# zhengchen1999/DOVE

Hardware: AMD Instinct MI355X
Metric: SR frames/s (33x720x1280 4x one-step, whole job) (higher is better)
Workload: dtype bf16; 1 GPU; synthetic 33x720x1280 HR clip (LR 180x320, 4x), one-step t=399, CogVideoX1.5-5B VAE + 42-layer DiT random-init, 1 clip per GPU (BASELINE configs[1]); weight_sums=True, vae_streams=2, variant=headline (bf16)

## Files before the change

### dove_amd/csrc/graph.hip

```cpp
#include <dlfcn.h>
#include <math.h>
#include <stdio.h>
#include <stdlib.h>
#include <string.h>

#include <algorithm>
#include <map>
#include <string>
#include <unordered_map>
#include <vector>

#include "common.h"
#include "../../include/dove_hip.h"
#include "ctx_access.h"

namespace {

#define CHK(expr)            \
  do {                       \
    const int rc__ = (expr); \
    if (rc__ != 0) return rc__; \
  } while (0)
#define HIPCHK(expr)                                                              \
  do {                                                                            \
// ... 1821 lines not shown
  DOVE_CHECK_ARG(oall, "workspace exhausted (DiT head)");
  std::vector<size_t> g_off(R), g_cnt(R);
  for (int j = 0; j < R; ++j) {
    const long long a0 = std::max<long long>(bounds[j], L) - L, a1 = std::max<long long>(bounds[j + 1], L) - L;
    g_off[j] = (size_t)a0 * width * 2; g_cnt[j] = (size_t)(a1 - a0) * width * 2;
  }
  bf16_t* po = nullptr;
  if (v1 > v0) {
    bf16_t* xv = hs + (size_t)lt_loc * D;
    bf16_t* a1 = A((size_t)(v1 - v0) * D * 2);
    DOVE_CHECK_ARG(a1, "workspace exhausted (DiT head)");
    CHK(dove_layernorm_modulate_bf16(xv, a1, v1 - v0, D, cf.dit_norm_eps, c->nf_g, c->nf_b, nullptr, 0, stream));
    CHK(dove_layernorm_modulate_bf16(a1, n1, v1 - v0, D, cf.dit_norm_eps, c->no_g, c->no_b, c->final_mod, 0, stream));
    CHK(linear(c, n1, v1 - v0, c->proj_out, ConvOpt(), &po, stream));
    c->arena.release(a1);
  }
  CHK(all_gather_v(c, po, oall, g_off.data(), g_cnt.data(), stream));
  CHK(dove_unpatchify(oall, width, T, cf.dit_out_channels, h, w, pt, p, v_out, out_dtype, stream));
  c->arena.release(po); c->arena.release(oall); c->arena.release(n1); c->arena.release(hs);
  return DOVE_OK;
}

extern "C" int dove_dit_forward(dove_ctx* c, const void* hidden, int dtype, int T, int h, int w, const void* text, int L, int timestep,
                                const dove_dit_aux* aux, void* v_out, int out_dtype, void* stream) {
  DOVE_CHECK_ARG(hidden && text && v_out, "dove_dit_forward: null pointer");
  const auto& cf = c->cfg;
  const int p = cf.dit_patch, pt = cf.dit_patch_t, Cc = cf.dit_in_channels, D = cf.dit_heads * cf.dit_head_dim, Hh = cf.dit_heads;
  DOVE_CHECK_ARG(T % pt == 0 && h % p == 0 && w % p == 0 && L >= 1, "dove_dit_forward: T / h / w must be multiples of the patch sizes");
  StageGuard guard(c);
  CHK(ensure_ws(c, 1 + 4 * (T - 1), 8 * h, 8 * w));
  if (c->nranks > 1) return dit_forward_ulysses(c, hidden, dtype, T, h, w, text, L, timestep, aux, v_out, out_dtype, stream);
  const long long nv = (long long)(T / pt) * (h / p) * (w / p), N = L + nv, npad = ru(N, 128);
  const float *cosp, *sinp;
  if (aux && aux->rope_cos && aux->rope_sin) { cosp = aux->rope_cos; sinp = aux->rope_sin; }
  else CHK(rope_tables(c, T / pt, h / p, w / p, &cosp, &sinp, stream));
  CHK(modulation(c, timestep, aux ? aux->timestep_proj : nullptr, stream));
  if (c->attn_n != N) {
    if (c->Qh) { (void)hipFree(c->Qh); (void)hipFree(c->Kh); (void)hipFree(c->Vt); }
    const size_t b = (size_t)Hh * npad * 64 * 2;
    HIPCHK(hipMalloc((void**)&c->Qh, b)); HIPCHK(hipMalloc((void**)&c->Kh, b)); HIPCHK(hipMalloc((void**)&c->Vt, b));
    HIPCHK(hipMemsetAsync(c->Qh, 0, b, (hipStream_t)stream)); HIPCHK(hipMemsetAsync(c->Kh, 0, b, (hipStream_t)stream)); HIPCHK(hipMemsetAsync(c->Vt, 0, b, (hipStream_t)stream));
    c->attn_n = N;
  }
  auto A = [&](size_t bytes) -> bf16_t* { return (bf16_t*)c->arena.alloc(bytes); };
  bf16_t* hs = A((size_t)N * D * 2);
  bf16_t* n1 = A((size_t)N * D * 2);
  const int feat_pad = c->pe_proj.cin_pad;
  bf16_t* tok = A((size_t)nv * feat_pad * 2);
  DOVE_CHECK_ARG(hs && n1 && tok, "workspace exhausted (DiT token buffers)");
  if (feat_pad > Cc * pt * p * p) HIPCHK(hipMemsetAsync(tok, 0, (size_t)nv * feat_pad * 2, (hipStream_t)stream));
  CHK(dove_patchify(hidden, dtype, T, Cc, h, w, pt, p, tok, feat_pad, stream));
  ConvOpt o; bf16_t* dummy;
  o = ConvOpt(); o.out = hs; CHK(linear(c, (const bf16_t*)text, L, c->pe_text, o, &dummy, stream));
  o = ConvOpt(); o.out = hs + (size_t)L * D; CHK(linear(c, tok, nv, c->pe_proj, o, &dummy, stream));
  c->arena.release(tok);
  const float qscale = (1.0f / sqrtf((float)cf.dit_head_dim)) * 1.4426950408889634f;
  float* norm2 = (float*)c->arena.alloc((size_t)Hh * 2 * sizeof(float));
  DOVE_CHECK_ARG(norm2, "workspace exhausted (attention score bounds)");
  if (c->opt_attn_mx && c->attn8_n != N) {
    if (c->Q8) { (void)hipFree(c->Q8); (void)hipFree(c->K8); (void)hipFree(c->V8); (void)hipFree(c->Vs8); }
    const size_t b8 = (size_t)Hh * npad * 64;
    HIPCHK(hipMalloc((void**)&c->Q8, b8)); HIPCHK(hipMalloc((void**)&c->K8, b8)); HIPCHK(hipMalloc((void**)&c->V8, b8));
    HIPCHK(hipMalloc((void**)&c->Vs8, (size_t)Hh * (npad / 64) * 64 * 2));
    HIPCHK(hipMemsetAsync(c->Q8, 0, b8, (hipStream_t)stream)); HIPCHK(hipMemsetAsync(c->K8, 0, b8, (hipStream_t)stream));
    HIPCHK(hipMemsetAsync(c->V8, 0, b8, (hipStream_t)stream)); HIPCHK(hipMemsetAsync(c->Vs8, 0, (size_t)Hh * (npad / 64) * 64 * 2, (hipStream_t)stream));
    c->attn8_n = N;
  }
  auto big = [&](const bf16_t* x, const Packed& pc, const PackedMx& p8, ConvOpt oo, bf16_t** out) -> int {
    if (!c->opt_linear_mx) return linear(c, x, N, pc, oo, out, stream);
    const int K = p8.K, Nn = p8.rows;
    uint8_t* xq = (uint8_t*)c->arena.alloc((size_t)N * K);
    uint32_t* xs = (uint32_t*)c->arena.alloc((size_t)(K / 256) * N * 2 * 4);
    bf16_t* y = oo.out ? oo.out : (bf16_t*)c->arena.alloc((size_t)N * Nn * 2);
    if (!xq || !xs || !y) { dove_set_error("workspace exhausted (MXFP8 linear)"); return DOVE_EINVAL; }
    CHK(dove_mx_quant_bf16(x, N, K, xq, xs, stream));
    CHK(dove_linear_mxfp8(xq, xs, p8.q, p8.s, p8.bias, oo.resid, oo.gate, y, N, Nn, K, Nn, oo.ldr, oo.gate_split, oo.act, stream));
    c->arena.release(xq); c->arena.release(xs);
    *out = y;
    return 0;
  };
  for (auto& b : c->blocks) {
    CHK(dove_layernorm_modulate_bf16(hs, n1, N, D, cf.dit_norm_eps, b.ln1_g, b.ln1_b, b.m1, L, stream));
    bf16_t* qkv;
    CHK(big(n1, b.qkv, b.qkv8, ConvOpt(), &qkv));
    if (c->opt_attn_mx) {
      CHK(dove_qkv_post_mxfp8(qkv, N, npad, Hh, 64, L, b.nq_g, b.nq_b, b.nk_g, b.nk_b, cosp, sinp, qscale, 1e-6f, c->Q8, c->K8, c->V8, c->Vs8, stream));
      c->arena.release(qkv);
      CHK(dove_attention_fwd_mxfp8(c->Q8, c->K8, c->V8, c->Vs8, n1, N, npad, Hh, 64, D, stream));
    } else {
      CHK(dove_qkv_post_bf16(qkv, N, npad, Hh, 64, L, b.nq_g, b.nq_b, b.nk_g, b.nk_b, cosp, sinp, qscale, 1e-6f, c->Qh, c->Kh, c->Vt, 1, norm2, stream));
      c->arena.release(qkv);
      CHK(dove_attention_fwd_bf16(c->Qh, c->Kh, c->Vt, n1, N, npad, Hh, 64, D, norm2, stream));
    }
    o = ConvOpt(); o.resid = hs; o.ldr = D; o.gate = b.g1; o.gate_split = L; o.out = hs;
    CHK(big(n1, b.out, b.out8, o, &dummy));
    CHK(dove_layernorm_modulate_bf16(hs, n1, N, D, cf.dit_norm_eps, b.ln2_g, b.ln2_b, b.m2, L, stream));
    bf16_t* f1;
    o = ConvOpt(); o.act = 1;
    CHK(big(n1, b.ff1, b.ff18, o, &f1));
    o = ConvOpt(); o.resid = hs; o.ldr = D; o.gate = b.g2; o.gate_split = L; o.out = hs;
    CHK(big(f1, b.ff2, b.ff28, o, &dummy));
    c->arena.release(f1);
  }
  bf16_t* xv = hs + (size_t)L * D;
  bf16_t* a1 = A((size_t)nv * D * 2);
  DOVE_CHECK_ARG(a1, "workspace exhausted (DiT head)");
  CHK(dove_layernorm_modulate_bf16(xv, a1, nv, D, cf.dit_norm_eps, c->nf_g, c->nf_b, nullptr, 0, stream));
  CHK(dove_layernorm_modulate_bf16(a1, n1, nv, D, cf.dit_norm_eps, c->no_g, c->no_b, c->final_mod, 0, stream));
  bf16_t* po;
  CHK(linear(c, n1, nv, c->proj_out, ConvOpt(), &po, stream));
  CHK(dove_unpatchify(po, c->proj_out.cout_store(), T, cf.dit_out_channels, h, w, pt, p, v_out, out_dtype, stream));
  c->arena.release(po); c->arena.release(a1); c->arena.release(n1); c->arena.release(hs); c->arena.release(norm2);
  return DOVE_OK;
}

extern "C" int dove_sr_clip(dove_ctx* c, const void* video_in, int dtype, int F, int H, int W, const void* noise, int noise_dtype,
                            const void* text, int Ltxt, int timestep, float sqrt_alpha, float sqrt_one_minus_alpha, const dove_dit_aux* aux,
                            const dove_pre_noise* pre, void* video_out, int out_dtype, void* stream) {
  DOVE_CHECK_ARG(video_in && noise && text && video_out, "dove_sr_clip: null pointer");
  DOVE_CHECK_ARG(!pre || pre->eps, "dove_sr_clip: pre_noise without eps");
  StageGuard guard(c);
  DOVE_CHECK_ARG(F >= 1 && H % 16 == 0 && W % 16 == 0, "dove_sr_clip: H and W must be multiples of 16 (8x VAE, 2x patch)");
  CHK(ensure_ws(c, F, H, W));
  const auto& cf = c->cfg;
  const int Lc = cf.vae_latent_channels, h = H / 8, w = W / 8;
  hipStream_t s = (hipStream_t)stream;
  Tensor m;
  CHK(vae_encode_cl(c, video_in, dtype, F, H, W, &m, stream));
  const int T = m.T;
  const long long fsz = (long long)h * w;
  if (c->nranks > 1) {
    RankPlan rp;
    rank_plan(c, true, F, &rp);
    std::vector<size_t> off(c->nranks), cnt(c->nranks);
    for (int j = 0; j < c->nranks; ++j) { off[j] = (size_t)rp.rank_first[j] * fsz * m.C * 2; cnt[j] = (size_t)rp.rank_count[j] * fsz * m.C * 2; }
    CHK(all_gather_v(c, (char*)m.p + off[c->rank], m.p, off.data(), cnt.data(), stream));
  }
  bf16_t* samp = (bf16_t*)c->arena.alloc((size_t)Lc * T * fsz * 2);
  DOVE_CHECK_ARG(samp, "workspace exhausted");
  CHK(dove_posterior_sample(m.p, m.C, Lc, (long long)T * fsz, noise, noise_dtype, samp, DOVE_BF16, stream));
  free_t(c, m);
  const int ncopy = T % cf.dit_patch_t, Td = T + ncopy;
  bf16_t* lat = (bf16_t*)c->arena.alloc((size_t)Td * Lc * fsz * 2);
  bf16_t* scaled = (bf16_t*)c->arena.alloc((size_t)Lc * T * fsz * 2);
  DOVE_CHECK_ARG(lat && scaled, "workspace exhausted");
  CHK(dove_axpby(samp, samp, scaled, DOVE_BF16, (long long)Lc * T * fsz, cf.vae_scaling_factor, 0.0f, stream));
  for (int t = 0; t < Td; ++t) {
    const int ts = t < ncopy ? 0 : t - ncopy;
    CHK(copy2d(lat + (long long)t * Lc * fsz, (size_t)fsz * 2, scaled + (long long)ts * fsz, (size_t)T * fsz * 2, (size_t)fsz * 2, Lc, s));
  }
  c->arena.release(samp); c->arena.release(scaled);
  if (pre) {
    bf16_t* noisy = (bf16_t*)c->arena.alloc((size_t)Td * Lc * fsz * 2);
    DOVE_CHECK_ARG(noisy, "workspace exhausted");
    const void* eps = pre->eps;
    bf16_t* eps16 = nullptr;
    if (pre->eps_dtype != DOVE_BF16) {
      eps16 = (bf16_t*)c->arena.alloc((size_t)Td * Lc * fsz * 2);
      DOVE_CHECK_ARG(eps16, "workspace exhausted");
      hipLaunchKernelGGL(to_bf16_kernel, dim3(256), dim3(256), 0, s, pre->eps, pre->eps_dtype, (long long)Td * Lc * fsz, eps16);
      eps = eps16;
    }
    CHK(dove_axpby(lat, eps, noisy, DOVE_BF16, (long long)Td * Lc * fsz, pre->sqrt_alpha, pre->sqrt_one_minus_alpha, stream));
    c->arena.release(lat); c->arena.release(eps16);
    lat = noisy;
  }
  bf16_t* vel = (bf16_t*)c->arena.alloc((size_t)Td * Lc * fsz * 2);
  DOVE_CHECK_ARG(vel, "workspace exhausted");
  CHK(dove_dit_forward(c, lat, DOVE_BF16, Td, h, w, text, Ltxt, timestep, aux, vel, DOVE_BF16, stream));
  bf16_t* x0 = (bf16_t*)c->arena.alloc((size_t)Td * Lc * fsz * 2);
  DOVE_CHECK_ARG(x0, "workspace exhausted");
  CHK(dove_axpby(lat, vel, x0, DOVE_BF16, (long long)Td * Lc * fsz, sqrt_alpha, -sqrt_one_minus_alpha, stream));
// ... 11 lines not shown
```

### dove_amd/csrc/igemm.hip

```cpp
#include "igemm_args.h"


template <int BN, int BK>
struct FastCfg {
  static constexpr int BM = 128;
  static constexpr int CPR = BK / 8;
  static constexpr int CPR_LOG = (BK == 64) ? 3 : 2;
  static constexpr int RPG = 256 / CPR;
  static constexpr int NA = BM / RPG;
  static constexpr int B_SLOTS = BN * CPR;
  static constexpr int NB = (B_SLOTS + 255) / 256;
  static constexpr int A_BYTES = BM * BK * 2, B_BYTES = BN * BK * 2, STAGE = A_BYTES + B_BYTES;
  static constexpr int WN = (BN >= 128) ? 2 : 1, WM = 4 / WN;
  static constexpr int PT = (BM / WM) / 32, CT = (BN / WN) / 32;
  static constexpr int KK = BK / 16;
};

template <int BN, int BK>
__global__ __launch_bounds__(256) void igemm_fast_kernel(const IgemmArgs a) {
  using Cf = FastCfg<BN, BK>;
  constexpr int NA = Cf::NA, NB = Cf::NB, PT = Cf::PT, CT = Cf::CT, KK = Cf::KK, STAGE = Cf::STAGE, A_BYTES = Cf::A_BYTES;
  extern __shared__ __attribute__((aligned(16))) char smem[];
  const int tid = threadIdx.x, lane = tid & 63;
  const int wave = __builtin_amdgcn_readfirstlane(tid >> 6);
  __builtin_assume(wave >= 0 && wave < 4);
  const int wm = wave / Cf::WN, wn = wave % Cf::WN;

  unsigned rest = xcd_remap(blockIdx.x, gridDim.x);
  const int tn = rest % a.tiles_n; rest /= a.tiles_n;
  const int twi = rest % a.tiles_w; rest /= a.tiles_w;
  const int thi = rest % a.tiles_h;
  const int t = rest / a.tiles_h;
  const int n0 = tn * BN;
  const int TWm = (1 << a.tw_log2) - 1;
  const int oh0 = thi * (128 >> a.tw_log2), ow0 = twi << a.tw_log2;

  const int cs = tid & (Cf::CPR - 1);
  const int rsub = tid >> Cf::CPR_LOG;
  const int c = (BK == 64) ? (cs ^ ((rsub >> 1) & 7)) : (cs ^ ((rsub >> 2) & 3));
  int rowoff[NA];
  unsigned mask[NA];
#pragma unroll
  for (int j = 0; j < NA; ++j) {
    const int m = j * Cf::RPG + rsub;
    const int oh = oh0 + (m >> a.tw_log2), ow = ow0 + (m & TWm);
    const bool mv = (oh < a.H_out) && (ow < a.W_out);
    const int ih0 = oh * a.stride - a.pad_h, iw0 = ow * a.stride - a.pad_w;
    rowoff[j] = ((ih0 * a.W_in + iw0) * a.Cin + c * 8) * 2;
    unsigned mk = 0;
    for (int dh = 0; dh < a.kh; ++dh)
      for (int dw = 0; dw < a.kw; ++dw) {
        const bool ok = mv && ((unsigned)(ih0 + dh) < (unsigned)a.H_in) && ((unsigned)(iw0 + dw) < (unsigned)a.W_in);
        mk |= (ok ? 1u : 0u) << (dh * a.kw + dw);
      }
    mask[j] = mk;
  }
  int boff_g[NB];
#pragma unroll
  for (int j = 0; j < NB; ++j) boff_g[j] = ((j * Cf::RPG + rsub) * a.Cin + c * 8) * 2;

  const long long frame_elems = (long long)a.H_in * a.W_in * a.Cin;
  const unsigned frame_bytes = (unsigned)(frame_elems * 2);
  const unsigned wtap_bytes = (unsigned)((long long)BN * a.Cin * 2);
  const long long wtap_stride = (long long)a.Cout_pad * a.Cin;
  const int kc_per_tap = a.Cin / BK;
  const int nk = a.kt * a.kh * a.kw * kc_per_tap;

  auto frame_ptr = [&](int dt) -> const bf16_t* { return igemm_src_frame(a, t, dt, frame_elems); };
  int s_kc = 0, s_dw = 0, s_dh = 0, s_dt = 0;
  const bf16_t* s_fp = frame_ptr(0);
  const bf16_t* s_wp = a.w + (long long)n0 * a.Cin;
  int s_tapdelta = 0;
  unsigned s_tapbit = 1u;

  auto stage = [&](auto bufc) {
    constexpr int BUF = decltype(bufc)::value;
    const auto srd_a = __builtin_amdgcn_make_buffer_rsrc((void*)s_fp, (short)0, (int)frame_bytes, 0x00020000);
    const auto srd_b = __builtin_amdgcn_make_buffer_rsrc((void*)s_wp, (short)0, (int)wtap_bytes, 0x00020000);
    const int soff = s_kc * (BK * 2);
#pragma unroll
    for (int j = 0; j < NA; ++j) {
      const unsigned voff = (mask[j] & s_tapbit) ? (unsigned)(rowoff[j] + s_tapdelta) : 0x80000000u;
      __builtin_amdgcn_raw_ptr_buffer_load_lds(srd_a, (lds_ptr_t)(smem + BUF * STAGE + (j * 256 + wave * 64) * 16), 16, voff, soff, 0, 0);
// ... 621 lines not shown
        for (int p = 0; p < 4; ++p) {
          const int oh = c.oh0 + RPW * wave + (kPart == 1 ? 2 * p : p);
          const long long pix0 = kSub ? ((long long)c.t * a.H_out + 2 * oh + (c.ph >> 1)) * a.W_out + 2 * c.ow0 + (c.ph & 1)
                                      : ((long long)c.t * a.H_out + oh) * a.W_out + c.ow0;
          const bool okh = kSub ? oh < a.H_in : oh < a.h_lim;
          const int span_px = kSub ? 2 * halo8::TW : (kPart == 1 ? a.W_out + 16 : halo8::TW);
          const auto srd_o = __builtin_amdgcn_make_buffer_rsrc((void*)(a.out + pix0 * a.ldo + c.n0), (short)0,
                                                               okh ? (int)(span_px * a.ldo * 2) : 0, 0x00020000);
          const auto srd_r = __builtin_amdgcn_make_buffer_rsrc((void*)(kRes ? a.resid + pix0 * a.ldr + c.n0 : a.out), (short)0,
                                                               (kRes && okh) ? (int)((kPart == 1 ? a.W_out + 16 : halo8::TW) * a.ldr * 2) : 0, 0x00020000);
          unsigned oo[4], ro[4];
          const bool ok1 = oh + 1 < a.h_lim;
#pragma unroll
          for (int it = 0; it < 4; ++it) {
            if (kPart == 1) { oo[it] = (it >= 2 && !ok1) ? 0x80000000u : o_off[it]; ro[it] = (it >= 2 && !ok1) ? 0x80000000u : r_off[it]; }
            else { oo[it] = o_off[it]; ro[it] = r_off[it]; }
          }
#pragma unroll
          for (int h = 0; h < 2; ++h) {
            u32x4 rr[4];
            if (kRes) {
#pragma unroll
              for (int it = 0; it < 4; ++it) rr[it] = __builtin_amdgcn_raw_buffer_load_b128(srd_r, (int)ro[it], h * 128, 0);
            }
            asm volatile("s_waitcnt lgkmcnt(0)" ::: "memory");
            f32x4 lo[4], hi4[4];
#pragma unroll
            for (int it = 0; it < 4; ++it) {
              lo[it] = *(const f32x4*)(eslice + (it * 8 + e_px) * EROW + e_ch * 32);
              hi4[it] = *(const f32x4*)(eslice + (it * 8 + e_px) * EROW + e_ch * 32 + 16);
            }
            asm volatile("s_waitcnt lgkmcnt(0)" ::: "memory");
            if (p < 3 || h < 1) wr(h ? p + 1 : p, h ^ 1);
#pragma unroll
            for (int it = 0; it < 4; ++it) {
              f32x4 x0 = lo[it] + bias_r[h][0], x1 = hi4[it] + bias_r[h][1];
              if (kRes) {
                const u32x4 r = rr[it];
                x0 += f32x4{__uint_as_float(r[0] << 16), __uint_as_float(r[0] & 0xffff0000u), __uint_as_float(r[1] << 16),
                            __uint_as_float(r[1] & 0xffff0000u)};
                x1 += f32x4{__uint_as_float(r[2] << 16), __uint_as_float(r[2] & 0xffff0000u), __uint_as_float(r[3] << 16),
                            __uint_as_float(r[3] & 0xffff0000u)};
              }
              const u32x4 v = {pack_bf2(x0[0], x0[1]), pack_bf2(x0[2], x0[3]), pack_bf2(x1[0], x1[1]), pack_bf2(x1[2], x1[3])};
              if (kGn) {
                const bool valid = okh && oo[it] != 0x80000000u;
#pragma unroll
                for (int e = 0; e < 4; ++e) {
                  const uint32_t w = valid ? v[e] : 0u;
                  const f32x2 f = {__uint_as_float(w << 16), __uint_as_float(w & 0xffff0000u)};
                  gs[h][e >> 1] += f;
                  gq[h][e >> 1] += f * f;
                }
              }
              __builtin_amdgcn_raw_buffer_store_b128(v, srd_o, (int)oo[it], h * 128, 0);
              __builtin_amdgcn_sched_barrier(0);
              asm volatile("s_nop 3" ::: "memory");
              __builtin_amdgcn_sched_barrier(0);
            }
          }
          if (kGn && kPart == 1 && p == 1) gn_flush(0);
        }
        if (kGn) gn_flush(kPart == 1 ? 1 : 0);
      };
      if (a.gn_partial) {
        if (a.resid) emit(std::true_type{}, std::true_type{});
        else emit(std::false_type{}, std::true_type{});
      } else {
        if (a.resid) emit(std::true_type{}, std::false_type{});
        else emit(std::false_type{}, std::false_type{});
      }
    }
    asm volatile("s_waitcnt vmcnt(0)" ::: "memory");
  }
}

namespace gemm8p {
constexpr int ROWB = 128;
constexpr int OPB = 256 * ROWB;
constexpr int XB = 0, WB = 2 * OPB;
constexpr int EPI = 4 * OPB;
constexpr int LDS_BYTES = EPI + 8 * 4096;
}
template <bool kAct, bool kGate>
__global__ __launch_bounds__(512, 2) void gemm8p_kernel(const IgemmArgs a, long long M) {
  using gemm4x::BM;
  using namespace gemm8p;
  extern __shared__ __attribute__((aligned(16))) char smem[];
  const int tid = threadIdx.x, lane = tid & 63;
  const int wave = __builtin_amdgcn_readfirstlane(tid >> 6);
  __builtin_assume(wave >= 0 && wave < 8);
  const int hi = lane >> 5, l31 = lane & 31;
  const int q4 = lane >> 4, l15 = lane & 15;
  const int grp = wave >> 2, wc = wave & 3;

  G4Const kc;
  kc.K = a.Cin;
  kc.M = M;
  kc.tiles_n = a.tiles_n;
  kc.ntiles = (int)((M + BM - 1) / BM) * a.tiles_n;
  kc.G = (int)gridDim.x;
  kc.nk4 = a.Cin / 128;
  const int ntiles = kc.ntiles, G = kc.G, nk4 = kc.nk4;

  unsigned voff[4];
#pragma unroll
  for (int jj = 0; jj < 4; ++jj) {
    const int row = (wave * 4 + jj) * 8 + (lane >> 3);
    const int c = (lane & 7) ^ ((row >> 1) & 7);
    voff[jj] = (unsigned)((row * a.Cin + c * 8) * 2);
  }
  G4State st;
  const bf16_t *ca_base = a.x, *cw_base = a.w, *na_base = a.x, *nw_base = a.w;
  int ca_nrec = 0, cw_nrec = 0, c_soff = 0, na_nrec = 0, nw_nrec = 0, n_soff = 0;
  auto publish = [&](const G4State& q) {
    ca_base = na_base; cw_base = nw_base; ca_nrec = na_nrec; cw_nrec = nw_nrec; c_soff = n_soff;
    na_base = q.a_base; nw_base = q.w_base; na_nrec = q.a_nrec; nw_nrec = q.w_nrec; n_soff = q.soff;
  };
  auto stage = [&](auto bufc, const bf16_t* ab, int anrec, const bf16_t* wb, int wnrec, int soff) {
    constexpr int buf = decltype(bufc)::value;
    const auto srd_a = __builtin_amdgcn_make_buffer_rsrc((void*)ab, (short)0, anrec, 0x00020000);
    const auto srd_w = __builtin_amdgcn_make_buffer_rsrc((void*)wb, (short)0, wnrec, 0x00020000);
#pragma unroll
    for (int jj = 0; jj < 4; ++jj)
      __builtin_amdgcn_raw_ptr_buffer_load_lds(srd_a, (lds_ptr_t)(smem + XB + buf * OPB + wave * 4096 + jj * 1024), 16, voff[jj], soff, 0, 0);
#pragma unroll
    for (int jj = 0; jj < 4; ++jj)
      __builtin_amdgcn_raw_ptr_buffer_load_lds(srd_w, (lds_ptr_t)(smem + WB + buf * OPB + wave * 4096 + jj * 1024), 16, voff[jj], soff, 0, 0);
  };

  int aoff[2][2], boff[2][2];
  {
    const int ra = grp * 128 + l31, rb = wc * 64 + l31;
#pragma unroll
    for (int h = 0; h < 2; ++h)
#pragma unroll
      for (int kk = 0; kk < 2; ++kk) {
        const int ch = h * 4 + kk * 2 + hi;
        aoff[h][kk] = XB + ra * ROWB + ((ch ^ ((ra >> 1) & 7)) << 4);
        boff[h][kk] = WB + rb * ROWB + ((ch ^ ((rb >> 1) & 7)) << 4);
        asm volatile("" : "+v"(aoff[h][kk]), "+v"(boff[h][kk]));
      }
  }
  int aoff16[2], boff16[2];
  {
    const int ra = grp * 128 + l15, rb = wc * 64 + l15;
#pragma unroll
    for (int h = 0; h < 2; ++h) {
      aoff16[h] = XB + ra * ROWB + (((h * 4 + q4) ^ ((ra >> 1) & 7)) << 4);
      boff16[h] = WB + rb * ROWB + (((h * 4 + q4) ^ ((rb >> 1) & 7)) << 4);
      asm volatile("" : "+v"(aoff16[h]), "+v"(boff16[h]));
    }
  }
  f32x4 acc16[4][8];
  bf16x8 x16[8], w16[4];

  g4_open_tile(st, a, kc, (int)blockIdx.x);
  publish(st);
  stage(std::integral_constant<int, 0>{}, na_base, na_nrec, nw_base, nw_nrec, n_soff);
  g4_advance(st, a, kc);
  publish(st);
  asm volatile("s_waitcnt vmcnt(0)" ::: "memory");
  __builtin_amdgcn_s_barrier();
  asm volatile("" ::: "memory");
  if (grp) {
    __builtin_amdgcn_sched_barrier(0);
    __builtin_amdgcn_s_barrier();
    __builtin_amdgcn_sched_barrier(0);
  }

  auto step = [&](auto uc, bool hold) {
    constexpr int u = decltype(uc)::value;
    constexpr int buf = u >> 1, h = u & 1;
#pragma unroll
    for (int pb = 0; pb < 8; ++pb) x16[pb] = *(const bf16x8*)(smem + aoff16[h] + buf * OPB + pb * (16 * ROWB));
#pragma unroll
    for (int ib = 0; ib < 4; ++ib) w16[ib] = *(const bf16x8*)(smem + boff16[h] + buf * OPB + ib * (16 * ROWB));
    if (u == 0) stage(std::integral_constant<int, 1>{}, ca_base, ca_nrec, cw_base, cw_nrec, c_soff + ROWB);
    if (u == 2) stage(std::integral_constant<int, 0>{}, na_base, na_nrec, nw_base, nw_nrec, n_soff);
    __builtin_amdgcn_sched_barrier(0);
    if (h == 1 && grp) asm volatile("s_waitcnt vmcnt(0)" ::: "memory");
    asm volatile("s_waitcnt lgkmcnt(0)" ::: "memory");
    __builtin_amdgcn_s_barrier();
    __builtin_amdgcn_sched_barrier(0);
    __builtin_amdgcn_s_setprio(1);
#pragma unroll
    for (int ib = 0; ib < 4; ++ib)
#pragma unroll
      for (int pb = 0; pb < 8; ++pb) acc16[ib][pb] = __builtin_amdgcn_mfma_f32_16x16x32_bf16(w16[ib], x16[pb], acc16[ib][pb], 0, 0, 0);
    __builtin_amdgcn_s_setprio(0);
    __builtin_amdgcn_sched_barrier(0);
    if (h == 1 && !grp) asm volatile("s_waitcnt vmcnt(0)" ::: "memory");
    if (u == 3 && hold) return;
    __builtin_amdgcn_s_barrier();
    __builtin_amdgcn_sched_barrier(0);
  };

  const int e_px = lane >> 2, e_ch = lane & 3;
  for (int tile = (int)blockIdx.x; tile < ntiles; tile += G) {
    const G4Tile c = g4_decode(kc, tile);
    const int col0 = c.n0 + wc * 64;
#pragma unroll
    for (int ib = 0; ib < 4; ++ib)
#pragma unroll
      for (int pb = 0; pb < 8; ++pb) acc16[ib][pb] = f32x4{0.f, 0.f, 0.f, 0.f};

    for (int kq = 0; kq < nk4; ++kq) {
      step(std::integral_constant<int, 0>{}, false);
      step(std::integral_constant<int, 1>{}, false);
      step(std::integral_constant<int, 2>{}, false);
      step(std::integral_constant<int, 3>{}, grp && kq == nk4 - 1);
      __builtin_amdgcn_sched_barrier(0);
      g4_advance(st, a, kc);
      publish(st);
      __builtin_amdgcn_sched_barrier(0);
    }

    asm volatile("" ::: "memory");
    f32x4 bias_r[2][2], gate_r[2][2][2];
#pragma unroll
    for (int h = 0; h < 2; ++h) {
      const int cb = col0 + h * 32 + e_ch * 8;
      bias_r[h][0] = bias_r[h][1] = f32x4{0.f, 0.f, 0.f, 0.f};
      if (a.bias) { bias_r[h][0] = *(const f32x4*)(a.bias + cb); bias_r[h][1] = *(const f32x4*)(a.bias + cb + 4); }
      if (kGate) {
#pragma unroll
        for (int cls = 0; cls < 2; ++cls) {
          gate_r[cls][h][0] = *(const f32x4*)(a.gate + (long long)cls * a.Cout_pad + cb);
          gate_r[cls][h][1] = *(const f32x4*)(a.gate + (long long)cls * a.Cout_pad + cb + 4);
        }
      }
    }
    {
      char* const eslice = smem + EPI + wave * 4096;
      unsigned o_off[2], r_off[2];
#pragma unroll
      for (int it = 0; it < 2; ++it) {
        const int px = it * 16 + e_px;
        o_off[it] = (unsigned)((px * (int)a.ldo + e_ch * 8) * 2);
        r_off[it] = (unsigned)((px * (int)a.ldr + e_ch * 8) * 2);
      }
      auto emit = [&](auto has_resid) {
        constexpr bool kRes = decltype(has_resid)::value;
#pragma unroll
        for (int p = 0; p < 4; ++p) {
          const long long row0 = (long long)c.m0 + grp * 128 + p * 32;
          const long long vl = M - row0;
          const int rows = vl >= 32 ? 32 : (vl > 0 ? (int)vl : 0);
          const auto srd_o = __builtin_amdgcn_make_buffer_rsrc((void*)(a.out + row0 * a.ldo + col0), (short)0,
                                                               rows * (int)a.ldo * 2, 0x00020000);
          const auto srd_r = __builtin_amdgcn_make_buffer_rsrc((void*)(kRes ? a.resid + row0 * a.ldr + col0 : a.out), (short)0,
                                                               kRes ? rows * (int)a.ldr * 2 : 0, 0x00020000);
#pragma unroll
          for (int h = 0; h < 2; ++h) {
            u32x4 rr[2];
            if (kRes) {
#pragma unroll
              for (int it = 0; it < 2; ++it) rr[it] = __builtin_amdgcn_raw_buffer_load_b128(srd_r, (int)r_off[it], h * 64, 0);
            }
#pragma unroll
            for (int dj = 0; dj < 2; ++dj)
#pragma unroll
              for (int di = 0; di < 2; ++di) {
                const int row = dj * 16 + l15, ch = di * 4 + q4;
                *(f32x4*)(eslice + row * 128 + ((ch ^ (row & 7)) << 4)) = acc16[2 * h + di][2 * p + dj];
              }
            asm volatile("s_waitcnt lgkmcnt(0)" ::: "memory");
            f32x4 lo[2], hi4[2];
#pragma unroll
            for (int it = 0; it < 2; ++it) {
              const int px = it * 16 + e_px;
              lo[it] = *(const f32x4*)(eslice + px * 128 + (((2 * e_ch) ^ (px & 7)) << 4));
              hi4[it] = *(const f32x4*)(eslice + px * 128 + (((2 * e_ch + 1) ^ (px & 7)) << 4));
            }
            asm volatile("s_waitcnt lgkmcnt(0)" ::: "memory");
#pragma unroll
            for (int it = 0; it < 2; ++it) {
              f32x4 x0 = lo[it] + bias_r[h][0], x1 = hi4[it] + bias_r[h][1];
              if (kAct) {
#pragma unroll
                for (int e = 0; e < 4; ++e) { x0[e] = gelu_tanh_f(x0[e]); x1[e] = gelu_tanh_f(x1[e]); }
              }
              if (kRes) {
                const u32x4 r = rr[it];
                const f32x4 r0 = {__uint_as_float(r[0] << 16), __uint_as_float(r[0] & 0xffff0000u), __uint_as_float(r[1] << 16),
                                  __uint_as_float(r[1] & 0xffff0000u)};
                const f32x4 r1 = {__uint_as_float(r[2] << 16), __uint_as_float(r[2] & 0xffff0000u), __uint_as_float(r[3] << 16),
                                  __uint_as_float(r[3] & 0xffff0000u)};
                if (kGate) {
                  const bool vid = row0 + it * 16 + e_px >= a.gate_split;
                  const f32x4 g0 = vid ? gate_r[1][h][0] : gate_r[0][h][0];
                  const f32x4 g1 = vid ? gate_r[1][h][1] : gate_r[0][h][1];
                  x0 = r0 + g0 * x0;
                  x1 = r1 + g1 * x1;
                } else {
                  x0 += r0;
                  x1 += r1;
                }
              }
              const u32x4 v = {pack_bf2(x0[0], x0[1]), pack_bf2(x0[2], x0[3]), pack_bf2(x1[0], x1[1]), pack_bf2(x1[2], x1[3])};
              if (a.nt_out) __builtin_amdgcn_raw_buffer_store_b128(v, srd_o, (int)o_off[it], h * 64, 2);
              else __builtin_amdgcn_raw_buffer_store_b128(v, srd_o, (int)o_off[it], h * 64, 0);
              __builtin_amdgcn_sched_barrier(0);
              asm volatile("s_nop 3" ::: "memory");
              __builtin_amdgcn_sched_barrier(0);
            }
          }
        }
      };
      if (a.resid) emit(std::true_type{});
      else emit(std::false_type{});
    }
    __builtin_amdgcn_s_waitcnt(0x0F70);
    asm volatile("" ::: "memory");
    if (grp) {
      __builtin_amdgcn_sched_barrier(0);
      __builtin_amdgcn_s_barrier();
      __builtin_amdgcn_sched_barrier(0);
    }
  }
  if (!grp) {
    __builtin_amdgcn_sched_barrier(0);
    __builtin_amdgcn_s_barrier();
  }
}

static std::atomic<bf16_t*> g_zero_page[DOVE_MAX_DEVICES] = {};

static const bf16_t* zero_page() {
  int dev = 0;
  if (hipGetDevice(&dev) != hipSuccess || dev < 0 || dev >= DOVE_MAX_DEVICES) return nullptr;
  bf16_t* z = g_zero_page[dev].load(std::memory_order_acquire);
  if (!z) {
    void* p = nullptr;
    if (hipMalloc(&p, 4096) != hipSuccess) return nullptr;
    if (hipMemset(p, 0, 4096) != hipSuccess) return nullptr;
    bf16_t* expect = nullptr;
    if (g_zero_page[dev].compare_exchange_strong(expect, (bf16_t*)p, std::memory_order_acq_rel)) z = (bf16_t*)p;
    else { (void)hipFree(p); z = expect; }
  }
  return z;
}

namespace smallk { constexpr int ROWS = 32; }
__global__ __launch_bounds__(256) void smallk_kernel(const bf16_t* __restrict__ x, const bf16_t* __restrict__ w, const float* __restrict__ bias,
                                                     bf16_t* __restrict__ out, long long M, int cout_store, long long ldo) {
  typedef __bf16 v2bf __attribute__((ext_vector_type(2)));
  __shared__ uint4 xs[4 * smallk::ROWS][4];
  const int lane = threadIdx.x & 63, wave = threadIdx.x >> 6;
  const long long rb = (long long)blockIdx.x * 4 * smallk::ROWS;
#pragma unroll
  for (int i = 0; i < 2; ++i) {
    const int idx = threadIdx.x + i * 256;
    const long long m = rb + (idx >> 2);
    xs[idx >> 2][idx & 3] = m < M ? *(const uint4*)(x + m * 32 + (idx & 3) * 8) : uint4{0u, 0u, 0u, 0u};
  }
  const int n0 = (blockIdx.y * 64 + lane) * 4;
  const bool live = n0 < cout_store;
  uint32_t wr[4][16];
  float b[4] = {0.f, 0.f, 0.f, 0.f};
  if (live) {
#pragma unroll
    for (int j = 0; j < 4; ++j)
#pragma unroll
      for (int q = 0; q < 4; ++q) {
        const uint4 v = *(const uint4*)(w + (long long)(n0 + j) * 32 + q * 8);
        wr[j][q * 4 + 0] = v.x; wr[j][q * 4 + 1] = v.y; wr[j][q * 4 + 2] = v.z; wr[j][q * 4 + 3] = v.w;
      }
    if (bias) { b[0] = bias[n0]; b[1] = bias[n0 + 1]; b[2] = bias[n0 + 2]; b[3] = bias[n0 + 3]; }
  }
  __syncthreads();
  if (!live) return;
  const long long r0 = rb + wave * smallk::ROWS;
#pragma unroll 4
  for (int r = 0; r < smallk::ROWS; ++r) {
    const long long m = r0 + r;
    if (m >= M) break;
    uint32_t xr[16];
#pragma unroll
    for (int q = 0; q < 4; ++q) {
      const uint4 v = xs[wave * smallk::ROWS + r][q];
      xr[q * 4 + 0] = v.x; xr[q * 4 + 1] = v.y; xr[q * 4 + 2] = v.z; xr[q * 4 + 3] = v.w;
    }
    float acc[4] = {b[0], b[1], b[2], b[3]};
#pragma unroll
    for (int k = 0; k < 16; ++k)
#pragma unroll
      for (int j = 0; j < 4; ++j)
        acc[j] = __builtin_amdgcn_fdot2_f32_bf16(__builtin_bit_cast(v2bf, wr[j][k]), __builtin_bit_cast(v2bf, xr[k]), acc[j], false);
    uint2 o;
    o.x = pack_bf2(acc[0], acc[1]);
    o.y = pack_bf2(acc[2], acc[3]);
    *(uint2*)(out + m * ldo + n0) = o;
  }
}

enum ConvKernel { K_IGEMM = 0, K_IGEMM_FAST, K_HALO4X, K_HALO4X_UP, K_GEMM8P, K_SMALLK, K_HALO4X_SUB };
static const char* const kKernelNames[] = {"igemm_kernel", "igemm_fast_kernel", "conv3x3_halo4x_kernel", "conv3x3_halo4x_kernel", "gemm8p_kernel",
                                           "smallk_kernel", "conv3x3_halo4x_kernel"};

static inline int desc_nb(const dove_conv_desc* d) { return d->nb > 1 ? d->nb : 1; }

static ConvKernel select_kernel(const dove_conv_desc* d) {
  const long long M = (long long)desc_nb(d) * d->t_out * d->h_out * d->w_out;
  const bool frame_fits = (long long)d->h_in * d->w_in * d->cin * 2 < (1ll << 31);
  const bool plain_gemm = d->kt == 1 && d->kh == 1 && d->kw == 1 && d->stride == 1 && d->up == 0 && d->tmode == 0 &&
                          d->t_in == d->t_out && d->h_in == d->h_out && d->w_in == d->w_out && d->cout_pad % 128 == 0 && M >= 4096 &&
// ... 1 lines not shown
  const bool pointwise = d->kt == 1 && d->kh == 1 && d->kw == 1 && d->stride == 1 && d->up == 0 && d->tmode == 0 && d->t_in == d->t_out &&
                         d->h_in == d->h_out && d->w_in == d->w_out;
  if (pointwise && d->cin == 32 && d->act == 0 && !d->resid && !d->gate && d->cout_store >= 128) return K_SMALLK;
  if (plain_gemm) {
    if (d->cout_pad % 256 == 0 && d->cout_store % 256 == 0 && d->cin % 128 == 0 && d->cin >= 256 && (long long)256 * d->cin * 2 < (1ll << 31) &&
        d->ldo < (1 << 20) && d->ldr < (1 << 20) && (d->act == 0 || d->act == 1))
      return K_GEMM8P;
  }
  const bool conv3 = d->kh == 3 && d->kw == 3 && d->stride == 1 && d->pad_h == 1 && d->pad_w == 1 && d->act == 0 && !d->gate &&
                     d->cout_pad % 128 == 0 && frame_fits;
  if (conv3) {
    const bool same = d->up == 0 && d->tmode == 0 && d->h_out == d->h_in && d->w_out == d->w_in && d->w_out >= 16 && d->h_out >= 16;
    const bool ups = d->up == 1 && d->kt == 1 && d->h_out == 2 * d->h_in && d->w_out == 2 * d->w_in && d->h_out >= 16 && d->w_out >= 32;
    const bool h4 = d->cout_store % 128 == 0 && d->cin % 64 == 0 && d->ldo < (1 << 20) && (!d->resid || d->ldr < (1 << 20));
    if (same && h4) return K_HALO4X;
    if (ups && h4 && d->w_sub && d->h_in >= 16 && d->w_in >= 32) return K_HALO4X_SUB;
    if (ups && h4) return K_HALO4X_UP;
  }
  const int BN = (d->cout_pad % 128 == 0) ? 128 : ((d->cout_pad % 64 == 0) ? 64 : 32);
  const bool fits = frame_fits && (long long)BN * d->cin * 2 < (1ll << 31);
  return (d->up == 0 && fits) ? K_IGEMM_FAST : K_IGEMM;
}

static bool desc_size_ok(const dove_conv_desc* d, const char* who) {
  if (d && d->struct_size == sizeof(dove_conv_desc) && d->reserved == 0) return true;
  if (d) dove_set_error("%s: dove_conv_desc.struct_size is %u, this library (ABI %d) expects %zu - the caller's binding was written "
                        "against another include/dove_hip.h", who, d->struct_size, DOVE_ABI_VERSION, sizeof(dove_conv_desc));
  else dove_set_error("%s: null descriptor", who);
  return false;
}
extern "C" const char* dove_conv_kernel_name(const dove_conv_desc* d) { return desc_size_ok(d, "conv_kernel_name") ? kKernelNames[select_kernel(d)] : ""; }

template <int BN, int BK>
static int launch_igemm_fast(const IgemmArgs& a, unsigned grid, hipStream_t s) {
  constexpr int lds = 2 * (128 * BK * 2 + BN * BK * 2);
  static PerDeviceOnce attr_set;
  if (auto once_ = attr_set.guard()) (void)hipFuncSetAttribute((const void*)igemm_fast_kernel<BN, BK>, hipFuncAttributeMaxDynamicSharedMemorySize, lds);
  hipLaunchKernelGGL((igemm_fast_kernel<BN, BK>), dim3(grid), dim3(256), lds, s, a);
  DOVE_CHECK_LAUNCH("dove_conv_igemm_bf16");
  return DOVE_OK;
}

static int cu_count() {
  static std::atomic<int> cus[DOVE_MAX_DEVICES] = {};
  int dev = 0;
  (void)hipGetDevice(&dev);
  int n = (dev >= 0 && dev < DOVE_MAX_DEVICES) ? cus[dev].load(std::memory_order_relaxed) : 0;
  if (!n) {
    n = 256;
    (void)hipDeviceGetAttribute(&n, hipDeviceAttributeMultiprocessorCount, dev);
    if (dev >= 0 && dev < DOVE_MAX_DEVICES) cus[dev].store(n, std::memory_order_relaxed);
  }
  return n;
}

extern "C" long long dove_conv_gn_partial_rows(const dove_conv_desc* d) {
  if (!desc_size_ok(d, "conv_gn_partial_rows")) return 0;
  const ConvKernel k = select_kernel(d);
  if (k != K_HALO4X && k != K_HALO4X_UP && k != K_HALO4X_SUB) return 0;
  if (d->cout_store != 128 && d->cout_store != 256 && d->cout_store != 512) return 0;
  if (d->cout_store != d->cout_pad) return 0;
  if (k == K_HALO4X_SUB) {
    const long long th = (d->h_in + halo8::TH - 1) / halo8::TH, tw = (d->w_in + halo8::TW - 1) / halo8::TW;
    return (long long)desc_nb(d) * d->t_out * th * tw * 16;
  }
  const long long th = (d->h_out + halo8::TH - 1) / halo8::TH, tw = (d->w_out + halo8::TW - 1) / halo8::TW;
  return (long long)desc_nb(d) * d->t_out * th * tw * 4;
}

static bool halo4x_plan(const dove_conv_desc* d) {
  const int tiles_w = (d->w_out + halo8::TW - 1) / halo8::TW, tiles_h = (d->h_out + halo8::TH - 1) / halo8::TH;
  const int wrem = d->w_out % halo8::TW;
  if (wrem < 1 || wrem > halo8::TW / 2) return false;
  const int cus = cu_count();
  const long long per = (long long)desc_nb(d) * d->t_out * (d->cout_pad / 128);
  auto rounds = [&](long long tiles) { return (tiles * per + cus - 1) / cus; };
  return rounds((long long)tiles_h * (tiles_w - 1)) + rounds((d->h_out + 31) / 32) < rounds((long long)tiles_h * tiles_w);
}
extern "C" int dove_conv_partial_launches(const dove_conv_desc* d) {
  if (!desc_size_ok(d, "conv_partial_launches") || select_kernel(d) != K_HALO4X) return 0;
  return halo4x_plan(d) ? 1 : 0;
}

static int conv_dispatch(const dove_conv_desc* d, void* stream, ConvKernel kern);

static bool gemm_tail_split(const dove_conv_desc* d, long long* rows_main) {
  const long long M = (long long)d->t_out * d->h_out * d->w_out;
  if (d->t_out != 1 || d->h_out != 1 || desc_nb(d) > 1) return false;
  const int cus = cu_count(), tiles_n = d->cout_pad / 256;
  const long long row_tiles = (M + gemm4x::BM - 1) / gemm4x::BM, ntiles = row_tiles * tiles_n;
  if (ntiles <= cus || ntiles % cus == 0) return false;
  const long long main_rt = (ntiles / cus) * cus / tiles_n;
  if (main_rt < 1 || main_rt >= row_tiles) return false;
  const long long tail_rows = M - main_rt * gemm4x::BM;
  const long long tail_blocks = ((tail_rows + 127) / 128) * (d->cout_pad / 128);
  if (tail_blocks > 2ll * cus) return false;
  if ((long long)128 * d->cin * 2 >= (1ll << 31)) return false;
  *rows_main = main_rt * gemm4x::BM;
  return true;
}

extern "C" int dove_conv_igemm_bf16(const dove_conv_desc* d, void* stream) {
  if (!desc_size_ok(d, "conv_igemm")) return DOVE_EINVAL;
  DOVE_CHECK_ARG(d->x && d->w && d->out, "conv_igemm: null pointer");
  DOVE_CHECK_ARG(d->cin % 32 == 0 && d->cin > 0, "conv_igemm: Cin (%d) must be a positive multiple of 32 (pad on pack)", d->cin);
  DOVE_CHECK_ARG(d->cout_pad % 32 == 0 && d->cout_pad > 0, "conv_igemm: Cout_pad (%d) must be a multiple of 32", d->cout_pad);
  DOVE_CHECK_ARG(d->cout_store % 4 == 0 && d->cout_store <= d->cout_pad && d->cout_store > 0, "conv_igemm: bad cout_store %d", d->cout_store);
  DOVE_CHECK_ARG(d->ldo % 4 == 0 && d->ldo >= d->cout_store, "conv_igemm: ldo (%lld) must be a multiple of 4 and >= cout_store", d->ldo);
  DOVE_CHECK_ARG(!d->resid || (d->ldr % 4 == 0 && d->ldr >= d->cout_store), "conv_igemm: bad ldr %lld", d->ldr);
  DOVE_CHECK_ARG(!d->gate || d->resid, "conv_igemm: gate needs resid");
  DOVE_CHECK_ARG(d->kt >= 1 && d->kt <= 3 && d->kh >= 1 && d->kw >= 1, "conv_igemm: bad kernel size");
  DOVE_CHECK_ARG(d->stride == 1 || d->stride == 2, "conv_igemm: stride must be 1 or 2");
  DOVE_CHECK_ARG(d->up == 0 || d->up == 1, "conv_igemm: up must be 0/1");
  DOVE_CHECK_ARG(d->kt == 1 || (d->tmode == 0 && d->t_in == d->t_out), "conv_igemm: causal temporal taps need t_in == t_out and tmode 0");
  DOVE_CHECK_ARG(d->t_out > 0 && d->h_out > 0 && d->w_out > 0 && d->t_in > 0 && d->h_in > 0 && d->w_in > 0, "conv_igemm: empty tensor");
  DOVE_CHECK_ARG(d->nb >= 0 && d->nb <= 4096 && (long long)desc_nb(d) * d->t_out < (1 << 20), "conv_igemm: bad instance count nb = %d", d->nb);
  DOVE_CHECK_ARG(d->cache_stride == 0 || (d->cache && d->cache_stride >= (long long)(d->kt - 1) * d->h_in * d->w_in * d->cin),
                 "conv_igemm: cache_stride (%lld) is smaller than one instance's cache", d->cache_stride);
  DOVE_CHECK_ARG(desc_nb(d) == 1 || !d->gate, "conv_igemm: nb > 1 is not combined with gate");
  DOVE_CHECK_ARG(d->reserved2 == 0 && d->tdup >= 0 && d->tdup <= 2, "conv_igemm: bad tdup %d", d->tdup);
  DOVE_CHECK_ARG(!d->tdup || (d->kt == 3 && d->w_pair), "conv_igemm: tdup declares frame pairs of a kt == 3 conv and needs w_pair");
  DOVE_CHECK_ARG(!d->tdup || d->cache || d->w_first, "conv_igemm: tdup without a conv cache needs w_first too (frames whose three taps read one frame)");
  DOVE_CHECK_ARG(d->tdup != 2 || !d->cache, "conv_igemm: tdup == 2 (first frame single) is the head of a clip: no conv cache");
  DOVE_CHECK_ARG(!d->gn_partial || dove_conv_gn_partial_rows(d) > 0,
                 "conv_igemm: gn_partial requested but this call does not dispatch to a kernel that fuses the statistics");
  const ConvKernel kern0 = select_kernel(d);
  DOVE_CHECK_ARG(!d->out_f32 || (kern0 == K_IGEMM_FAST && !d->resid && d->act == 0),
                 "conv_igemm: out_f32 is only implemented for plain convs that dispatch to igemm_fast_kernel");
  long long rows_main = 0;
  if (kern0 == K_GEMM8P && gemm_tail_split(d, &rows_main)) {
    dove_conv_desc m = *d, t = *d;
    m.w_in = m.w_out = (int)rows_main;
    const long long tail = (long long)d->w_out - rows_main;
    t.w_in = t.w_out = (int)tail;
    t.x = (const char*)d->x + rows_main * d->cin * 2;
    t.out = (char*)d->out + rows_main * d->ldo * 2;
    if (d->resid) t.resid = (const char*)d->resid + rows_main * d->ldr * 2;
    t.gate_split = d->gate_split > rows_main ? d->gate_split - rows_main : 0;
    const int rc = conv_dispatch(&m, stream, K_GEMM8P);
    return rc ? rc : conv_dispatch(&t, stream, K_IGEMM_FAST);
  }
  return conv_dispatch(d, stream, kern0);
}

static int conv_dispatch(const dove_conv_desc* d, void* stream, ConvKernel kern) {
  const bf16_t* zp = zero_page();
  DOVE_CHECK_ARG(zp, "conv_igemm: could not allocate the zero page");
  IgemmArgs a;
  a.x = (const bf16_t*)d->x; a.cache = (const bf16_t*)d->cache; a.w = (const bf16_t*)d->w;
  a.bias = d->bias; a.resid = (const bf16_t*)d->resid; a.gate = d->gate; a.out = (bf16_t*)d->out; a.zero = zp;
  const int nb = desc_nb(d);
  a.T_out = nb * d->t_out; a.H_out = d->h_out; a.W_out = d->w_out;
  a.T_in = nb * d->t_in; a.H_in = d->h_in; a.W_in = d->w_in;
  a.seg_out = d->t_out; a.seg_in = d->t_in;
  a.cache_bs = d->cache_stride ? d->cache_stride : (long long)(d->kt - 1) * d->h_in * d->w_in * d->cin;
  a.Cin = d->cin; a.Cout_pad = d->cout_pad; a.Cout_st = d->cout_store;
  a.kt = d->kt; a.kh = d->kh; a.kw = d->kw; a.stride = d->stride; a.pad_h = d->pad_h; a.pad_w = d->pad_w;
  a.up = d->up; a.tmode = d->tmode; a.act = d->act; a.ldo = d->ldo; a.ldr = d->ldr; a.gate_split = d->gate_split;
  a.gn_partial = nullptr; a.cpg_log = 0;
  a.w_first = nullptr;
  a.w_pair = nullptr; a.tdup = 0;
  a.sub = 0;
  a.out_f32 = d->out_f32;
  a.nt_out = 0;
  a.reserved = 0;
  hipStream_t s = (hipStream_t)stream;
  const long long M = (long long)nb * d->t_out * d->h_out * d->w_out;
  switch (kern) {
    case K_GEMM8P: {
      a.tiles_n = d->cout_pad / 256;
      a.nt_out = (long long)M * d->ldo * 2 > (256ll << 20);
      const long long nt = ((M + gemm4x::BM - 1) / gemm4x::BM) * a.tiles_n;
      DOVE_CHECK_ARG(nt > 0 && nt < (1ll << 31), "conv_igemm: grid too large");
      DOVE_CHECK_ARG(!(d->gate && d->act), "conv_igemm: gate with activation is not a path of the reference");
      const int cus = cu_count();
      const unsigned grid4 = nt > cus ? (unsigned)cus : (unsigned)nt;
      static PerDeviceOnce attr8;
      if (auto once_ = attr8.guard()) {
        (void)hipFuncSetAttribute((const void*)gemm8p_kernel<false, false>, hipFuncAttributeMaxDynamicSharedMemorySize, gemm8p::LDS_BYTES);
        (void)hipFuncSetAttribute((const void*)gemm8p_kernel<true, false>, hipFuncAttributeMaxDynamicSharedMemorySize, gemm8p::LDS_BYTES);
        (void)hipFuncSetAttribute((const void*)gemm8p_kernel<false, true>, hipFuncAttributeMaxDynamicSharedMemorySize, gemm8p::LDS_BYTES);
      }
      if (d->gate) hipLaunchKernelGGL((gemm8p_kernel<false, true>), dim3(grid4), dim3(512), gemm8p::LDS_BYTES, s, a, M);
      else if (d->act == 1) hipLaunchKernelGGL((gemm8p_kernel<true, false>), dim3(grid4), dim3(512), gemm8p::LDS_BYTES, s, a, M);
      else hipLaunchKernelGGL((gemm8p_kernel<false, false>), dim3(grid4), dim3(512), gemm8p::LDS_BYTES, s, a, M);
      DOVE_CHECK_LAUNCH("dove_conv_igemm_bf16(gemm8p)");
      return DOVE_OK;
    }
    case K_SMALLK: {
      dim3 grid((unsigned)((M + 4 * smallk::ROWS - 1) / (4 * smallk::ROWS)), (unsigned)((d->cout_store + 255) / 256));
      hipLaunchKernelGGL(smallk_kernel, grid, dim3(256), 0, s, a.x, a.w, a.bias, a.out, M, d->cout_store, d->ldo);
      DOVE_CHECK_LAUNCH("dove_conv_igemm_bf16(smallk)");
      return DOVE_OK;
    }
    case K_HALO4X_SUB: {
      a.gn_partial = d->gn_partial;
      a.cpg_log = d->cout_store == 128 ? 2 : (d->cout_store == 256 ? 3 : 4);
      a.sub = 1;
      a.w = (const bf16_t*)d->w_sub;
      a.ty0 = a.tx0 = 0;
      a.tiles_w = (d->w_in + halo8::TW - 1) / halo8::TW;
      a.tiles_h = (d->h_in + halo8::TH - 1) / halo8::TH;
      a.tiles_n = 4 * (d->cout_pad / 128);
      a.nty = a.tiles_h; a.ntx = a.tiles_w; a.h_lim = d->h_out; a.w_lim = d->w_out;
      const long long g4 = (long long)a.T_out * a.tiles_h * a.tiles_w * a.tiles_n;
      DOVE_CHECK_ARG(g4 > 0 && g4 < (1ll << 31), "conv_igemm: grid too large");
      static PerDeviceOnce attrs;
      if (auto once_ = attrs.guard()) (void)hipFuncSetAttribute((const void*)(conv3x3_halo4x_kernel<false, true>), hipFuncAttributeMaxDynamicSharedMemorySize, Halo4xCfg::LDS_BYTES);
      const int cus = cu_count();
      const unsigned grid = g4 > cus ? (unsigned)cus : (unsigned)g4;
      hipLaunchKernelGGL((conv3x3_halo4x_kernel<false, true>), dim3(grid), dim3(256), Halo4xCfg::LDS_BYTES, s, a);
      DOVE_CHECK_LAUNCH("dove_conv_igemm_bf16(halo4x sub-pixel)");
      return DOVE_OK;
    }
    case K_HALO4X:
    case K_HALO4X_UP: {
      a.gn_partial = d->gn_partial;
      a.w_first = (kern == K_HALO4X && d->kt == 3 && !d->cache) ? (const bf16_t*)d->w_first : nullptr;
      if (kern == K_HALO4X && d->kt == 3 && d->tdup) { a.tdup = d->tdup; a.w_pair = (const bf16_t*)d->w_pair; }
      a.cpg_log = d->cout_store == 128 ? 2 : (d->cout_store == 256 ? 3 : 4);
      a.tiles_w = (d->w_out + halo8::TW - 1) / halo8::TW;
      a.tiles_h = (d->h_out + halo8::TH - 1) / halo8::TH;
      a.tiles_n = d->cout_pad / 128;
      a.ty0 = a.tx0 = 0; a.nty = a.tiles_h; a.ntx = a.tiles_w; a.h_lim = d->h_out; a.w_lim = d->w_out;
      const long long g4 = (long long)a.T_out * a.tiles_h * a.tiles_w * a.tiles_n;
      DOVE_CHECK_ARG(g4 > 0 && g4 < (1ll << 31), "conv_igemm: grid too large");
      static PerDeviceOnce attr4;
      if (auto once_ = attr4.guard()) {
        (void)hipFuncSetAttribute((const void*)(conv3x3_halo4x_kernel<false>), hipFuncAttributeMaxDynamicSharedMemorySize, Halo4xCfg::LDS_BYTES);
        (void)hipFuncSetAttribute((const void*)(conv3x3_halo4x_kernel<false, false, 1>), hipFuncAttributeMaxDynamicSharedMemorySize, H4Geo<1>::LDS_BYTES);
        (void)hipFuncSetAttribute((const void*)(conv3x3_halo4x_kernel<true>), hipFuncAttributeMaxDynamicSharedMemorySize, Halo4xCfg::LDS_BYTES);
      }
      const int cus = cu_count();
      const unsigned grid = g4 > cus ? (unsigned)cus : (unsigned)g4;
      if (kern == K_HALO4X_UP) hipLaunchKernelGGL((conv3x3_halo4x_kernel<true>), dim3(grid), dim3(256), Halo4xCfg::LDS_BYTES, s, a);
      else {
        const bool wpart = halo4x_plan(d);
        const int wm = wpart ? (a.tiles_w - 1) * halo8::TW : d->w_out, cols_main = wpart ? a.tiles_w - 1 : a.tiles_w;
        auto launch = [&](int part, int nty, int tx0, int ntx, int w_lim) {
          if (nty <= 0 || ntx <= 0) return;
          IgemmArgs b = a;
          b.ty0 = 0; b.nty = nty; b.tx0 = tx0; b.ntx = ntx; b.h_lim = d->h_out; b.w_lim = w_lim;
          const long long g = (long long)b.T_out * nty * ntx * b.tiles_n;
          const unsigned gr = g > cus ? (unsigned)cus : (unsigned)g;
          if (part == 0) hipLaunchKernelGGL((conv3x3_halo4x_kernel<false, false, 0>), dim3(gr), dim3(256), H4Geo<0>::LDS_BYTES, s, b);
          else hipLaunchKernelGGL((conv3x3_halo4x_kernel<false, false, 1>), dim3(gr), dim3(256), H4Geo<1>::LDS_BYTES, s, b);
        };
        launch(0, a.tiles_h, 0, cols_main, wm);
        if (wpart) launch(1, (d->h_out + 31) / 32, cols_main, 1, d->w_out);
      }
      DOVE_CHECK_LAUNCH("dove_conv_igemm_bf16(halo4x)");
      return DOVE_OK;
    }
    default: break;
  }
  int twl = 7;
  if (d->h_out > 1) {
    twl = 4;
    if (d->w_out <= 8) twl = 3;
    if (d->w_out <= 4) twl = 2;
  }
  a.tw_log2 = twl;
  const int TW = 1 << twl, TH = 128 >> twl;
  a.tiles_w = (d->w_out + TW - 1) / TW;
  a.tiles_h = (d->h_out + TH - 1) / TH;
  const int BN = (d->cout_pad % 128 == 0) ? 128 : ((d->cout_pad % 64 == 0) ? 64 : 32);
// ... 11 lines not shown
```

### dove_amd/csrc/igemm_args.h

```cpp
#pragma once
#include <stdlib.h>

#include <type_traits>

#include "common.h"
#include "../../include/dove_hip.h"

struct IgemmArgs {
  const bf16_t* x;
  const bf16_t* cache;
  const bf16_t* w;
  const float* bias;
  const bf16_t* resid;
  const float* gate;
  bf16_t* out;
  const bf16_t* zero;
  int T_out, H_out, W_out;
  int T_in, H_in, W_in;
  int Cin, Cout_pad, Cout_st;
  int kt, kh, kw, stride, pad_h, pad_w, up, tmode, act;
  long long ldo, ldr;
  long long gate_split;
  int tw_log2, tiles_w, tiles_h, tiles_n;
  int reserved;
  float* gn_partial;
  int cpg_log;
  int out_f32;
  int nt_out;
  int seg_out, seg_in;
  long long cache_bs;
  const bf16_t* w_first;
  const bf16_t* w_pair;
  int tdup;
  int ty0, tx0, nty, ntx;
  int h_lim, w_lim;
  int sub;
};

__device__ __forceinline__ const bf16_t* igemm_src_frame(const IgemmArgs& a, int t, int dt, long long frame_elems) {
  const int b = a.seg_out == a.T_out ? 0 : t / a.seg_out;
  const int tl = t - b * a.seg_out;
  const long long f0 = (long long)b * a.seg_in;
  if (a.kt > 1) {
    const int fv = tl + dt - (a.kt - 1);
    if (fv >= 0) return a.x + (f0 + fv) * frame_elems;
    if (a.cache) return a.cache + (long long)b * a.cache_bs + (long long)(a.kt - 1 + fv) * frame_elems;
    return a.x + f0 * frame_elems;
  }
  const int tin = a.tmode == 0 ? tl : (a.tmode == 1 ? (tl >> 1) : (tl == 0 ? 0 : 1 + ((tl - 1) >> 1)));
  return a.x + (f0 + tin) * frame_elems;
}

typedef __attribute__((address_space(3))) void* lds_ptr_t;

namespace gemm4x {
constexpr int BM = 256, BN = 256;
constexpr int ROWB = 64;
}
struct G4Tile { int m0, n0; };
struct G4Const { int ntiles, G, tiles_n, nk4, K; long long M; };
struct G4State {
  int n_tile, n_k4;
  bool n_on;
  const bf16_t *a_base, *w_base;
  int a_nrec, w_nrec, soff;
};
__device__ __forceinline__ G4Tile g4_decode(const G4Const& k, int id) {
  const unsigned rest = xcd_remap((unsigned)(id < k.ntiles ? id : k.ntiles - 1), (unsigned)k.ntiles);
  const unsigned GM = k.tiles_n > 16 ? 8u : 1u;
  const unsigned tiles_m = (unsigned)(k.ntiles / k.tiles_n);
  const unsigned per_group = GM * (unsigned)k.tiles_n;
  const unsigned group = rest / per_group, within = rest - group * per_group;
  const unsigned left = tiles_m - group * GM;
  const unsigned gm = left < GM ? left : GM;
  G4Tile q;
  q.m0 = __builtin_amdgcn_readfirstlane((int)(group * GM + within % gm) * gemm4x::BM);
  q.n0 = __builtin_amdgcn_readfirstlane((int)(within / gm) * gemm4x::BN);
  return q;
}
__device__ __forceinline__ void g4_open_tile(G4State& s, const IgemmArgs& a, const G4Const& k, int id) {
  s.n_tile = id;
  s.n_on = id < k.ntiles;
  const G4Tile q = g4_decode(k, id);
  const long long left = k.M - q.m0;
  const int rows = left < gemm4x::BM ? (int)left : gemm4x::BM;
  s.a_base = a.x + (long long)q.m0 * k.K;
  s.w_base = a.w + (long long)q.n0 * k.K;
  s.a_nrec = s.n_on ? rows * k.K * 2 : 0;
  s.w_nrec = s.n_on ? gemm4x::BN * k.K * 2 : 0;
  s.n_k4 = 0;
  s.soff = 0;
}
__device__ __forceinline__ void g4_advance(G4State& s, const IgemmArgs& a, const G4Const& k) {
  if (++s.n_k4 == k.nk4) g4_open_tile(s, a, k, s.n_tile + k.G);
  s.soff = s.n_k4 * (4 * gemm4x::ROWB);
}

int launch_igemm_legacy(const IgemmArgs& a, unsigned grid, int BN, bool bk64, hipStream_t s);
```

### dove_amd/csrc/norm.hip

```cpp
#include "common.h"
#include "../../include/dove_hip.h"

__global__ __launch_bounds__(256) void gn_partial_kernel(const bf16_t* __restrict__ xall, long long npix, int C,
                                                         int cpp_log, float* __restrict__ partial_all) {
  const bf16_t* __restrict__ x = xall + (long long)blockIdx.y * npix * C;
  float* __restrict__ partial = partial_all + (long long)blockIdx.y * gridDim.x * 64;
  __shared__ float red[256 * 17];
  __shared__ float chan[2 * 2048];
  const int tid = threadIdx.x;
  const int cpp = 1 << cpp_log;
  const int q = tid & (cpp - 1), sub = tid >> cpp_log;
  const int nsub = 256 >> cpp_log;
  float s[8], ss[8];
#pragma unroll
  for (int e = 0; e < 8; ++e) { s[e] = 0.f; ss[e] = 0.f; }
  for (long long p = (long long)blockIdx.x * nsub + sub; p < npix; p += (long long)gridDim.x * nsub) {
    const uint4 v = *(const uint4*)(x + p * C + q * 8);
    float f[8];
    unpack8(v, f);
#pragma unroll
    for (int e = 0; e < 8; ++e) { s[e] += f[e]; ss[e] += f[e] * f[e]; }
  }
  float* r = red + (q * nsub + sub) * 17;
#pragma unroll
  for (int e = 0; e < 8; ++e) { r[e] = s[e]; r[8 + e] = ss[e]; }
  __syncthreads();
  for (int o = tid; o < 2 * C; o += 256) {
    const int ch = o >> 1, which = o & 1;
    const int qq = ch >> 3, e = ch & 7;
    float acc = 0.f;
    for (int k = 0; k < nsub; ++k) acc += red[(qq * nsub + k) * 17 + which * 8 + e];
    chan[o] = acc;
  }
  __syncthreads();
  const int cpg = C / 32;
  if (tid < 64) {
    const int g = tid >> 1, which = tid & 1;
    float acc = 0.f;
    for (int k = 0; k < cpg; ++k) acc += chan[(g * cpg + k) * 2 + which];
    partial[(long long)blockIdx.x * 64 + tid] = acc;
  }
}

template <typename PT>
__global__ __launch_bounds__(256) void gn_finalize_kernel(const PT* __restrict__ partial_all, int nblocks, double count,
                                                          float eps, float* __restrict__ stats_all) {
  const PT* __restrict__ partial = partial_all + (long long)blockIdx.x * nblocks * 64;
  float* __restrict__ stats = stats_all + blockIdx.x * 64;
  const int tid = threadIdx.x, j = tid & 63, part = tid >> 6;
  double acc = 0.0;
#pragma unroll 8
  for (int b = part; b < nblocks; b += 4) acc += (double)partial[(long long)b * 64 + j];
  __shared__ double sh[256];
  sh[tid] = acc;
  __syncthreads();
  if (tid < 64) sh[tid] = (sh[tid] + sh[tid + 64]) + (sh[tid + 128] + sh[tid + 192]);
  __syncthreads();
  if (tid < 32) {
    const double mean = sh[tid * 2] / count;
    double var = sh[tid * 2 + 1] / count - mean * mean;
    if (var < 0.0) var = 0.0;
    stats[tid * 2] = (float)mean;
    stats[tid * 2 + 1] = (float)(1.0 / sqrt(var + (double)eps));
  }
}

template <typename PT>
__global__ __launch_bounds__(256) void gn_sums_kernel(const PT* __restrict__ partial, int nblocks, double* __restrict__ sums) {
  const int tid = threadIdx.x, j = tid & 63, part = tid >> 6;
  double acc = 0.0;
#pragma unroll 8
  for (int b = part; b < nblocks; b += 4) acc += (double)partial[(long long)b * 64 + j];
  __shared__ double sh[256];
  sh[tid] = acc;
  __syncthreads();
  if (tid < 64) sums[tid] = (sh[tid] + sh[tid + 64]) + (sh[tid + 128] + sh[tid + 192]);
}
__global__ void gn_finalize_sums_kernel(const double* __restrict__ sums, double count, float eps, float* __restrict__ stats) {
  const int g = threadIdx.x;
  if (count <= 0.0) count = sums[64];
  if (g < 32) {
    const double mean = sums[g * 2] / count;
    double var = sums[g * 2 + 1] / count - mean * mean;
// ... 239 lines not shown
      Bv[cls * D + c] = b * (1.0f + sc) + sh;
    }
  }
  __syncthreads();
  const int lane = threadIdx.x & 63, wave = threadIdx.x >> 6;
  for (int r = 0; r < 8; ++r) {
    const long long row = (long long)blockIdx.x * 32 + wave * 8 + r;
    if (row >= rows) break;
    const bf16_t* xr = x + row * D;
    float f[NIT][8];
    float s = 0.f;
#pragma unroll
    for (int i = 0; i < NIT; ++i) {
      const int c0 = (i * 64 + lane) * 8;
      if (c0 < D) {
        unpack8(*(const uint4*)(xr + c0), f[i]);
#pragma unroll
        for (int e = 0; e < 8; ++e) s += f[i][e];
      } else {
#pragma unroll
        for (int e = 0; e < 8; ++e) f[i][e] = 0.f;
      }
    }
    const float mean = wave_sum(s) / (float)D;
    float v = 0.f;
#pragma unroll
    for (int i = 0; i < NIT; ++i) {
      const int c0 = (i * 64 + lane) * 8;
      if (c0 < D) {
#pragma unroll
        for (int e = 0; e < 8; ++e) { const float d = f[i][e] - mean; v += d * d; }
      }
    }
    const float rstd = rsqrtf(wave_sum(v) / (float)D + eps);
    const int cls = row < split ? 0 : 1;
    bf16_t* yr = y + row * D;
#pragma unroll
    for (int i = 0; i < NIT; ++i) {
      const int c0 = (i * 64 + lane) * 8;
      if (c0 < D) {
        const f32x4 a0 = *(const f32x4*)(A + cls * D + c0), a1 = *(const f32x4*)(A + cls * D + c0 + 4);
        const f32x4 b0 = *(const f32x4*)(Bv + cls * D + c0), b1 = *(const f32x4*)(Bv + cls * D + c0 + 4);
        float o[8];
#pragma unroll
        for (int e = 0; e < 4; ++e) {
          o[e] = (f[i][e] - mean) * rstd * a0[e] + b0[e];
          o[4 + e] = (f[i][4 + e] - mean) * rstd * a1[e] + b1[e];
        }
        *(uint4*)(yr + c0) = pack8(o);
      }
    }
  }
}

extern "C" int dove_layernorm_modulate_bf16(const void* x, void* y, long long rows, int D, float eps,
                                             const float* gamma, const float* beta, const float* mod,
                                             long long split, void* stream) {
  DOVE_CHECK_ARG(x && y && gamma && beta, "layernorm_modulate: null pointer");
  DOVE_CHECK_ARG(D % 8 == 0 && D > 0 && D <= 4096, "layernorm_modulate: D (%d) must be a multiple of 8, <= 4096", D);
  DOVE_CHECK_ARG(rows > 0, "layernorm_modulate: empty input");
  const int nit = (D + 511) / 512;
  const unsigned grid = (unsigned)((rows + 31) / 32);
  const size_t lds = (size_t)4 * D * sizeof(float);
  hipStream_t s = (hipStream_t)stream;
#define LN_LAUNCH(N)                                                                                          \
  hipLaunchKernelGGL((ln_mod_kernel<N>), dim3(grid), dim3(256), lds, s, (const bf16_t*)x, (bf16_t*)y, rows, D, eps, \
                     gamma, beta, mod, split)
  switch (nit) {
    case 1: LN_LAUNCH(1); break;
    case 2: LN_LAUNCH(2); break;
    case 3: LN_LAUNCH(3); break;
    case 4: LN_LAUNCH(4); break;
    case 5: LN_LAUNCH(5); break;
    case 6: LN_LAUNCH(6); break;
    case 7: LN_LAUNCH(7); break;
    default: LN_LAUNCH(8); break;
  }
#undef LN_LAUNCH
  DOVE_CHECK_LAUNCH("dove_layernorm_modulate_bf16");
  return DOVE_OK;
}

constexpr int QK_HB = 8;
__global__ __launch_bounds__(256) void qk_post_kernel(const bf16_t* __restrict__ qkv, long long N, long long Npad, int heads, int text_len,
                                                      const float* __restrict__ gq, const float* __restrict__ bq,
                                                      const float* __restrict__ gk, const float* __restrict__ bk,
                                                      const float* __restrict__ cosT, const float* __restrict__ sinT, float qscale, float eps,
                                                      bf16_t* __restrict__ Qh, bf16_t* __restrict__ Kh, float* __restrict__ norm2) {
  __shared__ unsigned smax[4][QK_HB];
  const int c = threadIdx.x & 7;
  const int h0 = blockIdx.y * QK_HB, which = blockIdx.z;
  const long long n = (long long)blockIdx.x * 32 + (threadIdx.x >> 3);
  const int D = heads * 64;
  const bool live = n < N;
  const long long nn = live ? n : N - 1;
  const float* gam = (which == 0 ? gq : gk) + c * 8;
  const float* bet = (which == 0 ? bq : bk) + c * 8;
  const f32x4 g0 = *(const f32x4*)gam, g1 = *(const f32x4*)(gam + 4), b0 = *(const f32x4*)bet, b1 = *(const f32x4*)(bet + 4);
  const bool rope = nn >= text_len && cosT;
  f32x4 c0 = {1.f, 1.f, 1.f, 1.f}, c1 = c0, s0 = {0.f, 0.f, 0.f, 0.f}, s1 = s0;
  if (rope) {
    const float* cr = cosT + (nn - text_len) * 64 + c * 8;
    const float* sr = sinT + (nn - text_len) * 64 + c * 8;
    c0 = *(const f32x4*)cr; c1 = *(const f32x4*)(cr + 4); s0 = *(const f32x4*)sr; s1 = *(const f32x4*)(sr + 4);
  }
  const float sc = which == 0 ? qscale : 1.0f;
  const bf16_t* src = qkv + nn * (3LL * D) + (long long)which * D + c * 8;
  bf16_t* dst = (which == 0 ? Qh : Kh) + nn * 64 + c * 8;
  uint4 raw[QK_HB];
#pragma unroll
  for (int j = 0; j < QK_HB; ++j) raw[j] = h0 + j < heads ? *(const uint4*)(src + (h0 + j) * 64) : uint4{0u, 0u, 0u, 0u};
#pragma unroll
  for (int j = 0; j < QK_HB; ++j) {
    float f[8];
    unpack8(raw[j], f);
    float s = 0.f;
#pragma unroll
    for (int e = 0; e < 8; ++e) s += f[e];
    s += __shfl_xor(s, 1); s += __shfl_xor(s, 2); s += __shfl_xor(s, 4);
    const float mean = s * (1.0f / 64.0f);
    float v = 0.f;
#pragma unroll
    for (int e = 0; e < 8; ++e) { const float t = f[e] - mean; v += t * t; }
    v += __shfl_xor(v, 1); v += __shfl_xor(v, 2); v += __shfl_xor(v, 4);
    const float rstd = rsqrtf(v * (1.0f / 64.0f) + eps);
#pragma unroll
    for (int e = 0; e < 8; ++e) f[e] = (f[e] - mean) * rstd * (e < 4 ? g0[e] : g1[e - 4]) + (e < 4 ? b0[e] : b1[e - 4]);
    if (rope) {
#pragma unroll
      for (int i = 0; i < 4; ++i) {
        const float a = f[2 * i], b = f[2 * i + 1];
        const float ca = i < 2 ? c0[2 * i] : c1[2 * i - 4], cb = i < 2 ? c0[2 * i + 1] : c1[2 * i - 3];
        const float sa = i < 2 ? s0[2 * i] : s1[2 * i - 4], sb = i < 2 ? s0[2 * i + 1] : s1[2 * i - 3];
        f[2 * i] = a * ca - b * sa;
        f[2 * i + 1] = b * cb + a * sb;
      }
    }
#pragma unroll
    for (int e = 0; e < 8; ++e) f[e] *= sc;
    const uint4 packed = pack8(f);
    if (live && h0 + j < heads) *(uint4*)(dst + (long long)(h0 + j) * Npad * 64) = packed;
    if (norm2) {
      float r[8];
      unpack8(packed, r);
      float q = 0.f;
#pragma unroll
      for (int e = 0; e < 8; ++e) q += r[e] * r[e];
      q += __shfl_xor(q, 1); q += __shfl_xor(q, 2); q += __shfl_xor(q, 4);
      unsigned qb = __float_as_uint(q);
      qb = max(qb, (unsigned)__shfl_xor((int)qb, 8)); qb = max(qb, (unsigned)__shfl_xor((int)qb, 16)); qb = max(qb, (unsigned)__shfl_xor((int)qb, 32));
      if ((threadIdx.x & 63) == 0) smax[threadIdx.x >> 6][j] = qb;
    }
  }
  if (norm2) {
    __syncthreads();
    const int j = threadIdx.x;
    if (j < QK_HB && h0 + j < heads) {
      atomicMax((unsigned*)(norm2 + (h0 + j) * 2 + which), max(max(smax[0][j], smax[1][j]), max(smax[2][j], smax[3][j])));
    }
  }
}

__global__ __launch_bounds__(256) void v_post_kernel(const bf16_t* __restrict__ qkv, long long N, long long Npad, int heads,
                                                     bf16_t* __restrict__ Vt, int v_swap) {
  __shared__ float vt[4][64][65];
  const int lane = threadIdx.x & 63, wave = threadIdx.x >> 6;
  const int h = blockIdx.y;
  const long long n0 = ((long long)blockIdx.x * 4 + wave) * 64;
  if (n0 >= N) return;
  const int D = heads * 64;
  const int t8 = lane >> 3, c = lane & 7;
#pragma unroll
  for (int i = 0; i < 8; ++i) {
    const long long n = n0 + i * 8 + t8;
    float f[8];
    if (n < N) unpack8(*(const uint4*)(qkv + n * (3LL * D) + 2LL * D + h * 64 + c * 8), f);
    else {
#pragma unroll
      for (int e = 0; e < 8; ++e) f[e] = 0.f;
    }
#pragma unroll
    for (int e = 0; e < 8; ++e) vt[wave][i * 8 + t8][c * 8 + e] = f[e];
  }
  __builtin_amdgcn_wave_barrier();
  asm volatile("s_waitcnt lgkmcnt(0)" ::: "memory");
  if ((Npad & 7) == 0) {
    bf16_t* dst = Vt + ((long long)h * 64 + lane) * Npad + n0;
#pragma unroll
    for (int j = 0; j < 8; ++j) {
      float o[8];
      const int g16 = (j >> 1) * 16, odd = (j & 1) * 4;
#pragma unroll
      for (int e = 0; e < 8; ++e) o[e] = v_swap ? vt[wave][g16 + odd + (e & 3) + (e >> 2) * 8][lane] : vt[wave][j * 8 + e][lane];
      if (n0 + j * 8 + 8 <= Npad) *(uint4*)(dst + j * 8) = pack8(o);
    }
  } else {
    bf16_t* dst = Vt + ((long long)h * 64 + lane) * Npad + n0;
    for (int j = 0; j < 64 && n0 + j < N; ++j) dst[j] = f2bf(vt[wave][j][lane]);
  }
}

extern "C" int dove_qkv_post_bf16(const void* qkv, long long N, long long Npad, int heads, int head_dim, int text_len,
                                   const float* gq, const float* bq, const float* gk, const float* bk,
                                   const float* cosT, const float* sinT, float qscale, float eps, void* Qh, void* Kh,
                                   void* Vt, int v_order, float* norm2, void* stream) {
  DOVE_CHECK_ARG(qkv && Qh && Kh && Vt && gq && bq && gk && bk, "qkv_post: null pointer");
  DOVE_CHECK_ARG(head_dim == 64, "qkv_post: head_dim must be 64 (got %d)", head_dim);
  DOVE_CHECK_ARG(N > 0 && Npad >= N, "qkv_post: Npad must be >= N");
  DOVE_CHECK_ARG((cosT == nullptr) == (sinT == nullptr), "qkv_post: cos/sin must both be given or both be null");
  DOVE_CHECK_ARG(v_order == 0 || (v_order == 1 && Npad % 16 == 0), "qkv_post: v_order 1 (quad-swapped V^T) needs Npad %% 16 == 0");
  if (norm2) {
    const hipError_t me = hipMemsetAsync(norm2, 0, sizeof(float) * 2 * heads, (hipStream_t)stream);
    if (me != hipSuccess) { dove_set_error("qkv_post: clearing norm2 failed: %s", hipGetErrorString(me)); return DOVE_ELAUNCH; }
  }
  hipLaunchKernelGGL(qk_post_kernel, dim3((unsigned)((N + 31) / 32), (unsigned)((heads + QK_HB - 1) / QK_HB), 2), dim3(256), 0, (hipStream_t)stream, (const bf16_t*)qkv, N, Npad, heads,
                     text_len, gq, bq, gk, bk, cosT, sinT, qscale, eps, (bf16_t*)Qh, (bf16_t*)Kh, norm2);
  hipLaunchKernelGGL(v_post_kernel, dim3((unsigned)((N + 255) / 256), heads), dim3(256), 0, (hipStream_t)stream, (const bf16_t*)qkv, N, Npad, heads,
                     (bf16_t*)Vt, v_order);
  DOVE_CHECK_LAUNCH("dove_qkv_post_bf16");
  return DOVE_OK;
}

__global__ __launch_bounds__(256) void vt_quad_swap_kernel(uint4* __restrict__ vt, long long ngroups) {
  const long long g = (long long)blockIdx.x * 256 + threadIdx.x;
  if (g >= ngroups) return;
  const uint4 a = vt[2 * g], b = vt[2 * g + 1];
  vt[2 * g] = uint4{a.x, a.y, b.x, b.y};
  vt[2 * g + 1] = uint4{a.z, a.w, b.z, b.w};
}
extern "C" int dove_vt_quad_swap_bf16(void* Vt, long long rows, long long Npad, void* stream) {
  DOVE_CHECK_ARG(Vt && rows > 0 && Npad > 0 && Npad % 16 == 0, "vt_quad_swap: Npad must be a positive multiple of 16");
  const long long ng = rows * (Npad / 16);
  hipLaunchKernelGGL(vt_quad_swap_kernel, dim3((unsigned)((ng + 255) / 256)), dim3(256), 0, (hipStream_t)stream, (uint4*)Vt, ng);
  DOVE_CHECK_LAUNCH("dove_vt_quad_swap_bf16");
  return DOVE_OK;
}

struct UlyPlaceArgs {
  const bf16_t *rq, *rk, *rv;
  bf16_t *Qh, *Kh, *Vt;
  int world, hloc;
  long long N, Npad;
  long long bound[17];
  long long off[17];
  int extra;
  float* norm2_out;
};
__device__ __forceinline__ int uly_rank(const UlyPlaceArgs& a, long long n) {
  int i = 0;
  while (i + 1 < a.world && n >= a.bound[i + 1]) ++i;
  return i;
}
__global__ __launch_bounds__(256) void ulysses_place_kernel(const UlyPlaceArgs a) {
  const long long t = (long long)blockIdx.x * 256 + threadIdx.x;
  if (blockIdx.y == 3) {
    if (t >= a.hloc * 2) return;
    const int h = (int)(t >> 1), e = (int)(t & 1);
    unsigned m = 0u;
    for (int i = 0; i < a.world; ++i) {
      const long long ci = a.bound[i + 1] - a.bound[i];
      m = max(m, ((const unsigned*)(a.rk + a.off[i] + ((long long)h * (ci + 1) + ci) * 64))[e]);
    }
    ((unsigned*)a.norm2_out)[t] = m;
    return;
  }
  if (blockIdx.y < 2) {
    const long long total = (long long)a.hloc * a.N * 8;
    if (t >= total) return;
    const int c = (int)(t & 7);
    const long long n = (t >> 3) % a.N;
    const int h = (int)((t >> 3) / a.N);
    const int i = uly_rank(a, n);
    const long long ci = a.bound[i + 1] - a.bound[i] + a.extra;
    const bf16_t* src = (blockIdx.y == 0 ? a.rq : a.rk) + a.off[i] + ((long long)h * ci + (n - a.bound[i])) * 64 + c * 8;
    bf16_t* dst = (blockIdx.y == 0 ? a.Qh : a.Kh) + ((long long)h * a.Npad + n) * 64 + c * 8;
    *(uint4*)dst = *(const uint4*)src;
  } else {
    const long long quads = a.Npad >> 2, total = (long long)a.hloc * 64 * quads;
    if (t >= total) return;
    const long long qd = t % quads;
    const long long row = t / quads;
    const int h = (int)(row >> 6), d = (int)(row & 63);
    bf16_t v[4];
#pragma unroll
    for (int e = 0; e < 4; ++e) {
      const long long n = qd * 4 + e;
      v[e] = 0;
      if (n < a.N) {
        const int i = uly_rank(a, n);
        const long long ci = a.bound[i + 1] - a.bound[i] + a.extra;
        v[e] = a.rv[a.off[i] + ((long long)h * 64 + d) * ci + (n - a.bound[i])];
      }
    }
    const int q = (int)(qd & 3);
    const long long pq = (qd & ~3ll) | (q == 1 ? 2 : (q == 2 ? 1 : q));
    uint2 w;
    w.x = (uint32_t)v[0] | ((uint32_t)v[1] << 16);
    w.y = (uint32_t)v[2] | ((uint32_t)v[3] << 16);
    *(uint2*)(a.Vt + row * a.Npad + pq * 4) = w;
  }
}
extern "C" int dove_ulysses_place_bf16(const void* rq, const void* rk, const void* rv, const long long* counts, int world, int hloc, long long N,
                                       long long Npad, void* Qh, void* Kh, void* Vt, float* norm2_out, void* stream) {
// ... 25 lines not shown
```

### dove_amd/lib.py

```python
from __future__ import annotations

import ctypes as C
import os

import torch

_HERE = os.path.dirname(os.path.abspath(__file__))
LIB_PATH = os.path.join(_HERE, "libdove_hip.so")
_lib = None

F32, BF16, U8 = 0, 1, 2
METRIC_PSNR, METRIC_SSIM, METRIC_RGB_TO_Y = 1, 2, 4
COLORFIX_WAVELET, COLORFIX_ADAIN, COLORFIX_CLAMP = 1, 2, 1
YUV_444, YUV_422, YUV_420, YUV_MONO = 0, 1, 2, 3
YUV_SITING_LEFT, YUV_SITING_CENTRE = 0, 1
VIDEO_RGB_U8, VIDEO_YUV = 0, 1
RESIZE_BILINEAR, RESIZE_BICUBIC, RESIZE_AREA = 0, 1, 2
ACT_NONE, ACT_RELU, ACT_SIGMOID, ACT_TANH = 0, 1, 2, 3


class ConvDesc(C.Structure):
    _fields_ = [
        ("struct_size", C.c_uint), ("reserved", C.c_uint),
        ("x", C.c_void_p), ("cache", C.c_void_p), ("w", C.c_void_p), ("bias", C.c_void_p),
# ... 27 lines not shown
    _fields_ = [("data", C.c_void_p), ("dtype", C.c_int), ("reserved", C.c_int),
                ("sn", C.c_longlong), ("sc", C.c_longlong), ("sh", C.c_longlong), ("sw", C.c_longlong)]


class YuvFormat(C.Structure):
    _fields_ = [("coef", C.c_int * 9), ("offset", C.c_int * 3), ("chroma", C.c_int), ("siting_h", C.c_int)]


class DitAux(C.Structure):
    _fields_ = [("rope_cos", C.c_void_p), ("rope_sin", C.c_void_p), ("timestep_proj", C.c_void_p)]


VIDEO_AUX_FN = C.CFUNCTYPE(C.c_int, C.c_void_p, C.c_int, C.c_int, C.c_int, C.POINTER(DitAux))


class VideoParams(C.Structure):
    _fields_ = [("struct_size", C.c_uint), ("reserved", C.c_uint),
                ("width", C.c_int), ("height", C.c_int), ("upscale", C.c_int),
                ("chunk_len", C.c_int), ("overlap_t", C.c_int), ("tile_h", C.c_int), ("tile_w", C.c_int), ("overlap_h", C.c_int),
                ("overlap_w", C.c_int), ("color_fix", C.c_int), ("in_format", C.c_int), ("out_format", C.c_int),
                ("in_yuv", YuvFormat), ("out_yuv", YuvFormat),
                ("text", C.c_void_p), ("text_len", C.c_int), ("timestep", C.c_int),
                ("sqrt_alpha", C.c_float), ("sqrt_one_minus_alpha", C.c_float),
                ("noise_step", C.c_int), ("noise_sqrt_alpha", C.c_float), ("noise_sqrt_one_minus_alpha", C.c_float),
                ("max_frames", C.c_int), ("max_push", C.c_int), ("seed", C.c_ulonglong),
                ("aux_fn", VIDEO_AUX_FN), ("aux_user", C.c_void_p)]

    def __init__(self, *a, **k):
        super().__init__(*a, **k)
        self.struct_size = C.sizeof(VideoParams)


class Conv2dF32Args(C.Structure):
    _fields_ = [("struct_size", C.c_uint), ("reserved", C.c_uint),
                ("x", C.c_void_p), ("w", C.c_void_p), ("bias", C.c_void_p), ("scale", C.c_void_p), ("shift", C.c_void_p), ("out", C.c_void_p),
                ("n", C.c_int), ("h", C.c_int), ("w_in", C.c_int), ("cin", C.c_int), ("cout", C.c_int), ("kh", C.c_int), ("kw", C.c_int),
                ("stride", C.c_int), ("act", C.c_int), ("out_mul", C.c_float), ("ldx", C.c_longlong), ("ldo", C.c_longlong)]

    def __init__(self, *a, **k):
        super().__init__(*a, **k)
        self.struct_size = C.sizeof(Conv2dF32Args)


class ConvnetConvF32Args(C.Structure):
    _fields_ = [("struct_size", C.c_uint), ("reserved", C.c_uint),
                ("x", C.c_void_p), ("w", C.c_void_p), ("bias", C.c_void_p), ("out", C.c_void_p),
                ("n", C.c_int), ("h", C.c_int), ("w_in", C.c_int), ("cin", C.c_int), ("cout", C.c_int), ("kh", C.c_int), ("kw", C.c_int),
                ("stride", C.c_int), ("pad_h", C.c_int), ("pad_w", C.c_int), ("relu", C.c_int), ("reserved2", C.c_int),
                ("ldx", C.c_longlong), ("ldo", C.c_longlong)]

    def __init__(self, *a, **k):
        super().__init__(*a, **k)
        self.struct_size = C.sizeof(ConvnetConvF32Args)


class PreNoise(C.Structure):
    _fields_ = [("eps", C.c_void_p), ("eps_dtype", C.c_int), ("sqrt_alpha", C.c_float), ("sqrt_one_minus_alpha", C.c_float)]


OPT_VAE_TILING, OPT_VAE_SAMPLE_HEIGHT, OPT_VAE_SAMPLE_WIDTH, OPT_DIT_LINEAR_MXFP8, OPT_DIT_ATTN_MXFP8, OPT_WEIGHT_SUMS, OPT_VAE_STREAMS = 1, 2, 3, 4, 5, 6, 7
STAT_HALO_PREPOSTED, STAT_HALO_BLOCKING, STAT_HALO_SENT, STAT_HALO_COMMUNICATORS = 100, 101, 102, 103


_VP, _I, _LL, _F = C.c_void_p, C.c_int, C.c_longlong, C.c_float
_ULL, _PI, _PLL = C.c_ulonglong, C.POINTER(C.c_int), C.POINTER(C.c_longlong)
XFER_FN = C.CFUNCTYPE(C.c_int, C.c_void_p, C.c_int, C.c_void_p, C.c_size_t, C.c_void_p)
GROUP_FN = C.CFUNCTYPE(C.c_int, C.c_void_p, C.c_void_p)

SIGNATURES = {
    "dove_conv_igemm_bf16": [C.POINTER(ConvDesc), _VP],
    "dove_groupnorm_stats_bf16": [_VP, _LL, _LL, _I, _F, _VP, _I, _VP, _VP],
    "dove_groupnorm_finalize_partials": [_VP, _LL, C.c_double, _F, _VP, _VP, _VP],
    "dove_groupnorm_stats_nb_bf16": [_VP, _I, _LL, _LL, _I, _F, _VP, _I, _VP, _VP],
    "dove_groupnorm_finalize_partials_nb": [_VP, _LL, _I, C.c_double, _F, _VP, C.c_size_t, _VP, _VP],
    "dove_groupnorm_apply_nb_bf16": [_VP, _VP, _I, _I, _I, _I, _I, _VP, _VP, _VP, _I, _VP, _I, _I, _I, _I, C.POINTER(C.c_int), _VP],
    "dove_avgpool_time_nb_bf16": [_VP, _I, _I, _LL, _VP, _VP],
    "dove_groupnorm_sums_bf16": [_VP, _LL, _LL, _I, _VP, _I, _VP, _VP],
    "dove_groupnorm_finalize_sums": [_VP, C.c_double, _F, _VP, _VP],
    "dove_groupnorm_sums_from_partials": [_VP, _LL, _VP, _VP, _VP],
    "dove_groupnorm_apply_bf16": [_VP, _VP, _I, _I, _I, _I, _VP, _VP, _VP, _I, _VP, _I, _I, _I, C.POINTER(C.c_int), _VP],
    "dove_layernorm_modulate_bf16": [_VP, _VP, _LL, _I, _F, _VP, _VP, _VP, _LL, _VP],
    "dove_qkv_post_bf16": [_VP, _LL, _LL, _I, _I, _I, _VP, _VP, _VP, _VP, _VP, _VP, _F, _F, _VP, _VP, _VP, _I, _VP, _VP],
    "dove_vt_quad_swap_bf16": [_VP, _LL, _LL, _VP],
    "dove_ulysses_place_bf16": [_VP, _VP, _VP, C.POINTER(C.c_longlong), _I, _I, _LL, _LL, _VP, _VP, _VP, _VP, _VP],
    "dove_cl_im2col3x3_from_ncthw": [_VP, _I, _I, _I, _I, _I, _I, _F, _F, _VP, _VP],
    "dove_conv_out_gather": [_VP, _LL, _I, _I, _I, _I, _VP, _F, _F, _F, _F, _VP, _I, _VP],
    "dove_attention_fwd_bf16": [_VP, _VP, _VP, _VP, _LL, _LL, _I, _I, _LL, _VP, _VP],
    "dove_qkv_post_mxfp8": [_VP, _LL, _LL, _I, _I, _I, _VP, _VP, _VP, _VP, _VP, _VP, _F, _F, _VP, _VP, _VP, _VP, _VP],
    "dove_attention_fwd_mxfp8": [_VP, _VP, _VP, _VP, _VP, _LL, _LL, _I, _I, _LL, _VP],
    "dove_cl_from_ncthw": [_VP, _I, _I, _LL, _I, _F, _F, _VP, _VP],
    "dove_ncthw_from_cl": [_VP, _LL, _I, _LL, _F, _F, _F, _F, _VP, _I, _VP],
    "dove_avgpool_time_bf16": [_VP, _I, _LL, _VP, _VP],
    "dove_posterior_sample": [_VP, _LL, _I, _LL, _VP, _I, _VP, _I, _VP],
    "dove_axpby": [_VP, _VP, _VP, _I, _LL, _F, _F, _VP],
    "dove_patchify": [_VP, _I, _I, _I, _I, _I, _I, _I, _VP, _LL, _VP],
    "dove_unpatchify": [_VP, _LL, _I, _I, _I, _I, _I, _I, _VP, _I, _VP],
    "dove_gemv_bf16": [_VP, _VP, _VP, _I, _I, _I, _VP, _VP],
    "dove_blend_edge_bf16": [_VP, _VP, _I, _I, _I, _I, _I, _I, _I, _I, _VP],
    "dove_preprocess_u8": [_VP, _I, _I, _I, _I, _I, _I, _I, _VP, _I, _VP],
    "dove_postprocess_u8": [_VP, _I, _I, _I, _I, _I, _I, _I, _VP, _VP],
    "dove_rmsnorm_bf16": [_VP, _VP, _LL, _I, _F, _VP, _VP],
    "dove_gated_gelu_bf16": [_VP, _VP, _LL, _I, _VP],
    "dove_attention_bias_bf16": [_VP, _VP, _VP, _LL, _VP, _VP, _LL, _I, _I, _I, _VP],
    "dove_mx_quant_bf16": [_VP, _LL, _I, _VP, _VP, _VP],
    "dove_create": [_I, C.POINTER(ModelConfig), C.POINTER(_VP)],
    "dove_set_weight": [_VP, C.c_char_p, _VP, C.POINTER(C.c_longlong), _I, _I],
    "dove_finalize_weights": [_VP],
    "dove_set_workspace": [_VP, _VP, C.c_size_t],
    "dove_vae_encode": [_VP, _VP, _I, _I, _I, _I, _VP, _I, _VP],
    "dove_dit_forward": [_VP, _VP, _I, _I, _I, _I, _VP, _I, _I, C.POINTER(DitAux), _VP, _I, _VP],
    "dove_vae_decode": [_VP, _VP, _I, _I, _I, _I, _F, _I, _VP, _I, _VP],
    "dove_sr_clip": [_VP, _VP, _I, _I, _I, _I, _VP, _I, _VP, _I, _I, _F, _F, C.POINTER(DitAux), C.POINTER(PreNoise), _VP, _I, _VP],
    "dove_set_option": [_VP, _I, _LL],
    "dove_comm_unique_id": [_VP],
    "dove_comm_init": [_VP, _VP, _I, _I],
    "dove_comm_init_custom": [_VP, _I, _I, XFER_FN, XFER_FN, _VP],
    "dove_comm_set_group": [_VP, GROUP_FN, GROUP_FN],
    "dove_shard_frames": [_VP, _I, _I, C.POINTER(C.c_int), C.POINTER(C.c_int)],
    "dove_conv_out_gather_cl": [_VP, _LL, _I, _I, _I, _I, _VP, _VP, _I, _VP],
    "dove_tile_gather_bf16": [_VP, _I, _I, _I, _I, _I, _I, _I, _I, C.POINTER(C.c_int), C.POINTER(C.c_int), _I, _VP, _VP],
    "dove_linear_mxfp8": [_VP, _VP, _VP, _VP, _VP, _VP, _VP, _VP, _LL, _I, _I, _LL, _LL, _LL, _I, _VP],
    "dove_fr_metrics": [C.POINTER(ImageView), C.POINTER(ImageView), _I, _I, _I, _I, _I, _VP, C.c_size_t, _VP, _VP],
    "dove_color_fix": [C.POINTER(ImageView), _F, _F, C.POINTER(ImageView), _F, _F, _I, _I, _I, _I, _I, C.POINTER(ImageView), _VP,
                       C.c_size_t, _VP],
    "dove_rgb_to_yuv_u8": [C.POINTER(ImageView), _I, _I, _I, C.POINTER(YuvFormat), _VP, _VP],
    "dove_yuv_to_rgb_u8": [_VP, _I, _I, _I, C.POINTER(YuvFormat), _VP, _VP],
    "dove_plan_padding": [_I, _I, _I, _PI, _PI, _PI],
    "dove_plan_output_size": [_I, _I, _I, _PI, _PI],
    "dove_plan_temporal_chunks": [_I, _I, _I, _PI, _I],
    "dove_plan_spatial_tiles": [_I, _I, _I, _I, _I, _I, _PI, _I],
    "dove_plan_valid_region": [_PI, _I, _I, _I, _I, _I, _I, _PI, _PI],
    "dove_plan_pieces": [_I, _I, _I, _I, _I, _I, _I, _I, _I, _PI, _PI, _PI, _I],
    "dove_plan_check_coverage": [_PI, _I, _I, _I, _I],
    "dove_chunk_planner_create": [_I, _I, C.POINTER(_VP)],
    "dove_chunk_planner_next": [_VP, _LL, _I, _PLL, _PLL, _PI],
    "dove_philox_u32": [_VP, _LL, _ULL, _ULL, _ULL, _VP],
    "dove_randn": [_VP, _I, _LL, _ULL, _ULL, _ULL, _VP],
    "dove_blur2d_f32": [_VP, _I, _I, _I, _VP, _I, _I, _VP, _VP],
    "dove_resize_f32": [_VP, _I, _I, _I, _I, _I, _I, _VP, _VP],
    "dove_add_gaussian_noise_f32": [_VP, _I, _I, _I, C.POINTER(C.c_float), _I, _ULL, _ULL, _LL, _VP, _VP],
    "dove_add_poisson_noise_f32": [_VP, _I, _I, _I, C.POINTER(C.c_float), _I, _ULL, _ULL, _LL, _VP, C.c_size_t, _VP, _VP],
    "dove_jpeg_roundtrip": [_VP, _I, _I, _I, _PI, _VP, C.c_size_t, _VP, _VP],
    "dove_stitch": [_VP, _I, _I, _I, _PI, _VP, _I, _I, _I, _I, _I, _I, _VP],
    "dove_video_open": [_VP, C.POINTER(VideoParams), C.POINTER(_VP)],
    "dove_video_info": [_VP, C.POINTER(C.c_size_t), C.POINTER(C.c_size_t), _PI, _PI, _PI],
    "dove_video_push": [_VP, _VP, _I, _VP],
    "dove_video_end_of_input": [_VP],
    "dove_video_need": [_VP, _PLL, _PI],
    "dove_video_step": [_VP, _VP, C.c_size_t, _PI, _PI, _VP],
    "dove_conv2d_f32": [C.POINTER(Conv2dF32Args), _VP],
    "dove_instance_norm_f32": [_VP, _I, _I, _I, _I, _VP, _I, _F, _VP, C.c_size_t, _VP, _VP],
    "dove_corr_volume_f32": [_VP, _VP, _I, _I, _I, _I, _F, _VP, _VP],
    "dove_avgpool2_f32": [_VP, _LL, _I, _I, _VP, _VP],
    "dove_corr_lookup_f32": [_VP, _VP, _VP, _VP, _VP, _LL, _I, _I, _I, _I, _VP, _VP],
    "dove_gru_gate_f32": [_VP, _LL, _VP, _LL, _I, _I, _LL, _VP, _VP],
    "dove_gru_update_f32": [_VP, _LL, _VP, _LL, _VP, _LL, _I, _LL, _VP],
    "dove_add_f32": [_VP, _LL, _VP, _LL, _VP, _LL, _I, _LL, _I, _VP],
    "dove_convex_upsample_f32": [_VP, _LL, _VP, _I, _I, _I, _VP, _VP],
    "dove_flow_warp_error": [_VP, _VP, _I, _VP, _VP, _I, _I, _I, _VP, C.c_size_t, _VP, _VP, _VP, _VP],
    "dove_convnet_conv_f32": [C.POINTER(ConvnetConvF32Args), _VP],
    "dove_percep_prep_f32": [C.POINTER(ImageView), _I, _I, _I, _I, _F, _F, C.POINTER(C.c_float), C.POINTER(C.c_float), _VP, _VP],
    "dove_maxpool_f32": [_VP, _LL, _I, _I, _I, _I, _I, _I, _VP, _LL, _VP],
    "dove_l2pool_f32": [_VP, _LL, _I, _I, _I, _I, _VP, _LL, _VP],
    "dove_lpips_layer": [_VP, _VP, _LL, _VP, _I, _I, _I, _I, _VP, C.c_size_t, _VP, _VP],
    "dove_dists_layer": [_VP, _VP, _LL, _VP, _VP, _I, _I, _I, _I, _VP, C.c_size_t, _VP, _VP],
}
# ... 98 lines not shown
```

### dove_amd/ops.py

```python
from __future__ import annotations

import ctypes as C
import math
from dataclasses import dataclass

import torch

from . import lib as L


def _ru(x: int, m: int) -> int:
    return (x + m - 1) // m * m


@dataclass
class PackedConv:
    w: torch.Tensor
    bias: torch.Tensor | None
    kt: int
    kh: int
    kw: int
    cin: int
    cin_pad: int
    cout: int
# ... 248 lines not shown
    if nb > 1:
        assert x.dim() == 4 and x.shape[0] % nb == 0
        stats = torch.empty(nb, 32, 2, dtype=torch.float32, device=x.device)
        L.check(L.load().dove_groupnorm_stats_nb_bf16(L.ptr(x), nb, x.numel() // Cc // nb, _frame_pix(x), Cc, eps, L.ptr(ws), ws.numel() // 64,
                                                      L.ptr(stats), L.stream_ptr()), "dove_groupnorm_stats_nb_bf16")
        return stats
    stats = torch.empty(32, 2, dtype=torch.float32, device=x.device)
    L.check(L.load().dove_groupnorm_stats_bf16(L.ptr(x), x.numel() // Cc, _frame_pix(x), Cc, eps, L.ptr(ws), ws.numel() // 64, L.ptr(stats),
                                               L.stream_ptr()), "dove_groupnorm_stats_bf16")
    return stats


def groupnorm_sums(x: torch.Tensor) -> torch.Tensor:
    L.require_cuda(x)
    assert x.dtype == torch.bfloat16
    Cc = x.shape[-1]
    sums = torch.empty(32, 2, dtype=torch.float64, device=x.device)
    ws = _ws(x.device, _gn_rows_needed(x, x.shape[0] if x.dim() == 4 else 1))
    L.check(L.load().dove_groupnorm_sums_bf16(L.ptr(x), x.numel() // Cc, _frame_pix(x), Cc, L.ptr(ws), ws.numel() // 64, L.ptr(sums),
                                              L.stream_ptr()), "dove_groupnorm_sums_bf16")
    return sums


def groupnorm_sums_of(x: torch.Tensor) -> torch.Tensor:
    rows = getattr(x, "gn_rows", None)
    if rows is None:
        return groupnorm_sums(x)
    sums = torch.empty(32, 2, dtype=torch.float64, device=x.device)
    L.check(L.load().dove_groupnorm_sums_from_partials(L.ptr(rows), rows.shape[0], L.ptr(_ws(x.device)), L.ptr(sums), L.stream_ptr()),
            "dove_groupnorm_sums_from_partials")
    return sums


def groupnorm_from_sums(sums: torch.Tensor, count: float, eps: float) -> torch.Tensor:
    L.require_cuda(sums)
    assert sums.dtype == torch.float64 and (sums.shape == (32, 2) if count is not None else sums.numel() == 65)
    stats = torch.empty(32, 2, dtype=torch.float32, device=sums.device)
    L.check(L.load().dove_groupnorm_finalize_sums(L.ptr(sums.contiguous()), 0.0 if count is None else float(count), eps, L.ptr(stats), L.stream_ptr()),
            "dove_groupnorm_finalize_sums")
    return stats


def groupnorm_apply(x, stats, gamma, beta, *, silu=True, yb=None, sshift=0, tmap=None, out=None, nb=1):
    L.require_cuda(x, stats, gamma, beta, yb, out)
    T, H, W, Cc = x.shape
    assert T % nb == 0 and stats.numel() == nb * 64
    T //= nb
    if out is None:
        out = torch.empty_like(x)
    Tz = hz = wz = 0
    tm = None
    if yb is not None:
        assert yb.dtype == torch.bfloat16 and yb.shape[-1] == 2 * Cc and tmap is not None and len(tmap) == T and yb.shape[0] % nb == 0
        Tz, hz, wz = yb.shape[0] // nb, yb.shape[1], yb.shape[2]
        tm = (C.c_int * T)(*tmap)
    L.check(L.load().dove_groupnorm_apply_nb_bf16(L.ptr(x), L.ptr(out), nb, T, H, W, Cc, L.ptr(stats), L.ptr(gamma), L.ptr(beta),
                                                  int(silu), L.ptr(yb), Tz, hz, wz, sshift, tm, L.stream_ptr()),
            "dove_groupnorm_apply_nb_bf16")
    return out


def layernorm_modulate(x, gamma, beta, eps, mod=None, split=0, out=None):
    L.require_cuda(x, gamma, beta, mod, out)
    assert x.dtype == torch.bfloat16 and x.dim() == 2
    if out is None:
        out = torch.empty_like(x)
    if mod is not None:
        assert mod.dtype == torch.float32 and mod.shape == (2, 2, x.shape[1])
    L.check(L.load().dove_layernorm_modulate_bf16(L.ptr(x), L.ptr(out), x.shape[0], x.shape[1], eps, L.ptr(gamma),
                                                  L.ptr(beta), L.ptr(mod), split, L.stream_ptr()),
            "dove_layernorm_modulate_bf16")
    return out


def qkv_post(qkv, N, Npad, heads, text_len, gq, bq, gk, bk, cos, sin, qscale, eps, Qh, Kh, Vt, v_order=1, norm2=None):
    L.require_cuda(qkv, gq, bq, gk, bk, cos, sin, Qh, Kh, Vt, norm2)
    if norm2 is not None:
        assert norm2.dtype == torch.float32 and norm2.shape == (heads, 2) and norm2.is_contiguous()
    L.check(L.load().dove_qkv_post_bf16(L.ptr(qkv), N, Npad, heads, 64, text_len, L.ptr(gq), L.ptr(bq), L.ptr(gk), L.ptr(bk),
                                        L.ptr(cos), L.ptr(sin), qscale, eps, L.ptr(Qh), L.ptr(Kh), L.ptr(Vt), v_order, L.ptr(norm2),
                                        L.stream_ptr()), "dove_qkv_post_bf16")


def vt_quad_swap(Vt):
    L.require_cuda(Vt)
    assert Vt.is_contiguous()
    L.check(L.load().dove_vt_quad_swap_bf16(L.ptr(Vt), Vt.numel() // Vt.shape[-1], Vt.shape[-1], L.stream_ptr()), "dove_vt_quad_swap_bf16")
    return Vt


def ulysses_place(rq, rk, rv, counts, hloc, N, Npad, Qh, Kh, Vt, norm2_out=None):
    L.require_cuda(rq, rk, rv, Qh, Kh, Vt, norm2_out)
    if norm2_out is not None:
        assert norm2_out.dtype == torch.float32 and norm2_out.shape == (hloc, 2)
    cnt = (C.c_longlong * len(counts))(*[int(c) for c in counts])
    L.check(L.load().dove_ulysses_place_bf16(L.ptr(rq), L.ptr(rk), L.ptr(rv), cnt, len(counts), hloc, N, Npad, L.ptr(Qh), L.ptr(Kh), L.ptr(Vt),
                                             L.ptr(norm2_out), L.stream_ptr()), "dove_ulysses_place_bf16")


def attention(Qh, Kh, Vt, N, Npad, heads, out, norm2=None):
    L.require_cuda(Qh, Kh, Vt, out, norm2)
    if norm2 is not None:
        assert norm2.dtype == torch.float32 and norm2.shape == (heads, 2) and norm2.is_contiguous()
    L.check(L.load().dove_attention_fwd_bf16(L.ptr(Qh), L.ptr(Kh), L.ptr(Vt), L.ptr(out), N, Npad, heads, 64, out.shape[1], L.ptr(norm2),
                                             L.stream_ptr()), "dove_attention_fwd_bf16")
    return out


def attention_head_paths(norm2, heads=None):
    lib = L.load()
    if norm2 is None:
        host, n = None, int(heads)
    else:
        host = norm2.detach().float().cpu().contiguous()
        n = host.shape[0]
    path = (C.c_int * n)()
    L.check(lib.dove_attention_head_paths(None if host is None else C.cast(host.data_ptr(), C.POINTER(C.c_float)), n, path),
            "dove_attention_head_paths")
    return [lib.dove_attention_path_name(int(v)).decode() for v in path]


def qkv_post_mx(qkv, N, Npad, heads, text_len, gq, bq, gk, bk, cos, sin, qscale, eps, Q8, K8, V8t, Vs):
    L.require_cuda(qkv, gq, bq, gk, bk, cos, sin, Q8, K8, V8t, Vs)
    L.check(L.load().dove_qkv_post_mxfp8(L.ptr(qkv), N, Npad, heads, 64, text_len, L.ptr(gq), L.ptr(bq), L.ptr(gk), L.ptr(bk),
                                         L.ptr(cos), L.ptr(sin), qscale, eps, L.ptr(Q8), L.ptr(K8), L.ptr(V8t), L.ptr(Vs),
                                         L.stream_ptr()), "dove_qkv_post_mxfp8")


def attention_mx(Q8, K8, V8t, Vs, N, Npad, heads, out):
    L.require_cuda(Q8, K8, V8t, Vs, out)
    L.check(L.load().dove_attention_fwd_mxfp8(L.ptr(Q8), L.ptr(K8), L.ptr(V8t), L.ptr(Vs), L.ptr(out), N, Npad, heads, 64,
                                              out.shape[1], L.stream_ptr()), "dove_attention_fwd_mxfp8")
    return out


def cl_im2col3x3_from_ncthw(x: torch.Tensor, cp: int, scale=1.0, shift=0.0) -> torch.Tensor:
    L.require_cuda(x)
    Cc, T, H, W = x.shape
    y = torch.empty(T, H, W, cp, dtype=torch.bfloat16, device=x.device)
    L.check(L.load().dove_cl_im2col3x3_from_ncthw(L.ptr(x), L.dt_code(x), Cc, T, H, W, cp, scale, shift, L.ptr(y), L.stream_ptr()),
            "dove_cl_im2col3x3_from_ncthw")
    return y


def conv_out_gather(p: torch.Tensor, Cc: int, bias, dtype, scale=1.0, shift=0.0, lo=-math.inf, hi=math.inf) -> torch.Tensor:
    L.require_cuda(p, bias)
    assert p.dtype == torch.float32 and p.dim() == 4
    T, H, W, ld = p.shape
    y = torch.empty(Cc, T, H, W, dtype=dtype, device=p.device)
    L.check(L.load().dove_conv_out_gather(L.ptr(p), ld, T, H, W, Cc, L.ptr(bias), scale, shift, lo, hi, L.ptr(y), L.dt_code(y),
                                          L.stream_ptr()), "dove_conv_out_gather")
    return y


def conv_out_gather_cl(p: torch.Tensor, Cc: int, bias, ld: int = 8) -> torch.Tensor:
    L.require_cuda(p, bias)
    assert p.dtype == torch.float32 and p.dim() == 4
    T, H, W, ldp = p.shape
    y = torch.empty(T, H, W, ld, dtype=torch.bfloat16, device=p.device)
    L.check(L.load().dove_conv_out_gather_cl(L.ptr(p), ldp, T, H, W, Cc, L.ptr(bias), L.ptr(y), ld, L.stream_ptr()), "dove_conv_out_gather_cl")
    return y


def tile_gather(x: torch.Tensor, t0: int, nt: int, th: int, tw: int, origins, im2col_cin: int = 0) -> torch.Tensor:
    import ctypes as C
    L.require_cuda(x)
# ... 603 lines not shown
```

### dove_amd/transformer.py

```python
from __future__ import annotations

import math

import torch

from . import ops
from .config import AttrDict


def _ru(x, m):
    return (x + m - 1) // m * m


class CogVideoXTransformer3DModel:
    def __init__(self, config: dict, state_dict: dict, device="cuda", dtype=torch.bfloat16, linear_precision: str = "bf16",
                 attention_precision: str = "bf16"):
        self.config = AttrDict(config)
        self.device = torch.device(device)
        self.dtype = dtype
        c = self.config
        self.heads, self.hd = c["num_attention_heads"], c["attention_head_dim"]
        if self.hd != 64:
            raise NotImplementedError("HIP attention kernels are built for head_dim 64")
        self.D = self.heads * self.hd
# ... 86 lines not shown
    def _modulation(self, t: int):
        if t in self._mod_cache:
            return self._mod_cache[t]
        D = self.D
        temb = self.timestep_projection(t)
        e1 = ops.gemv(self.te[0][0], self.te[0][1], temb, act_in=0)
        emb = ops.gemv(self.te[1][0], self.te[1][1], e1, act_in=1)
        out = []
        for blk in self.blocks:
            item = {}
            for key, gname, mname in (("mod1", "gate1", "m1"), ("mod2", "gate2", "m2")):
                v = ops.gemv(blk[key][0], blk[key][1], emb, act_in=1).view(6, D)
                item[mname] = torch.stack([torch.stack([v[3], v[4]]), torch.stack([v[0], v[1]])]).contiguous()
                g = torch.zeros(2, _ru(D, 32), dtype=torch.float32, device=self.device)
                g[0, :D], g[1, :D] = v[5], v[2]
                item[gname] = g
            out.append(item)
        v = ops.gemv(self.mod_out[0], self.mod_out[1], emb, act_in=1).view(2, D)
        final = torch.stack([torch.stack([v[0], v[1]]), torch.stack([v[0], v[1]])]).contiguous()
        self._mod_cache = {t: (out, final)}
        return self._mod_cache[t]

    def _buffers(self, N):
        npad = _ru(N, 128)
        key = (N,)
        if key not in self._bufs:
            if self.attention_precision == "mxfp8":
                z = lambda *s: torch.zeros(*s, dtype=torch.uint8, device=self.device)
                self._bufs = {key: (npad, z(self.heads, npad, 64), z(self.heads, npad, 64), z(self.heads, 64, npad),
                                    z(self.heads, npad // 64, 64, 2))}
            else:
                z = lambda *s: torch.zeros(*s, dtype=torch.bfloat16, device=self.device)
                self._bufs = {key: (npad, z(self.heads, npad, 64), z(self.heads, npad, 64), z(self.heads, 64, npad), None)}
        return self._bufs[key]

    @torch.no_grad()
    def __call__(self, hidden_states, encoder_hidden_states, timestep, timestep_cond=None, ofs=None,
                 image_rotary_emb=None, attention_kwargs=None, return_dict: bool = True, _trace: dict | None = None):
        if image_rotary_emb is None:
            raise ValueError("image_rotary_emb is required (use_rotary_positional_embeddings=True)")
        B = hidden_states.shape[0]
        ts = [int(v) for v in timestep.reshape(-1).tolist()]
        if len(ts) == 1:
            ts = ts * B
        outs = [self._forward_one(hidden_states[b], encoder_hidden_states[b], ts[b], image_rotary_emb, _trace if b == 0 else None)
                for b in range(B)]
        out = torch.stack(outs)
        if return_dict:
            class _O:
                sample = out
            return _O()
        return (out,)

    forward = __call__

    def _forward_one(self, hidden, text, t, rope, trace=None):
        D, Lh = self.D, self.heads
        T, Cc, H, W = hidden.shape
        p, pt = self.p, self.pt
        hidden = hidden.to(self.device).contiguous()
        text = text.to(self.device, torch.bfloat16).contiguous()
        cos, sin = (r.to(self.device, torch.float32).contiguous() for r in rope)
        Lt = text.shape[0]
        nv = (T // pt) * (H // p) * (W // p)
        assert cos.shape == (nv, self.hd), (cos.shape, nv)
        N = Lt + nv
        blocks_mod, final_mod = self._modulation(t)
        npad, Qh, Kh, Vt, Vs = self._buffers(N)
        norm2 = torch.empty(Lh, 2, dtype=torch.float32, device=self.device)

        hs = torch.empty(N, D, dtype=torch.bfloat16, device=self.device)
        tok = ops.patchify(hidden, pt, p, self.pe_proj.cin_pad)
        ops.linear(text, self.pe_text, out=hs[:Lt])
        ops.linear(tok, self.pe_proj, out=hs[Lt:])
        qscale = (self.hd ** -0.5) * math.log2(math.e)
        if trace is not None:
            trace["embed"] = hs.clone()
        if self.linear_precision == "mxfp8":
            big = lambda x, w, **kw: ops.linear_mx(ops.mx_quant(x), w, **kw)
        else:
            big = ops.linear
        for bi, (blk, md) in enumerate(zip(self.blocks, blocks_mod)):
            n1 = ops.layernorm_modulate(hs, blk["ln1"][0], blk["ln1"][1], self.eps, md["m1"], Lt)
            qkv = big(n1, blk["qkv"])
            if Vs is not None:
                ops.qkv_post_mx(qkv, N, npad, Lh, Lt, blk["nq"][0], blk["nq"][1], blk["nk"][0], blk["nk"][1], cos, sin, qscale,
                                1e-6, Qh, Kh, Vt, Vs)
                att = ops.attention_mx(Qh, Kh, Vt, Vs, N, npad, Lh, n1)
            else:
                ops.qkv_post(qkv, N, npad, Lh, Lt, blk["nq"][0], blk["nq"][1], blk["nk"][0], blk["nk"][1], cos, sin, qscale,
                             1e-6, Qh, Kh, Vt, norm2=norm2)
                if self.attn_bound_trace is not None:
                    self.attn_bound_trace.append(norm2.clone())
                att = ops.attention(Qh, Kh, Vt, N, npad, Lh, n1, norm2=norm2 if self.attn_score_bound else None)
                if self.attn_bound_trace is not None:
                    self.attn_path_trace.append(norm2.clone() if self.attn_score_bound else torch.full_like(norm2, float("nan")))
            big(att, blk["out"], resid=hs, gate=md["gate1"], gate_split=Lt, out=hs)
            n2 = ops.layernorm_modulate(hs, blk["ln2"][0], blk["ln2"][1], self.eps, md["m2"], Lt, out=n1)
            f1 = big(n2, blk["ff1"], act=1)
            big(f1, blk["ff2"], resid=hs, gate=md["gate2"], gate_split=Lt, out=hs)
            if trace is not None:
                trace[f"block{bi}"] = hs.clone()
        xv = hs[Lt:]
        xv = ops.layernorm_modulate(xv, self.norm_final[0], self.norm_final[1], self.eps)
        xv = ops.layernorm_modulate(xv, self.norm_out[0], self.norm_out[1], self.eps, final_mod, 0)
        o = ops.linear(xv, self.proj_out)
        return ops.unpatchify(o, T, Cc, H, W, pt, p, self.dtype)
```

### include/dove_hip.h

```cpp
#ifndef DOVE_HIP_H
#define DOVE_HIP_H

#include <stddef.h>

#ifdef __cplusplus
extern "C" {
#endif

#define DOVE_ABI_VERSION 15

#define DOVE_F32 0
#define DOVE_BF16 1

const char* dove_last_error(void);
int dove_abi_version(void);
int dove_device_info(int dev, char* name, int name_len, int* cu_count, long long* total_mem);

typedef struct dove_conv_desc {
  unsigned int struct_size;
  unsigned int reserved;
  const void* x;
  const void* cache;
  const void* w;
  const float* bias;
  const void* resid;
  const float* gate;
  void* out;
  int t_in, h_in, w_in, cin;
  int t_out, h_out, w_out, cout_pad, cout_store;
  int kt, kh, kw, stride, pad_h, pad_w, up, tmode, act;
  long long ldo, ldr, gate_split;
  float* gn_partial;
  int out_f32;
  int nb;
  long long cache_stride;
  const void* w_first;
  const void* w_sub;
  const void* w_pair;
  int tdup;
  int reserved2;
} dove_conv_desc;
int dove_conv_igemm_bf16(const dove_conv_desc* d, void* stream);
const char* dove_conv_kernel_name(const dove_conv_desc* d);
int dove_conv_partial_launches(const dove_conv_desc* d);
long long dove_conv_gn_partial_rows(const dove_conv_desc* d);
int dove_groupnorm_finalize_partials(const float* partial, long long rows, double count, float eps, void* ws, float* stats,
                                     void* stream);

int dove_groupnorm_stats_bf16(const void* x, long long npix, long long frame_pix, int C, float eps, void* partial_ws, int ws_blocks,
                              float* stats, void* stream);
int dove_groupnorm_sums_bf16(const void* x, long long npix, long long frame_pix, int C, void* partial_ws, int ws_blocks, double* sums,
                             void* stream);
int dove_groupnorm_finalize_sums(const double* sums, double count, float eps, float* stats, void* stream);
int dove_groupnorm_sums_from_partials(const float* partial, long long rows, void* ws, double* sums, void* stream);
int dove_groupnorm_apply_bf16(const void* x, void* y, int T, int H, int W, int C, const float* stats,
                              const float* gamma, const float* beta, int silu, const void* yb, int hz, int wz,
                              int sshift, const int* tmap, void* stream);

int dove_groupnorm_stats_nb_bf16(const void* x, int nb, long long npix, long long frame_pix, int C, float eps, void* partial_ws,
                                 int ws_blocks, float* stats, void* stream);
int dove_groupnorm_finalize_partials_nb(const float* partial, long long rows, int nb, double count, float eps, void* ws, size_t ws_bytes,
                                        float* stats, void* stream);
int dove_groupnorm_apply_nb_bf16(const void* x, void* y, int nb, int T, int H, int W, int C, const float* stats, const float* gamma,
                                 const float* beta, int silu, const void* yb, int Tz, int hz, int wz, int sshift, const int* tmap,
                                 void* stream);
int dove_avgpool_time_nb_bf16(const void* x, int nb, int T, long long frame_elems, void* y, void* stream);

int dove_layernorm_modulate_bf16(const void* x, void* y, long long rows, int D, float eps, const float* gamma,
                                 const float* beta, const float* mod, long long split, void* stream);

int dove_qkv_post_bf16(const void* qkv, long long N, long long Npad, int heads, int head_dim, int text_len,
                       const float* gq, const float* bq, const float* gk, const float* bk, const float* cosT,
                       const float* sinT, float qscale, float eps, void* Qh, void* Kh, void* Vt, int v_order, float* norm2, void* stream);
int dove_vt_quad_swap_bf16(void* Vt, long long rows, long long Npad, void* stream);
int dove_ulysses_place_bf16(const void* rq, const void* rk, const void* rv, const long long* counts, int world, int hloc, long long N,
                            long long Npad, void* Qh, void* Kh, void* Vt, float* norm2_out, void* stream);

int dove_attention_fwd_bf16(const void* Qh, const void* Kh, const void* Vt, void* O, long long N, long long Npad,
                            int heads, int head_dim, long long ldo, float* norm2, void* stream);
int dove_attention_head_paths(const float* norm2_host, int heads, int* path);
const char* dove_attention_path_name(int path);

int dove_cl_from_ncthw(const void* x, int dtype, int C, long long npix, int Cp, float scale, float shift, void* y,
                       void* stream);
int dove_ncthw_from_cl(const void* x, long long ld, int C, long long npix, float scale, float shift, float lo,
                       float hi, void* y, int dtype, void* stream);
int dove_cl_im2col3x3_from_ncthw(const void* x, int dtype, int C, int T, int H, int W, int Cp, float scale, float shift, void* y,
                                 void* stream);
int dove_conv_out_gather(const float* p, long long ldp, int T, int H, int W, int C, const float* bias, float scale, float shift, float lo,
                         float hi, void* y, int dtype, void* stream);
int dove_avgpool_time_bf16(const void* x, int T, long long frame_elems, void* y, void* stream);
int dove_posterior_sample(const void* moments, long long ld, int latent_channels, long long npix, const void* noise,
                          int noise_dtype, void* out, int out_dtype, void* stream);
int dove_axpby(const void* x, const void* y, void* out, int dtype, long long n, float a, float b, void* stream);
int dove_patchify(const void* x, int dtype, int T, int C, int H, int W, int pt, int p, void* tokens, long long ld,
                  void* stream);
int dove_unpatchify(const void* tokens, long long ld, int T, int C, int H, int W, int pt, int p, void* y, int dtype,
                    void* stream);
int dove_conv_out_gather_cl(const float* p, long long ldp, int T, int H, int W, int C, const float* bias, void* y, int ldy, void* stream);
int dove_tile_gather_bf16(const void* x, int H, int W, int C, int t0, int nt, int th, int tw, int nb, const int* oy, const int* ox,
                          int im2col_cin, void* out, void* stream);
int dove_blend_edge_bf16(const void* a, void* b, int T, int Ha, int Wa, int Hb, int Wb, int ld, int extent, int axis,
                         void* stream);
int dove_preprocess_u8(const void* frames, int F0, int H0, int W0, int pad_f, int pad_h, int pad_w, int upscale, void* out,
                       int out_dtype, void* stream);
int dove_postprocess_u8(const void* video, int dtype, int F, int H, int W, int Fo, int Ho, int Wo, void* out, void* stream);

#define DOVE_U8 2
#define DOVE_METRIC_PSNR 1
#define DOVE_METRIC_SSIM 2
#define DOVE_METRIC_RGB_TO_Y 4
typedef struct dove_image_view {
  const void* data;
  int dtype;
  int reserved;
  long long sn, sc, sh, sw;
} dove_image_view;
size_t dove_fr_metrics_workspace_bytes(int n, int h, int w);
int dove_fr_metrics(const dove_image_view* pred, const dove_image_view* ref, int n, int channels, int h, int w, int flags, void* ws,
                    size_t ws_bytes, double* out, void* stream);
#define DOVE_COLORFIX_WAVELET 1
#define DOVE_COLORFIX_ADAIN 2
#define DOVE_COLORFIX_CLAMP 1
size_t dove_color_fix_workspace_bytes(int mode, int n, int h, int w);
int dove_color_fix(const dove_image_view* content, float c_scale, float c_bias, const dove_image_view* style, float s_scale, float s_bias,
                   int n, int h, int w, int mode, int flags, const dove_image_view* out, void* ws, size_t ws_bytes, void* stream);
#define DOVE_YUV_444 0
#define DOVE_YUV_422 1
#define DOVE_YUV_420 2
#define DOVE_YUV_MONO 3
#define DOVE_YUV_SITING_LEFT 0
#define DOVE_YUV_SITING_CENTRE 1
typedef struct dove_yuv_format {
  int coef[9];
  int offset[3];
  int chroma;
  int siting_h;
} dove_yuv_format;
size_t dove_yuv_frame_bytes(int h, int w, int chroma);
int dove_rgb_to_yuv_u8(const dove_image_view* rgb, int n, int h, int w, const dove_yuv_format* fmt, void* out, void* stream);
int dove_yuv_to_rgb_u8(const void* yuv, int n, int h, int w, const dove_yuv_format* fmt, void* out, void* stream);
int dove_gemv_bf16(const void* W, const float* bias, const float* x, int in_features, int out_features, int act_in,
                   float* y, void* stream);

int dove_mx_quant_bf16(const void* x, long long rows, int K, void* q, void* scales, void* stream);
int dove_linear_mxfp8(const void* xq, const void* xs, const void* wq, const void* ws, const float* bias, const void* resid,
                      const float* gate, void* out, long long M, int N, int K, long long ldo, long long ldr, long long gate_split,
                      int act, void* stream);

int dove_qkv_post_mxfp8(const void* qkv, long long N, long long Npad, int heads, int head_dim, int text_len,
                        const float* gq, const float* bq, const float* gk, const float* bk, const float* cosT,
                        const float* sinT, float qscale, float eps, void* Q8, void* K8, void* V8t, void* Vs,
                        void* stream);
int dove_attention_fwd_mxfp8(const void* Q8, const void* K8, const void* V8t, const void* Vs, void* O, long long N,
                             long long Npad, int heads, int head_dim, long long ldo, void* stream);

int dove_rmsnorm_bf16(const void* x, void* y, long long rows, int D, float eps, const float* weight, void* stream);
// ... 189 lines not shown
```

Baseline: 35.28 frames/s.

## Fuse QKV linear with q/k norm, RoPE and head scatter in GEMM epilogue

Refactors the gemm8p kernel into a body templated on an epilogue functor, then adds a QKV-post epilogue that applies q/k layernorm, rotary embedding, scaling and the scatter into Qh/Kh/Vt head layouts directly from the accumulators. The bf16 DiT path now calls a fused linear_qkv_post entry point instead of writing the full QKV activation and rereading it in a separate kernel. This removes one large intermediate round trip per block. In exchange the epilogue becomes heavier and may add register pressure to the GEMM, and a fallback scratch path exists for shapes the fused kernel does not cover.

```diff
diff --git a/dove_amd/csrc/graph.hip b/dove_amd/csrc/graph.hip
--- a/dove_amd/csrc/graph.hip
+++ b/dove_amd/csrc/graph.hip
@@ -1927,12 +1927,29 @@
   for (auto& b : c->blocks) {
     CHK(dove_layernorm_modulate_bf16(hs, n1, N, D, cf.dit_norm_eps, b.ln1_g, b.ln1_b, b.m1, L, stream));
     bf16_t* qkv;
-    CHK(big(n1, b.qkv, b.qkv8, ConvOpt(), &qkv));
-    if (c->opt_attn_mx) {
+    if (!c->opt_attn_mx && !c->opt_linear_mx) {
+      dove_conv_desc d;
+      memset(&d, 0, sizeof(d));
+      d.struct_size = (unsigned)sizeof(d);
+      d.x = n1; d.w = b.qkv.w; d.bias = b.qkv.bias;
+      d.t_in = d.h_in = d.t_out = d.h_out = 1; d.w_in = d.w_out = (int)N; d.cin = b.qkv.cin_pad; d.nb = 1;
+      d.cout_pad = b.qkv.cout_pad; d.cout_store = b.qkv.cout_store(); d.ldo = d.cout_store;
+      d.kt = d.kh = d.kw = 1; d.stride = 1;
+      long long rows_fused = 0, sbytes = 0;
+      CHK(dove_linear_qkv_post_plan(&d, N, npad, Hh, 1, &rows_fused, &sbytes));
+      void* scratch = sbytes ? c->arena.alloc((size_t)sbytes) : nullptr;
+      DOVE_CHECK_ARG(!sbytes || scratch, "workspace exhausted (QKV scratch)");
+      CHK(dove_linear_qkv_post_bf16(&d, N, npad, Hh, 64, L, b.nq_g, b.nq_b, b.nk_g, b.nk_b, cosp, sinp, qscale, 1e-6f, c->Qh, c->Kh, c->Vt, 1,
+                                    norm2, scratch, sbytes, stream));
+      c->arena.release(scratch);
+      CHK(dove_attention_fwd_bf16(c->Qh, c->Kh, c->Vt, n1, N, npad, Hh, 64, D, norm2, stream));
+    } else if (c->opt_attn_mx) {
+      CHK(big(n1, b.qkv, b.qkv8, ConvOpt(), &qkv));
       CHK(dove_qkv_post_mxfp8(qkv, N, npad, Hh, 64, L, b.nq_g, b.nq_b, b.nk_g, b.nk_b, cosp, sinp, qscale, 1e-6f, c->Q8, c->K8, c->V8, c->Vs8, stream));
       c->arena.release(qkv);
       CHK(dove_attention_fwd_mxfp8(c->Q8, c->K8, c->V8, c->Vs8, n1, N, npad, Hh, 64, D, stream));
     } else {
+      CHK(big(n1, b.qkv, b.qkv8, ConvOpt(), &qkv));
       CHK(dove_qkv_post_bf16(qkv, N, npad, Hh, 64, L, b.nq_g, b.nq_b, b.nk_g, b.nk_b, cosp, sinp, qscale, 1e-6f, c->Qh, c->Kh, c->Vt, 1, norm2, stream));
       c->arena.release(qkv);
       CHK(dove_attention_fwd_bf16(c->Qh, c->Kh, c->Vt, n1, N, npad, Hh, 64, D, norm2, stream));
diff --git a/dove_amd/csrc/igemm.hip b/dove_amd/csrc/igemm.hip
--- a/dove_amd/csrc/igemm.hip
+++ b/dove_amd/csrc/igemm.hip
@@ -1,4 +1,5 @@
 #include "igemm_args.h"
+#include "qk_row.h"
 
 
 template <int BN, int BK>
@@ -786,140 +787,33 @@
 constexpr int EPI = 4 * OPB;
 constexpr int LDS_BYTES = EPI + 8 * 4096;
 }
+struct Gemm8pLane { int grp, wave, lane, l15, q4, e_px, e_ch; };
+__device__ __forceinline__ void gemm8p_block_put(char* eslice, const f32x4 (&acc16)[4][8], int p, int h, int q4, int l15) {
+#pragma unroll
+  for (int dj = 0; dj < 2; ++dj)
+#pragma unroll
+    for (int di = 0; di < 2; ++di) {
+      const int row = dj * 16 + l15, ch = di * 4 + q4;
+      *(f32x4*)(eslice + row * 128 + ((ch ^ (row & 7)) << 4)) = acc16[2 * h + di][2 * p + dj];
+    }
+  asm volatile("s_waitcnt lgkmcnt(0)" ::: "memory");
+}
+__device__ __forceinline__ void gemm8p_block_rows(const char* eslice, int e_px, int e_ch, f32x4 (&lo)[2], f32x4 (&hi4)[2]) {
+#pragma unroll
+  for (int it = 0; it < 2; ++it) {
+    const int px = it * 16 + e_px;
+    lo[it] = *(const f32x4*)(eslice + px * 128 + (((2 * e_ch) ^ (px & 7)) << 4));
+    hi4[it] = *(const f32x4*)(eslice + px * 128 + (((2 * e_ch + 1) ^ (px & 7)) << 4));
+  }
+  asm volatile("s_waitcnt lgkmcnt(0)" ::: "memory");
+}
+
 template <bool kAct, bool kGate>
-__global__ __launch_bounds__(512, 2) void gemm8p_kernel(const IgemmArgs a, long long M) {
-  using gemm4x::BM;
-  using namespace gemm8p;
-  extern __shared__ __attribute__((aligned(16))) char smem[];
-  const int tid = threadIdx.x, lane = tid & 63;
-  const int wave = __builtin_amdgcn_readfirstlane(tid >> 6);
-  __builtin_assume(wave >= 0 && wave < 8);
-  const int hi = lane >> 5, l31 = lane & 31;
-  const int q4 = lane >> 4, l15 = lane & 15;
-  const int grp = wave >> 2, wc = wave & 3;
-
-  G4Const kc;
-  kc.K = a.Cin;
-  kc.M = M;
-  kc.tiles_n = a.tiles_n;
-  kc.ntiles = (int)((M + BM - 1) / BM) * a.tiles_n;
-  kc.G = (int)gridDim.x;
-  kc.nk4 = a.Cin / 128;
-  const int ntiles = kc.ntiles, G = kc.G, nk4 = kc.nk4;
-
-  unsigned voff[4];
-#pragma unroll
-  for (int jj = 0; jj < 4; ++jj) {
-    const int row = (wave * 4 + jj) * 8 + (lane >> 3);
-    const int c = (lane & 7) ^ ((row >> 1) & 7);
-    voff[jj] = (unsigned)((row * a.Cin + c * 8) * 2);
-  }
-  G4State st;
-  const bf16_t *ca_base = a.x, *cw_base = a.w, *na_base = a.x, *nw_base = a.w;
-  int ca_nrec = 0, cw_nrec = 0, c_soff = 0, na_nrec = 0, nw_nrec = 0, n_soff = 0;
-  auto publish = [&](const G4State& q) {
-    ca_base = na_base; cw_base = nw_base; ca_nrec = na_nrec; cw_nrec = nw_nrec; c_soff = n_soff;
-    na_base = q.a_base; nw_base = q.w_base; na_nrec = q.a_nrec; nw_nrec = q.w_nrec; n_soff = q.soff;
-  };
-  auto stage = [&](auto bufc, const bf16_t* ab, int anrec, const bf16_t* wb, int wnrec, int soff) {
-    constexpr int buf = decltype(bufc)::value;
-    const auto srd_a = __builtin_amdgcn_make_buffer_rsrc((void*)ab, (short)0, anrec, 0x00020000);
-    const auto srd_w = __builtin_amdgcn_make_buffer_rsrc((void*)wb, (short)0, wnrec, 0x00020000);
-#pragma unroll
-    for (int jj = 0; jj < 4; ++jj)
-      __builtin_amdgcn_raw_ptr_buffer_load_lds(srd_a, (lds_ptr_t)(smem + XB + buf * OPB + wave * 4096 + jj * 1024), 16, voff[jj], soff, 0, 0);
-#pragma unroll
-    for (int jj = 0; jj < 4; ++jj)
-      __builtin_amdgcn_raw_ptr_buffer_load_lds(srd_w, (lds_ptr_t)(smem + WB + buf * OPB + wave * 4096 + jj * 1024), 16, voff[jj], soff, 0, 0);
-  };
-
-  int aoff[2][2], boff[2][2];
-  {
-    const int ra = grp * 128 + l31, rb = wc * 64 + l31;
-#pragma unroll
-    for (int h = 0; h < 2; ++h)
-#pragma unroll
-      for (int kk = 0; kk < 2; ++kk) {
-        const int ch = h * 4 + kk * 2 + hi;
-        aoff[h][kk] = XB + ra * ROWB + ((ch ^ ((ra >> 1) & 7)) << 4);
-        boff[h][kk] = WB + rb * ROWB + ((ch ^ ((rb >> 1) & 7)) << 4);
-        asm volatile("" : "+v"(aoff[h][kk]), "+v"(boff[h][kk]));
-      }
-  }
-  int aoff16[2], boff16[2];
-  {
-    const int ra = grp * 128 + l15, rb = wc * 64 + l15;
-#pragma unroll
-    for (int h = 0; h < 2; ++h) {
-      aoff16[h] = XB + ra * ROWB + (((h * 4 + q4) ^ ((ra >> 1) & 7)) << 4);
-      boff16[h] = WB + rb * ROWB + (((h * 4 + q4) ^ ((rb >> 1) & 7)) << 4);
-      asm volatile("" : "+v"(aoff16[h]), "+v"(boff16[h]));
-    }
-  }
-  f32x4 acc16[4][8];
-  bf16x8 x16[8], w16[4];
-
-  g4_open_tile(st, a, kc, (int)blockIdx.x);
-  publish(st);
-  stage(std::integral_constant<int, 0>{}, na_base, na_nrec, nw_base, nw_nrec, n_soff);
-  g4_advance(st, a, kc);
-  publish(st);
-  asm volatile("s_waitcnt vmcnt(0)" ::: "memory");
-  __builtin_amdgcn_s_barrier();
-  asm volatile("" ::: "memory");
-  if (grp) {
-    __builtin_amdgcn_sched_barrier(0);
-    __builtin_amdgcn_s_barrier();
-    __builtin_amdgcn_sched_barrier(0);
-  }
-
-  auto step = [&](auto uc, bool hold) {
-    constexpr int u = decltype(uc)::value;
-    constexpr int buf = u >> 1, h = u & 1;
-#pragma unroll
-    for (int pb = 0; pb < 8; ++pb) x16[pb] = *(const bf16x8*)(smem + aoff16[h] + buf * OPB + pb * (16 * ROWB));
-#pragma unroll
-    for (int ib = 0; ib < 4; ++ib) w16[ib] = *(const bf16x8*)(smem + boff16[h] + buf * OPB + ib * (16 * ROWB));
-    if (u == 0) stage(std::integral_constant<int, 1>{}, ca_base, ca_nrec, cw_base, cw_nrec, c_soff + ROWB);
-    if (u == 2) stage(std::integral_constant<int, 0>{}, na_base, na_nrec, nw_base, nw_nrec, n_soff);
-    __builtin_amdgcn_sched_barrier(0);
-    if (h == 1 && grp) asm volatile("s_waitcnt vmcnt(0)" ::: "memory");
-    asm volatile("s_waitcnt lgkmcnt(0)" ::: "memory");
-    __builtin_amdgcn_s_barrier();
-    __builtin_amdgcn_sched_barrier(0);
-    __builtin_amdgcn_s_setprio(1);
-#pragma unroll
-    for (int ib = 0; ib < 4; ++ib)
-#pragma unroll
-      for (int pb = 0; pb < 8; ++pb) acc16[ib][pb] = __builtin_amdgcn_mfma_f32_16x16x32_bf16(w16[ib], x16[pb], acc16[ib][pb], 0, 0, 0);
-    __builtin_amdgcn_s_setprio(0);
-    __builtin_amdgcn_sched_barrier(0);
-    if (h == 1 && !grp) asm volatile("s_waitcnt vmcnt(0)" ::: "memory");
-    if (u == 3 && hold) return;
-    __builtin_amdgcn_s_barrier();
-    __builtin_amdgcn_sched_barrier(0);
-  };
-
-  const int e_px = lane >> 2, e_ch = lane & 3;
-  for (int tile = (int)blockIdx.x; tile < ntiles; tile += G) {
-    const G4Tile c = g4_decode(kc, tile);
-    const int col0 = c.n0 + wc * 64;
-#pragma unroll
-    for (int ib = 0; ib < 4; ++ib)
-#pragma unroll
-      for (int pb = 0; pb < 8; ++pb) acc16[ib][pb] = f32x4{0.f, 0.f, 0.f, 0.f};
-
-    for (int kq = 0; kq < nk4; ++kq) {
-      step(std::integral_constant<int, 0>{}, false);
-      step(std::integral_constant<int, 1>{}, false);
-      step(std::integral_constant<int, 2>{}, false);
-      step(std::integral_constant<int, 3>{}, grp && kq == nk4 - 1);
-      __builtin_amdgcn_sched_barrier(0);
-      g4_advance(st, a, kc);
-      publish(st);
-      __builtin_amdgcn_sched_barrier(0);
-    }
-
+struct Gemm8pStore {
+  __device__ __forceinline__ void operator()(const IgemmArgs& a, long long M, const G4Tile& c, int col0, const Gemm8pLane& ln,
+                                             const f32x4 (&acc16)[4][8], char* smem) const {
+    using namespace gemm8p;
+    const int grp = ln.grp, wave = ln.wave, l15 = ln.l15, q4 = ln.q4, e_px = ln.e_px, e_ch = ln.e_ch;
     asm volatile("" ::: "memory");
     f32x4 bias_r[2][2], gate_r[2][2][2];
 #pragma unroll
@@ -962,22 +856,9 @@
 #pragma unroll
               for (int it = 0; it < 2; ++it) rr[it] = __builtin_amdgcn_raw_buffer_load_b128(srd_r, (int)r_off[it], h * 64, 0);
             }
-#pragma unroll
-            for (int dj = 0; dj < 2; ++dj)
-#pragma unroll
-              for (int di = 0; di < 2; ++di) {
-                const int row = dj * 16 + l15, ch = di * 4 + q4;
-                *(f32x4*)(eslice + row * 128 + ((ch ^ (row & 7)) << 4)) = acc16[2 * h + di][2 * p + dj];
-              }
-            asm volatile("s_waitcnt lgkmcnt(0)" ::: "memory");
             f32x4 lo[2], hi4[2];
-#pragma unroll
-            for (int it = 0; it < 2; ++it) {
-              const int px = it * 16 + e_px;
-              lo[it] = *(const f32x4*)(eslice + px * 128 + (((2 * e_ch) ^ (px & 7)) << 4));
-              hi4[it] = *(const f32x4*)(eslice + px * 128 + (((2 * e_ch + 1) ^ (px & 7)) << 4));
-            }
-            asm volatile("s_waitcnt lgkmcnt(0)" ::: "memory");
+            gemm8p_block_put(eslice, acc16, p, h, q4, l15);
+            gemm8p_block_rows(eslice, e_px, e_ch, lo, hi4);
 #pragma unroll
             for (int it = 0; it < 2; ++it) {
               f32x4 x0 = lo[it] + bias_r[h][0], x1 = hi4[it] + bias_r[h][1];
@@ -1015,6 +896,144 @@
       if (a.resid) emit(std::true_type{});
       else emit(std::false_type{});
     }
+  }
+};
+
+template <class Epi>
+__device__ __forceinline__ void gemm8p_body(const IgemmArgs& a, long long M, const Epi& epilogue) {
+  using gemm4x::BM;
+  using namespace gemm8p;
+  extern __shared__ __attribute__((aligned(16))) char smem[];
+  const int tid = threadIdx.x, lane = tid & 63;
+  const int wave = __builtin_amdgcn_readfirstlane(tid >> 6);
+  __builtin_assume(wave >= 0 && wave < 8);
+  const int hi = lane >> 5, l31 = lane & 31;
+  const int q4 = lane >> 4, l15 = lane & 15;
+  const int grp = wave >> 2, wc = wave & 3;
+
+  G4Const kc;
+  kc.K = a.Cin;
+  kc.M = M;
+  kc.tiles_n = a.tiles_n;
+  kc.ntiles = (int)((M + BM - 1) / BM) * a.tiles_n;
+  kc.G = (int)gridDim.x;
+  kc.nk4 = a.Cin / 128;
+  const int ntiles = kc.ntiles, G = kc.G, nk4 = kc.nk4;
+
+  unsigned voff[4];
+#pragma unroll
+  for (int jj = 0; jj < 4; ++jj) {
+    const int row = (wave * 4 + jj) * 8 + (lane >> 3);
+    const int c = (lane & 7) ^ ((row >> 1) & 7);
+    voff[jj] = (unsigned)((row * a.Cin + c * 8) * 2);
+  }
+  G4State st;
+  const bf16_t *ca_base = a.x, *cw_base = a.w, *na_base = a.x, *nw_base = a.w;
+  int ca_nrec = 0, cw_nrec = 0, c_soff = 0, na_nrec = 0, nw_nrec = 0, n_soff = 0;
+  auto publish = [&](const G4State& q) {
+    ca_base = na_base; cw_base = nw_base; ca_nrec = na_nrec; cw_nrec = nw_nrec; c_soff = n_soff;
+    na_base = q.a_base; nw_base = q.w_base; na_nrec = q.a_nrec; nw_nrec = q.w_nrec; n_soff = q.soff;
+  };
+  auto stage = [&](auto bufc, const bf16_t* ab, int anrec, const bf16_t* wb, int wnrec, int soff) {
+    constexpr int buf = decltype(bufc)::value;
+    const auto srd_a = __builtin_amdgcn_make_buffer_rsrc((void*)ab, (short)0, anrec, 0x00020000);
+    const auto srd_w = __builtin_amdgcn_make_buffer_rsrc((void*)wb, (short)0, wnrec, 0x00020000);
+#pragma unroll
+    for (int jj = 0; jj < 4; ++jj)
+      __builtin_amdgcn_raw_ptr_buffer_load_lds(srd_a, (lds_ptr_t)(smem + XB + buf * OPB + wave * 4096 + jj * 1024), 16, voff[jj], soff, 0, 0);
+#pragma unroll
+    for (int jj = 0; jj < 4; ++jj)
+      __builtin_amdgcn_raw_ptr_buffer_load_lds(srd_w, (lds_ptr_t)(smem + WB + buf * OPB + wave * 4096 + jj * 1024), 16, voff[jj], soff, 0, 0);
+  };
+
+  int aoff[2][2], boff[2][2];
+  {
+    const int ra = grp * 128 + l31, rb = wc * 64 + l31;
+#pragma unroll
+    for (int h = 0; h < 2; ++h)
+#pragma unroll
+      for (int kk = 0; kk < 2; ++kk) {
+        const int ch = h * 4 + kk * 2 + hi;
+        aoff[h][kk] = XB + ra * ROWB + ((ch ^ ((ra >> 1) & 7)) << 4);
+        boff[h][kk] = WB + rb * ROWB + ((ch ^ ((rb >> 1) & 7)) << 4);
+        asm volatile("" : "+v"(aoff[h][kk]), "+v"(boff[h][kk]));
+      }
+  }
+  int aoff16[2], boff16[2];
+  {
+    const int ra = grp * 128 + l15, rb = wc * 64 + l15;
+#pragma unroll
+    for (int h = 0; h < 2; ++h) {
+      aoff16[h] = XB + ra * ROWB + (((h * 4 + q4) ^ ((ra >> 1) & 7)) << 4);
+      boff16[h] = WB + rb * ROWB + (((h * 4 + q4) ^ ((rb >> 1) & 7)) << 4);
+      asm volatile("" : "+v"(aoff16[h]), "+v"(boff16[h]));
+    }
+  }
+  f32x4 acc16[4][8];
+  bf16x8 x16[8], w16[4];
+
+  g4_open_tile(st, a, kc, (int)blockIdx.x);
+  publish(st);
+  stage(std::integral_constant<int, 0>{}, na_base, na_nrec, nw_base, nw_nrec, n_soff);
+  g4_advance(st, a, kc);
+  publish(st);
+  asm volatile("s_waitcnt vmcnt(0)" ::: "memory");
+  __builtin_amdgcn_s_barrier();
+  asm volatile("" ::: "memory");
+  if (grp) {
+    __builtin_amdgcn_sched_barrier(0);
+    __builtin_amdgcn_s_barrier();
+    __builtin_amdgcn_sched_barrier(0);
+  }
+
+  auto step = [&](auto uc, bool hold) {
+    constexpr int u = decltype(uc)::value;
+    constexpr int buf = u >> 1, h = u & 1;
+#pragma unroll
+    for (int pb = 0; pb < 8; ++pb) x16[pb] = *(const bf16x8*)(smem + aoff16[h] + buf * OPB + pb * (16 * ROWB));
+#pragma unroll
+    for (int ib = 0; ib < 4; ++ib) w16[ib] = *(const bf16x8*)(smem + boff16[h] + buf * OPB + ib * (16 * ROWB));
+    if (u == 0) stage(std::integral_constant<int, 1>{}, ca_base, ca_nrec, cw_base, cw_nrec, c_soff + ROWB);
+    if (u == 2) stage(std::integral_constant<int, 0>{}, na_base, na_nrec, nw_base, nw_nrec, n_soff);
+    __builtin_amdgcn_sched_barrier(0);
+    if (h == 1 && grp) asm volatile("s_waitcnt vmcnt(0)" ::: "memory");
+    asm volatile("s_waitcnt lgkmcnt(0)" ::: "memory");
+    __builtin_amdgcn_s_barrier();
+    __builtin_amdgcn_sched_barrier(0);
+    __builtin_amdgcn_s_setprio(1);
+#pragma unroll
+    for (int ib = 0; ib < 4; ++ib)
+#pragma unroll
+      for (int pb = 0; pb < 8; ++pb) acc16[ib][pb] = __builtin_amdgcn_mfma_f32_16x16x32_bf16(w16[ib], x16[pb], acc16[ib][pb], 0, 0, 0);
+    __builtin_amdgcn_s_setprio(0);
+    __builtin_amdgcn_sched_barrier(0);
+    if (h == 1 && !grp) asm volatile("s_waitcnt vmcnt(0)" ::: "memory");
+    if (u == 3 && hold) return;
+    __builtin_amdgcn_s_barrier();
+    __builtin_amdgcn_sched_barrier(0);
+  };
+
+  const int e_px = lane >> 2, e_ch = lane & 3;
+  for (int tile = (int)blockIdx.x; tile < ntiles; tile += G) {
+    const G4Tile c = g4_decode(kc, tile);
+    const int col0 = c.n0 + wc * 64;
+#pragma unroll
+    for (int ib = 0; ib < 4; ++ib)
+#pragma unroll
+      for (int pb = 0; pb < 8; ++pb) acc16[ib][pb] = f32x4{0.f, 0.f, 0.f, 0.f};
+
+    for (int kq = 0; kq < nk4; ++kq) {
+      step(std::integral_constant<int, 0>{}, false);
+      step(std::integral_constant<int, 1>{}, false);
+      step(std::integral_constant<int, 2>{}, false);
+      step(std::integral_constant<int, 3>{}, grp && kq == nk4 - 1);
+      __builtin_amdgcn_sched_barrier(0);
+      g4_advance(st, a, kc);
+      publish(st);
+      __builtin_amdgcn_sched_barrier(0);
+    }
+
+    epilogue(a, M, c, col0, Gemm8pLane{grp, wave, lane, l15, q4, e_px, e_ch}, acc16, smem);
     __builtin_amdgcn_s_waitcnt(0x0F70);
     asm volatile("" ::: "memory");
     if (grp) {
@@ -1027,6 +1046,155 @@
     __builtin_amdgcn_sched_barrier(0);
     __builtin_amdgcn_s_barrier();
   }
+}
+
+
+template <bool kAct, bool kGate>
+__global__ __launch_bounds__(512, 2) void gemm8p_kernel(const IgemmArgs a, long long M) {
+  gemm8p_body(a, M, Gemm8pStore<kAct, kGate>{});
+}
+
+struct QkvEpiArgs {
+  const float *gq, *bq, *gk, *bk;
+  const float *cosT, *sinT;
+  bf16_t *Qh, *Kh, *Vt;
+  float* norm2;
+  long long Npad;
+  int heads, text_len;
+  float qscale, eps;
+};
+struct Gemm8pQkvPost {
+  QkvEpiArgs q;
+  __device__ __forceinline__ void operator()(const IgemmArgs& a, long long M, const G4Tile& c, int col0, const Gemm8pLane& ln,
+                                             const f32x4 (&acc16)[4][8], char* smem) const {
+    using namespace gemm8p;
+    const int grp = ln.grp, wave = ln.wave;
+    int lane = ln.lane;
+    asm volatile("" : "+v"(lane));
+    const int l15 = lane & 15, q4 = lane >> 4, e_px = lane >> 2, e_ch = lane & 3;
+    const int D = q.heads * 64;
+    const int sec = (col0 >= D ? 1 : 0) + (col0 >= 2 * D ? 1 : 0);
+    const int head = (col0 - sec * D) >> 6;
+    char* const eslice = smem + EPI + wave * 4096;
+    asm volatile("" ::: "memory");
+    if (sec < 2) {
+      const float sc = sec == 0 ? q.qscale : 1.0f;
+      char* const dst = (char*)((sec == 0 ? q.Qh : q.Kh) + (long long)head * q.Npad * 64);
+      auto row_sum = [](const float (&part)[2]) {
+        float s0 = part[0], s1 = part[1];
+        s0 += __shfl_xor(s0, 1); s1 += __shfl_xor(s1, 1);
+        s0 += __shfl_xor(s0, 2); s1 += __shfl_xor(s1, 2);
+        return s0 + s1;
+      };
+      unsigned qmax = 0u;
+#pragma unroll
+      for (int p = 0; p < 4; ++p) {
+        const int row0 = c.m0 + grp * 128 + p * 32;
+        uint4 raw[2][2];
+#pragma unroll
+        for (int h = 0; h < 2; ++h) {
+          f32x4 bias_r[2] = {f32x4{0.f, 0.f, 0.f, 0.f}, f32x4{0.f, 0.f, 0.f, 0.f}};
+          if (a.bias) { bias_r[0] = *(const f32x4*)(a.bias + col0 + h * 32 + e_ch * 8); bias_r[1] = *(const f32x4*)(a.bias + col0 + h * 32 + e_ch * 8 + 4); }
+          f32x4 lo[2], hi4[2];
+          gemm8p_block_put(eslice, acc16, p, h, q4, l15);
+          gemm8p_block_rows(eslice, e_px, e_ch, lo, hi4);
+#pragma unroll
+          for (int it = 0; it < 2; ++it) {
+            const f32x4 x0 = lo[it] + bias_r[0], x1 = hi4[it] + bias_r[1];
+            raw[it][h] = uint4{pack_bf2(x0[0], x0[1]), pack_bf2(x0[2], x0[3]), pack_bf2(x1[0], x1[1]), pack_bf2(x1[2], x1[3])};
+            asm volatile("" : "+v"(raw[it][h].x), "+v"(raw[it][h].y), "+v"(raw[it][h].z), "+v"(raw[it][h].w));
+          }
+        }
+        QkChunkCoef kf[2];
+#pragma unroll
+        for (int h = 0; h < 2; ++h) {
+          const float* gam = (sec == 0 ? q.gq : q.gk) + h * 32 + e_ch * 8;
+          const float* bet = (sec == 0 ? q.bq : q.bk) + h * 32 + e_ch * 8;
+          kf[h].g0 = *(const f32x4*)gam; kf[h].g1 = *(const f32x4*)(gam + 4); kf[h].b0 = *(const f32x4*)bet; kf[h].b1 = *(const f32x4*)(bet + 4);
+        }
+#pragma unroll
+        for (int it = 0; it < 2; ++it) {
+          int n = row0 + it * 16 + e_px;
+          asm volatile("" : "+v"(n));
+          const bool live = n < M;
+          const bool rope = live && n >= q.text_len && q.cosT;
+          QkChunkRope rp[2];
+#pragma unroll
+          for (int h = 0; h < 2; ++h) {
+            rp[h].c0 = f32x4{1.f, 1.f, 1.f, 1.f}; rp[h].c1 = rp[h].c0; rp[h].s0 = f32x4{0.f, 0.f, 0.f, 0.f}; rp[h].s1 = rp[h].s0;
+            if (rope) {
+              const unsigned ro = (unsigned)(n - q.text_len) * 256u + (unsigned)(h * 128 + e_ch * 32);
+              const float* cr = (const float*)((const char*)q.cosT + ro);
+              const float* sr = (const float*)((const char*)q.sinT + ro);
+              rp[h].c0 = *(const f32x4*)cr; rp[h].c1 = *(const f32x4*)(cr + 4); rp[h].s0 = *(const f32x4*)sr; rp[h].s1 = *(const f32x4*)(sr + 4);
+            }
+          }
+          uint4 packed[2];
+          const float q2 = qk_row_math<2>(raw[it], kf, rp, rope, sc, q.eps, row_sum, packed);
+          if (live) {
+            const unsigned so = (unsigned)n * 128u + (unsigned)(e_ch * 16);
+            *(uint4*)(dst + so) = packed[0];
+            *(uint4*)(dst + so + 64) = packed[1];
+            qmax = max(qmax, __float_as_uint(q2));
+          }
+          __builtin_amdgcn_sched_barrier(0);
+          asm volatile("s_nop 3" ::: "memory");
+          __builtin_amdgcn_sched_barrier(0);
+        }
+      }
+      if (q.norm2) {
+        qmax = max(qmax, (unsigned)__shfl_xor((int)qmax, 4)); qmax = max(qmax, (unsigned)__shfl_xor((int)qmax, 8));
+        qmax = max(qmax, (unsigned)__shfl_xor((int)qmax, 16)); qmax = max(qmax, (unsigned)__shfl_xor((int)qmax, 32));
+        if (lane == 0) atomicMax((unsigned*)(q.norm2 + head * 2 + sec), qmax);
+      }
+    } else {
+      const int d_l = lane & 31, half = lane >> 5;
+      char* const vrow = (char*)(q.Vt + (long long)head * 64 * q.Npad);
+      const unsigned npad = (unsigned)q.Npad;
+      int rd[4];
+#pragma unroll
+      for (int e3 = 0; e3 < 4; ++e3) {
+        const int t = half * 4 + e3;
+        rd[e3] = t * 128 + (((d_l >> 2) ^ t) << 4) + (d_l & 3) * 4;
+      }
+#pragma unroll
+      for (int p = 0; p < 4; ++p) {
+        const int row0 = c.m0 + grp * 128 + p * 32;
+        const bool group_on = (row0 & ~63) < M;
+#pragma unroll
+        for (int h = 0; h < 2; ++h) {
+          gemm8p_block_put(eslice, acc16, p, h, q4, l15);
+          int d = h * 32 + d_l;
+          asm volatile("" : "+v"(d));
+          const float bias_d = a.bias ? a.bias[col0 + d] : 0.f;
+          uint4 out8[2];
+#pragma unroll
+          for (int k = 0; k < 2; ++k) {
+            float o[8];
+#pragma unroll
+            for (int e = 0; e < 8; ++e) {
+              const int t = k * 16 + half * 4 + (e & 3) + (e >> 2) * 8;
+              const float x = *(const float*)(eslice + rd[e & 3] + (k * 16 + (e >> 2) * 8) * 128) + bias_d;
+              o[e] = row0 + t < M ? x : 0.f;
+            }
+            out8[k] = pack8(o);
+          }
+          asm volatile("s_waitcnt lgkmcnt(0)" ::: "memory");
+          if (group_on) {
+#pragma unroll
+            for (int k = 0; k < 2; ++k) *(uint4*)(vrow + ((unsigned)d * npad + (unsigned)(row0 + k * 16 + half * 8)) * 2u) = out8[k];
+          }
+          __builtin_amdgcn_sched_barrier(0);
+          asm volatile("s_nop 3" ::: "memory");
+          __builtin_amdgcn_sched_barrier(0);
+        }
+      }
+    }
+  }
+};
+
+__global__ __launch_bounds__(512, 2) void gemm8p_qkv_kernel(const IgemmArgs a, long long M, const QkvEpiArgs q) {
+  gemm8p_body(a, M, Gemm8pQkvPost{q});
 }
 
 static std::atomic<bf16_t*> g_zero_page[DOVE_MAX_DEVICES] = {};
@@ -1194,7 +1362,7 @@
   return halo4x_plan(d) ? 1 : 0;
 }
 
-static int conv_dispatch(const dove_conv_desc* d, void* stream, ConvKernel kern);
+static int conv_dispatch(const dove_conv_desc* d, void* stream, ConvKernel kern, const QkvEpiArgs* qkv = nullptr);
 
 static bool gemm_tail_split(const dove_conv_desc* d, long long* rows_main) {
   const long long M = (long long)d->t_out * d->h_out * d->w_out;
@@ -1255,7 +1423,77 @@
   return conv_dispatch(d, stream, kern0);
 }
 
-static int conv_dispatch(const dove_conv_desc* d, void* stream, ConvKernel kern) {
+struct QkvPlan { bool fused; long long rows_fused, scratch_rows; };
+static QkvPlan qkv_plan(const dove_conv_desc* d, long long N, long long Npad, int heads, int v_order) {
+  QkvPlan pl = {false, 0, N};
+  const long long D3 = 3ll * heads * 64;
+  if (select_kernel(d) != K_GEMM8P || v_order != 1 || Npad % 128 != 0 || heads % 4 != 0) return pl;
+  if (d->cout_pad != D3 || d->cout_store != D3 || d->act != 0 || d->resid || d->gate) return pl;
+  pl.fused = true;
+  long long rows_main = 0;
+  pl.rows_fused = gemm_tail_split(d, &rows_main) ? rows_main : N;
+  pl.scratch_rows = N - pl.rows_fused;
+  return pl;
+}
+static bool qkv_desc_ok(const dove_conv_desc* d, long long N, int heads, const char* who) {
+  if (!desc_size_ok(d, who)) return false;
+  if (heads > 0 && N > 0 && d->t_out == 1 && d->h_out == 1 && d->t_in == 1 && d->h_in == 1 && desc_nb(d) == 1 && d->w_out == N && d->w_in == N &&
+      d->kt == 1 && d->kh == 1 && d->kw == 1 && d->stride == 1 && d->up == 0 && d->tmode == 0 && d->cout_store == 3ll * heads * 64 &&
+      d->cout_pad >= d->cout_store && d->cout_pad % 32 == 0 && d->cin > 0 && d->cin % 32 == 0 && d->act == 0 && !d->resid && !d->gate && !d->out_f32 && !d->gn_partial)
+    return true;
+  dove_set_error("%s: the descriptor must be a plain token-major linear [1, 1, N] -> 3 * heads * 64 channels (no activation / residual)", who);
+  return false;
+}
+extern "C" int dove_linear_qkv_post_plan(const dove_conv_desc* gemm, long long N, long long Npad, int heads, int v_order, long long* rows_fused,
+                                         long long* scratch_bytes) {
+  if (!qkv_desc_ok(gemm, N, heads, "linear_qkv_post_plan")) return DOVE_EINVAL;
+  const QkvPlan pl = qkv_plan(gemm, N, Npad, heads, v_order);
+  if (rows_fused) *rows_fused = pl.rows_fused;
+  if (scratch_bytes) *scratch_bytes = pl.scratch_rows * 3ll * heads * 64 * 2;
+  return DOVE_OK;
+}
+extern "C" int dove_linear_qkv_post_bf16(const dove_conv_desc* gemm, long long N, long long Npad, int heads, int head_dim, int text_len,
+                                          const float* gq, const float* bq, const float* gk, const float* bk, const float* cosT, const float* sinT,
+                                          float qscale, float eps, void* Qh, void* Kh, void* Vt, int v_order, float* norm2, void* scratch,
+                                          long long scratch_bytes, void* stream) {
+  DOVE_CHECK_ARG(head_dim == 64, "linear_qkv_post: head_dim must be 64 (got %d)", head_dim);
+  if (!qkv_desc_ok(gemm, N, heads, "linear_qkv_post")) return DOVE_EINVAL;
+  DOVE_CHECK_ARG(gemm->x && gemm->w && Qh && Kh && Vt && gq && bq && gk && bk, "linear_qkv_post: null pointer");
+  DOVE_CHECK_ARG(Npad >= N && Npad < (1ll << 24), "linear_qkv_post: Npad must be >= N and below 2^24");
+  DOVE_CHECK_ARG((cosT == nullptr) == (sinT == nullptr), "linear_qkv_post: cos/sin must both be given or both be null");
+  DOVE_CHECK_ARG(v_order == 0 || (v_order == 1 && Npad % 16 == 0), "linear_qkv_post: v_order 1 (quad-swapped V^T) needs Npad %% 16 == 0");
+  DOVE_CHECK_ARG(text_len >= 0, "linear_qkv_post: negative text_len");
+  const QkvPlan pl = qkv_plan(gemm, N, Npad, heads, v_order);
+  const long long D3 = 3ll * heads * 64;
+  DOVE_CHECK_ARG(pl.scratch_rows == 0 || (scratch && scratch_bytes >= pl.scratch_rows * D3 * 2),
+                 "linear_qkv_post: scratch (%lld bytes) is smaller than dove_linear_qkv_post_plan asks for (%lld)", scratch_bytes, pl.scratch_rows * D3 * 2);
+  if (norm2) {
+    const hipError_t me = hipMemsetAsync(norm2, 0, sizeof(float) * 2 * heads, (hipStream_t)stream);
+    if (me != hipSuccess) { dove_set_error("linear_qkv_post: clearing norm2 failed: %s", hipGetErrorString(me)); return DOVE_ELAUNCH; }
+  }
+  dove_conv_desc t = *gemm;
+  t.out = scratch; t.ldo = D3;
+  if (!pl.fused) {
+    const int rc = dove_conv_igemm_bf16(&t, stream);
+    return rc ? rc : qkv_post_launch_rows(scratch, 0, N, Npad, heads, text_len, gq, bq, gk, bk, cosT, sinT, qscale, eps, Qh, Kh, Vt, v_order, norm2, stream);
+  }
+  QkvEpiArgs q;
+  q.gq = gq; q.bq = bq; q.gk = gk; q.bk = bk; q.cosT = cosT; q.sinT = sinT;
+  q.Qh = (bf16_t*)Qh; q.Kh = (bf16_t*)Kh; q.Vt = (bf16_t*)Vt; q.norm2 = norm2;
+  q.Npad = Npad; q.heads = heads; q.text_len = text_len; q.qscale = qscale; q.eps = eps;
+  dove_conv_desc m = *gemm;
+  m.out = nullptr;
+  m.w_in = m.w_out = (int)pl.rows_fused;
+  int rc = conv_dispatch(&m, stream, K_GEMM8P, &q);
+  if (rc || pl.scratch_rows == 0) return rc;
+  t.w_in = t.w_out = (int)pl.scratch_rows;
+  t.x = (const char*)gemm->x + pl.rows_fused * gemm->cin * 2;
+  rc = conv_dispatch(&t, stream, K_IGEMM_FAST);
+  return rc ? rc : qkv_post_launch_rows(scratch, pl.rows_fused, N, Npad, heads, text_len, gq, bq, gk, bk, cosT, sinT, qscale, eps, Qh, Kh, Vt, v_order,
+                                        norm2, stream);
+}
+
+static int conv_dispatch(const dove_conv_desc* d, void* stream, ConvKernel kern, const QkvEpiArgs* qkv) {
   const bf16_t* zp = zero_page();
   DOVE_CHECK_ARG(zp, "conv_igemm: could not allocate the zero page");
   IgemmArgs a;
@@ -1293,7 +1531,11 @@
         (void)hipFuncSetAttribute((const void*)gemm8p_kernel<true, false>, hipFuncAttributeMaxDynamicSharedMemorySize, gemm8p::LDS_BYTES);
         (void)hipFuncSetAttribute((const void*)gemm8p_kernel<false, true>, hipFuncAttributeMaxDynamicSharedMemorySize, gemm8p::LDS_BYTES);
       }
-      if (d->gate) hipLaunchKernelGGL((gemm8p_kernel<false, true>), dim3(grid4), dim3(512), gemm8p::LDS_BYTES, s, a, M);
+      if (qkv) {
+        static PerDeviceOnce attrq;
+        if (auto once_ = attrq.guard()) (void)hipFuncSetAttribute((const void*)gemm8p_qkv_kernel, hipFuncAttributeMaxDynamicSharedMemorySize, gemm8p::LDS_BYTES);
+        hipLaunchKernelGGL(gemm8p_qkv_kernel, dim3(grid4), dim3(512), gemm8p::LDS_BYTES, s, a, M, *qkv);
+      } else if (d->gate) hipLaunchKernelGGL((gemm8p_kernel<false, true>), dim3(grid4), dim3(512), gemm8p::LDS_BYTES, s, a, M);
       else if (d->act == 1) hipLaunchKernelGGL((gemm8p_kernel<true, false>), dim3(grid4), dim3(512), gemm8p::LDS_BYTES, s, a, M);
       else hipLaunchKernelGGL((gemm8p_kernel<false, false>), dim3(grid4), dim3(512), gemm8p::LDS_BYTES, s, a, M);
       DOVE_CHECK_LAUNCH("dove_conv_igemm_bf16(gemm8p)");
diff --git a/dove_amd/csrc/igemm_args.h b/dove_amd/csrc/igemm_args.h
--- a/dove_amd/csrc/igemm_args.h
+++ b/dove_amd/csrc/igemm_args.h
@@ -97,3 +97,7 @@
 }
 
 int launch_igemm_legacy(const IgemmArgs& a, unsigned grid, int BN, bool bk64, hipStream_t s);
+
+int qkv_post_launch_rows(const void* qkv, long long row0, long long N, long long Npad, int heads, int text_len, const float* gq, const float* bq,
+                         const float* gk, const float* bk, const float* cosT, const float* sinT, float qscale, float eps, void* Qh, void* Kh,
+                         void* Vt, int v_order, float* norm2, void* stream);
diff --git a/dove_amd/csrc/norm.hip b/dove_amd/csrc/norm.hip
--- a/dove_amd/csrc/norm.hip
+++ b/dove_amd/csrc/norm.hip
@@ -1,4 +1,5 @@
 #include "common.h"
+#include "qk_row.h"
 #include "../../include/dove_hip.h"
 
 __global__ __launch_bounds__(256) void gn_partial_kernel(const bf16_t* __restrict__ xall, long long npix, int C,
@@ -404,7 +405,7 @@
 }
 
 constexpr int QK_HB = 8;
-__global__ __launch_bounds__(256) void qk_post_kernel(const bf16_t* __restrict__ qkv, long long N, long long Npad, int heads, int text_len,
+__global__ __launch_bounds__(256) void qk_post_kernel(const bf16_t* __restrict__ qkv, long long row0, long long N, long long Npad, int heads, int text_len,
                                                       const float* __restrict__ gq, const float* __restrict__ bq,
                                                       const float* __restrict__ gk, const float* __restrict__ bk,
                                                       const float* __restrict__ cosT, const float* __restrict__ sinT, float qscale, float eps,
@@ -412,63 +413,36 @@
   __shared__ unsigned smax[4][QK_HB];
   const int c = threadIdx.x & 7;
   const int h0 = blockIdx.y * QK_HB, which = blockIdx.z;
-  const long long n = (long long)blockIdx.x * 32 + (threadIdx.x >> 3);
+  const long long n = row0 + (long long)blockIdx.x * 32 + (threadIdx.x >> 3);
   const int D = heads * 64;
   const bool live = n < N;
   const long long nn = live ? n : N - 1;
   const float* gam = (which == 0 ? gq : gk) + c * 8;
   const float* bet = (which == 0 ? bq : bk) + c * 8;
-  const f32x4 g0 = *(const f32x4*)gam, g1 = *(const f32x4*)(gam + 4), b0 = *(const f32x4*)bet, b1 = *(const f32x4*)(bet + 4);
+  QkChunkCoef kf[1];
+  kf[0].g0 = *(const f32x4*)gam; kf[0].g1 = *(const f32x4*)(gam + 4); kf[0].b0 = *(const f32x4*)bet; kf[0].b1 = *(const f32x4*)(bet + 4);
   const bool rope = nn >= text_len && cosT;
-  f32x4 c0 = {1.f, 1.f, 1.f, 1.f}, c1 = c0, s0 = {0.f, 0.f, 0.f, 0.f}, s1 = s0;
+  QkChunkRope rp[1];
+  rp[0].c0 = f32x4{1.f, 1.f, 1.f, 1.f}; rp[0].c1 = rp[0].c0; rp[0].s0 = f32x4{0.f, 0.f, 0.f, 0.f}; rp[0].s1 = rp[0].s0;
   if (rope) {
     const float* cr = cosT + (nn - text_len) * 64 + c * 8;
     const float* sr = sinT + (nn - text_len) * 64 + c * 8;
-    c0 = *(const f32x4*)cr; c1 = *(const f32x4*)(cr + 4); s0 = *(const f32x4*)sr; s1 = *(const f32x4*)(sr + 4);
+    rp[0].c0 = *(const f32x4*)cr; rp[0].c1 = *(const f32x4*)(cr + 4); rp[0].s0 = *(const f32x4*)sr; rp[0].s1 = *(const f32x4*)(sr + 4);
   }
   const float sc = which == 0 ? qscale : 1.0f;
-  const bf16_t* src = qkv + nn * (3LL * D) + (long long)which * D + c * 8;
+  const bf16_t* src = qkv + (nn - row0) * (3LL * D) + (long long)which * D + c * 8;
   bf16_t* dst = (which == 0 ? Qh : Kh) + nn * 64 + c * 8;
   uint4 raw[QK_HB];
 #pragma unroll
   for (int j = 0; j < QK_HB; ++j) raw[j] = h0 + j < heads ? *(const uint4*)(src + (h0 + j) * 64) : uint4{0u, 0u, 0u, 0u};
+  auto row_sum = [](const float (&part)[1]) { float s = part[0]; s += __shfl_xor(s, 1); s += __shfl_xor(s, 2); s += __shfl_xor(s, 4); return s; };
 #pragma unroll
   for (int j = 0; j < QK_HB; ++j) {
-    float f[8];
-    unpack8(raw[j], f);
-    float s = 0.f;
-#pragma unroll
-    for (int e = 0; e < 8; ++e) s += f[e];
-    s += __shfl_xor(s, 1); s += __shfl_xor(s, 2); s += __shfl_xor(s, 4);
-    const float mean = s * (1.0f / 64.0f);
-    float v = 0.f;
-#pragma unroll
-    for (int e = 0; e < 8; ++e) { const float t = f[e] - mean; v += t * t; }
-    v += __shfl_xor(v, 1); v += __shfl_xor(v, 2); v += __shfl_xor(v, 4);
-    const float rstd = rsqrtf(v * (1.0f / 64.0f) + eps);
-#pragma unroll
-    for (int e = 0; e < 8; ++e) f[e] = (f[e] - mean) * rstd * (e < 4 ? g0[e] : g1[e - 4]) + (e < 4 ? b0[e] : b1[e - 4]);
-    if (rope) {
-#pragma unroll
-      for (int i = 0; i < 4; ++i) {
-        const float a = f[2 * i], b = f[2 * i + 1];
-        const float ca = i < 2 ? c0[2 * i] : c1[2 * i - 4], cb = i < 2 ? c0[2 * i + 1] : c1[2 * i - 3];
-        const float sa = i < 2 ? s0[2 * i] : s1[2 * i - 4], sb = i < 2 ? s0[2 * i + 1] : s1[2 * i - 3];
-        f[2 * i] = a * ca - b * sa;
-        f[2 * i + 1] = b * cb + a * sb;
-      }
-    }
-#pragma unroll
-    for (int e = 0; e < 8; ++e) f[e] *= sc;
-    const uint4 packed = pack8(f);
-    if (live && h0 + j < heads) *(uint4*)(dst + (long long)(h0 + j) * Npad * 64) = packed;
+    const uint4 rw[1] = {raw[j]};
+    uint4 packed[1];
+    const float q = qk_row_math<1>(rw, kf, rp, rope, sc, eps, row_sum, packed);
+    if (live && h0 + j < heads) *(uint4*)(dst + (long long)(h0 + j) * Npad * 64) = packed[0];
     if (norm2) {
-      float r[8];
-      unpack8(packed, r);
-      float q = 0.f;
-#pragma unroll
-      for (int e = 0; e < 8; ++e) q += r[e] * r[e];
-      q += __shfl_xor(q, 1); q += __shfl_xor(q, 2); q += __shfl_xor(q, 4);
       unsigned qb = __float_as_uint(q);
       qb = max(qb, (unsigned)__shfl_xor((int)qb, 8)); qb = max(qb, (unsigned)__shfl_xor((int)qb, 16)); qb = max(qb, (unsigned)__shfl_xor((int)qb, 32));
       if ((threadIdx.x & 63) == 0) smax[threadIdx.x >> 6][j] = qb;
@@ -483,12 +457,12 @@
   }
 }
 
-__global__ __launch_bounds__(256) void v_post_kernel(const bf16_t* __restrict__ qkv, long long N, long long Npad, int heads,
+__global__ __launch_bounds__(256) void v_post_kernel(const bf16_t* __restrict__ qkv, long long row0, long long N, long long Npad, int heads,
                                                      bf16_t* __restrict__ Vt, int v_swap) {
   __shared__ float vt[4][64][65];
   const int lane = threadIdx.x & 63, wave = threadIdx.x >> 6;
   const int h = blockIdx.y;
-  const long long n0 = ((long long)blockIdx.x * 4 + wave) * 64;
+  const long long n0 = row0 + ((long long)blockIdx.x * 4 + wave) * 64;
   if (n0 >= N) return;
   const int D = heads * 64;
   const int t8 = lane >> 3, c = lane & 7;
@@ -496,7 +470,7 @@
   for (int i = 0; i < 8; ++i) {
     const long long n = n0 + i * 8 + t8;
     float f[8];
-    if (n < N) unpack8(*(const uint4*)(qkv + n * (3LL * D) + 2LL * D + h * 64 + c * 8), f);
+    if (n < N) unpack8(*(const uint4*)(qkv + (n - row0) * (3LL * D) + 2LL * D + h * 64 + c * 8), f);
     else {
 #pragma unroll
       for (int e = 0; e < 8; ++e) f[e] = 0.f;
@@ -520,6 +494,18 @@
     bf16_t* dst = Vt + ((long long)h * 64 + lane) * Npad + n0;
     for (int j = 0; j < 64 && n0 + j < N; ++j) dst[j] = f2bf(vt[wave][j][lane]);
   }
+}
+
+int qkv_post_launch_rows(const void* qkv, long long row0, long long N, long long Npad, int heads, int text_len, const float* gq, const float* bq,
+                         const float* gk, const float* bk, const float* cosT, const float* sinT, float qscale, float eps, void* Qh, void* Kh,
+                         void* Vt, int v_order, float* norm2, void* stream) {
+  const long long rows = N - row0;
+  hipLaunchKernelGGL(qk_post_kernel, dim3((unsigned)((rows + 31) / 32), (unsigned)((heads + QK_HB - 1) / QK_HB), 2), dim3(256), 0, (hipStream_t)stream,
+                     (const bf16_t*)qkv, row0, N, Npad, heads, text_len, gq, bq, gk, bk, cosT, sinT, qscale, eps, (bf16_t*)Qh, (bf16_t*)Kh, norm2);
+  hipLaunchKernelGGL(v_post_kernel, dim3((unsigned)((rows + 255) / 256), heads), dim3(256), 0, (hipStream_t)stream, (const bf16_t*)qkv, row0, N, Npad,
+                     heads, (bf16_t*)Vt, v_order);
+  DOVE_CHECK_LAUNCH("dove_qkv_post_bf16");
+  return DOVE_OK;
 }
 
 extern "C" int dove_qkv_post_bf16(const void* qkv, long long N, long long Npad, int heads, int head_dim, int text_len,
@@ -535,12 +521,7 @@
     const hipError_t me = hipMemsetAsync(norm2, 0, sizeof(float) * 2 * heads, (hipStream_t)stream);
     if (me != hipSuccess) { dove_set_error("qkv_post: clearing norm2 failed: %s", hipGetErrorString(me)); return DOVE_ELAUNCH; }
   }
-  hipLaunchKernelGGL(qk_post_kernel, dim3((unsigned)((N + 31) / 32), (unsigned)((heads + QK_HB - 1) / QK_HB), 2), dim3(256), 0, (hipStream_t)stream, (const bf16_t*)qkv, N, Npad, heads,
-                     text_len, gq, bq, gk, bk, cosT, sinT, qscale, eps, (bf16_t*)Qh, (bf16_t*)Kh, norm2);
-  hipLaunchKernelGGL(v_post_kernel, dim3((unsigned)((N + 255) / 256), heads), dim3(256), 0, (hipStream_t)stream, (const bf16_t*)qkv, N, Npad, heads,
-                     (bf16_t*)Vt, v_order);
-  DOVE_CHECK_LAUNCH("dove_qkv_post_bf16");
-  return DOVE_OK;
+  return qkv_post_launch_rows(qkv, 0, N, Npad, heads, text_len, gq, bq, gk, bk, cosT, sinT, qscale, eps, Qh, Kh, Vt, v_order, norm2, stream);
 }
 
 __global__ __launch_bounds__(256) void vt_quad_swap_kernel(uint4* __restrict__ vt, long long ngroups) {
diff --git a/dove_amd/csrc/qk_row.h b/dove_amd/csrc/qk_row.h
--- /dev/null
+++ b/dove_amd/csrc/qk_row.h
@@ -0,0 +1,58 @@
+#pragma once
+#include "common.h"
+
+struct QkChunkCoef { f32x4 g0, g1, b0, b1; };
+struct QkChunkRope { f32x4 c0, c1, s0, s1; };
+
+template <int NCH, class Reduce>
+__device__ __forceinline__ float qk_row_math(const uint4 (&raw)[NCH], const QkChunkCoef (&k)[NCH], const QkChunkRope (&r)[NCH], bool rope, float sc,
+                                             float eps, Reduce reduce, uint4 (&packed)[NCH]) {
+#pragma clang fp contract(off)
+  float f[NCH][8], part[NCH];
+#pragma unroll
+  for (int c = 0; c < NCH; ++c) {
+    unpack8(raw[c], f[c]);
+    float s = 0.f;
+#pragma unroll
+    for (int e = 0; e < 8; ++e) s = s + f[c][e];
+    part[c] = s;
+  }
+  const float mean = reduce(part) * (1.0f / 64.0f);
+#pragma unroll
+  for (int c = 0; c < NCH; ++c) {
+#pragma unroll
+    for (int e = 0; e < 8; ++e) f[c][e] = f[c][e] - mean;
+    float v = f[c][0] * f[c][0] + f[c][1] * f[c][1];
+#pragma unroll
+    for (int e = 2; e < 8; ++e) v = v + f[c][e] * f[c][e];
+    part[c] = v;
+  }
+  const float rstd = rsqrtf(__builtin_fmaf(reduce(part), 1.0f / 64.0f, eps));
+#pragma unroll
+  for (int c = 0; c < NCH; ++c) {
+    float* const x = f[c];
+#pragma unroll
+    for (int e = 0; e < 8; ++e) x[e] = __builtin_fmaf(x[e] * rstd, e < 4 ? k[c].g0[e] : k[c].g1[e - 4], e < 4 ? k[c].b0[e] : k[c].b1[e - 4]);
+    if (rope) {
+#pragma unroll
+      for (int i = 0; i < 4; ++i) {
+        const float a = x[2 * i], b = x[2 * i + 1];
+        const float ca = i < 2 ? r[c].c0[2 * i] : r[c].c1[2 * i - 4], cb = i < 2 ? r[c].c0[2 * i + 1] : r[c].c1[2 * i - 3];
+        const float sa = i < 2 ? r[c].s0[2 * i] : r[c].s1[2 * i - 4], sb = i < 2 ? r[c].s0[2 * i + 1] : r[c].s1[2 * i - 3];
+        const float bsa = b * sa;
+        x[2 * i] = i == 0 ? a * ca - bsa : __builtin_fmaf(a, ca, -bsa);
+        x[2 * i + 1] = i == 3 ? __builtin_fmaf(a, sb, b * cb) : __builtin_fmaf(b, cb, a * sb);
+      }
+    }
+#pragma unroll
+    for (int e = 0; e < 8; ++e) x[e] = x[e] * sc;
+    packed[c] = pack8(x);
+    float s[8];
+    unpack8(packed[c], s);
+    float q = __builtin_fmaf(s[0], s[0], s[1] * s[1]);
+#pragma unroll
+    for (int e = 2; e < 8; ++e) q = __builtin_fmaf(s[e], s[e], q);
+    part[c] = q;
+  }
+  return reduce(part);
+}
diff --git a/dove_amd/lib.py b/dove_amd/lib.py
--- a/dove_amd/lib.py
+++ b/dove_amd/lib.py
@@ -133,6 +133,8 @@
     "dove_layernorm_modulate_bf16": [_VP, _VP, _LL, _I, _F, _VP, _VP, _VP, _LL, _VP],
     "dove_qkv_post_bf16": [_VP, _LL, _LL, _I, _I, _I, _VP, _VP, _VP, _VP, _VP, _VP, _F, _F, _VP, _VP, _VP, _I, _VP, _VP],
     "dove_vt_quad_swap_bf16": [_VP, _LL, _LL, _VP],
+    "dove_linear_qkv_post_plan": [C.POINTER(ConvDesc), _LL, _LL, _I, _I, C.POINTER(C.c_longlong), C.POINTER(C.c_longlong)],
+    "dove_linear_qkv_post_bf16": [C.POINTER(ConvDesc), _LL, _LL, _I, _I, _I, _VP, _VP, _VP, _VP, _VP, _VP, _F, _F, _VP, _VP, _VP, _I, _VP, _VP, _LL, _VP],
     "dove_ulysses_place_bf16": [_VP, _VP, _VP, C.POINTER(C.c_longlong), _I, _I, _LL, _LL, _VP, _VP, _VP, _VP, _VP],
     "dove_cl_im2col3x3_from_ncthw": [_VP, _I, _I, _I, _I, _I, _I, _F, _F, _VP, _VP],
     "dove_conv_out_gather": [_VP, _LL, _I, _I, _I, _I, _VP, _F, _F, _F, _F, _VP, _I, _VP],
diff --git a/dove_amd/ops.py b/dove_amd/ops.py
--- a/dove_amd/ops.py
+++ b/dove_amd/ops.py
@@ -354,6 +354,56 @@
                                         L.stream_ptr()), "dove_qkv_post_bf16")
 
 
+def _qkv_linear_desc(N, pc: PackedConv, x=None):
+    Cx = pc.cin_pad
+    if x is not None and tuple(x.shape) != (N, Cx):
+        raise RuntimeError(f"linear_qkv_post: input is {tuple(x.shape)}, packed weight expects {(N, Cx)}")
+    d = L.ConvDesc()
+    d.nb = 1
+    if x is not None:
+        d.x, d.w = x.data_ptr(), pc.w.data_ptr()
+        d.bias = pc.bias.data_ptr() if pc.bias is not None else None
+    d.t_in, d.h_in, d.w_in, d.cin = 1, 1, N, Cx
+    d.t_out, d.h_out, d.w_out = 1, 1, N
+    d.cout_pad, d.cout_store = pc.cout_pad, pc.cout_store
+    d.kt, d.kh, d.kw, d.stride, d.pad_h, d.pad_w = pc.kt, pc.kh, pc.kw, 1, 0, 0
+    d.ldo = pc.cout_store
+    return d
+
+
+def linear_qkv_post_plan(N, pc: PackedConv, Npad, heads, v_order=1):
+    d = _qkv_linear_desc(N, pc)
+    rows, sb = C.c_longlong(0), C.c_longlong(0)
+    L.check(L.load().dove_linear_qkv_post_plan(C.byref(d), N, Npad, heads, v_order, C.byref(rows), C.byref(sb)), "dove_linear_qkv_post_plan")
+    return int(rows.value), int(sb.value)
+
+
+def linear_qkv_post(x, pc: PackedConv, Npad, heads, text_len, gq, bq, gk, bk, cos, sin, qscale, eps, Qh, Kh, Vt, v_order=1, norm2=None):
+    N = x.shape[0]
+    if not x.is_cuda:
+        qkv = linear(x, pc)
+        return qkv_post(qkv, N, Npad, heads, text_len, gq, bq, gk, bk, cos, sin, qscale, eps, Qh, Kh, Vt, v_order=v_order, norm2=norm2)
+    L.require_cuda(x, gq, bq, gk, bk, cos, sin, Qh, Kh, Vt, norm2)
+    assert x.dtype == torch.bfloat16 and x.dim() == 2 and x.is_contiguous(), (x.dtype, x.shape)
+    if norm2 is not None:
+        assert norm2.dtype == torch.float32 and norm2.shape == (heads, 2) and norm2.is_contiguous()
+    d = _qkv_linear_desc(N, pc, x)
+    rows, sb = C.c_longlong(0), C.c_longlong(0)
+    L.check(L.load().dove_linear_qkv_post_plan(C.byref(d), N, Npad, heads, v_order, C.byref(rows), C.byref(sb)), "dove_linear_qkv_post_plan")
+    scratch = torch.empty(sb.value // 2, dtype=torch.bfloat16, device=x.device) if sb.value else None
+    if _profiler is not None:
+        e0, e1 = torch.cuda.Event(enable_timing=True), torch.cuda.Event(enable_timing=True)
+        e0.record()
+    L.check(L.load().dove_linear_qkv_post_bf16(C.byref(d), N, Npad, heads, 64, text_len, L.ptr(gq), L.ptr(bq), L.ptr(gk), L.ptr(bk), L.ptr(cos),
+                                               L.ptr(sin), qscale, eps, L.ptr(Qh), L.ptr(Kh), L.ptr(Vt), v_order, L.ptr(norm2), L.ptr(scratch),
+                                               sb.value, L.stream_ptr()), "dove_linear_qkv_post_bf16")
+    if _profiler is not None:
+        e1.record()
+        flops = 2.0 * N * pc.cout * pc.cin
+        name = "gemm8p_qkv_kernel" if rows.value else L.load().dove_conv_kernel_name(C.byref(d)).decode() + "+qkv_post"
+        _profiler.append(((pc.cin, pc.cout, 1), flops, e0, e1, name, flops))
+
+
 def vt_quad_swap(Vt):
     L.require_cuda(Vt)
     assert Vt.is_contiguous()
diff --git a/dove_amd/transformer.py b/dove_amd/transformer.py
--- a/dove_amd/transformer.py
+++ b/dove_amd/transformer.py
@@ -192,14 +192,19 @@
             big = ops.linear
         for bi, (blk, md) in enumerate(zip(self.blocks, blocks_mod)):
             n1 = ops.layernorm_modulate(hs, blk["ln1"][0], blk["ln1"][1], self.eps, md["m1"], Lt)
-            qkv = big(n1, blk["qkv"])
             if Vs is not None:
+                qkv = big(n1, blk["qkv"])
                 ops.qkv_post_mx(qkv, N, npad, Lh, Lt, blk["nq"][0], blk["nq"][1], blk["nk"][0], blk["nk"][1], cos, sin, qscale,
                                 1e-6, Qh, Kh, Vt, Vs)
                 att = ops.attention_mx(Qh, Kh, Vt, Vs, N, npad, Lh, n1)
             else:
-                ops.qkv_post(qkv, N, npad, Lh, Lt, blk["nq"][0], blk["nq"][1], blk["nk"][0], blk["nk"][1], cos, sin, qscale,
-                             1e-6, Qh, Kh, Vt, norm2=norm2)
+                if self.linear_precision == "bf16":
+                    ops.linear_qkv_post(n1, blk["qkv"], npad, Lh, Lt, blk["nq"][0], blk["nq"][1], blk["nk"][0], blk["nk"][1], cos, sin, qscale,
+                                        1e-6, Qh, Kh, Vt, norm2=norm2)
+                else:
+                    qkv = big(n1, blk["qkv"])
+                    ops.qkv_post(qkv, N, npad, Lh, Lt, blk["nq"][0], blk["nq"][1], blk["nk"][0], blk["nk"][1], cos, sin, qscale,
+                                 1e-6, Qh, Kh, Vt, norm2=norm2)
                 if self.attn_bound_trace is not None:
                     self.attn_bound_trace.append(norm2.clone())
                 att = ops.attention(Qh, Kh, Vt, N, npad, Lh, n1, norm2=norm2 if self.attn_score_bound else None)
diff --git a/include/dove_hip.h b/include/dove_hip.h
--- a/include/dove_hip.h
+++ b/include/dove_hip.h
@@ -73,6 +73,12 @@
                        const float* gq, const float* bq, const float* gk, const float* bk, const float* cosT,
                        const float* sinT, float qscale, float eps, void* Qh, void* Kh, void* Vt, int v_order, float* norm2, void* stream);
 int dove_vt_quad_swap_bf16(void* Vt, long long rows, long long Npad, void* stream);
+int dove_linear_qkv_post_plan(const dove_conv_desc* gemm, long long N, long long Npad, int heads, int v_order, long long* rows_fused,
+                              long long* scratch_bytes);
+int dove_linear_qkv_post_bf16(const dove_conv_desc* gemm, long long N, long long Npad, int heads, int head_dim, int text_len,
+                              const float* gq, const float* bq, const float* gk, const float* bk, const float* cosT,
+                              const float* sinT, float qscale, float eps, void* Qh, void* Kh, void* Vt, int v_order, float* norm2,
+                              void* scratch, long long scratch_bytes, void* stream);
 int dove_ulysses_place_bf16(const void* rq, const void* rk, const void* rv, const long long* counts, int world, int hloc, long long N,
                             long long Npad, void* Qh, void* Kh, void* Vt, float* norm2_out, void* stream);
 
```

New measurement: 35.36 frames/s, median of 3. Within noise of the previous version (+0.2%).
